# sdecoder/AVX-sort-merge-joins

Hardware: AMD Instinct MI355X
Metric: join throughput Mtuples/s (R⋈S) + achieved HBM GB/s, 128M⋈128M at 1/2/4/8 GPU (higher is better)
Workload: dtype int64; 1 GPU; sortmergejoin_multiway R=128000000 S=128000000 per GPU, 16-byte tuples, uniform, PK/FK keys 1..|R|, row-id payloads (48-bit intermediates); tuples_per_relation_per_gpu=128000000, tuples_per_relation_total=128000000, tuple_bytes=16, payload=rowid, distribution=uniform, parallelism=range-partition x1

## Files before the change

avx-sort-merge-joins_amd/csrc/bucketsort.hip:

```cpp
#include <algorithm>
#include <type_traits>
#include <vector>

#include "smj_common.hpp"
#include "smj_internal.hpp"

namespace smj {

#ifndef SMJ_TP_THREADS
#define SMJ_TP_THREADS 1024
#endif
constexpr int TP_THREADS = SMJ_TP_THREADS;
#ifndef SMJ_TP_PERSIST
#define SMJ_TP_PERSIST 1
#endif
#ifndef SMJ_GS_XCD
#define SMJ_GS_XCD 1
#endif
#ifndef SMJ_GS_PAIR
#define SMJ_GS_PAIR 1
#endif
#ifndef SMJ_GS_TWO
#define SMJ_GS_TWO 1
#endif
#ifndef SMJ_GS_META_PREFETCH
#define SMJ_GS_META_PREFETCH 0
#endif
#ifndef SMJ_GS_ARGS_MEM
#define SMJ_GS_ARGS_MEM 1
#endif
#ifndef SMJ_TP_STAGE4
#define SMJ_TP_STAGE4 (64 * 1024)
#endif
#ifndef SMJ_TP_STAGE8
#define SMJ_TP_STAGE8 (128 * 1024)
#endif
template <class W>
constexpr int tp_items() {
    return (int)((sizeof(W) == 4 ? SMJ_TP_STAGE4 : sizeof(W) == 8 ? SMJ_TP_STAGE8 : 128 * 1024)
                 / sizeof(W)) / TP_THREADS;
}
template <class W>
constexpr uint32_t tile_elems() {
    return (uint32_t)(TP_THREADS * tp_items<W>());
}
static_assert(tile_elems<uint64_t>() <= 65535 + 1, "u16 prefix rows");
template <class Lay>
struct TileStage {
    static constexpr uint32_t kBytes = sizeof(typename Lay::W);
    static constexpr int kItems = tp_items<typename Lay::W>();
};
template <>
struct TileStage<LayP48> {
    static constexpr uint32_t kBytes = 4;
    static constexpr int kItems = tp_items<uint64_t>();
};
template <class Lay>
constexpr uint32_t tile_elems_l() {
    return (uint32_t)(TP_THREADS * TileStage<Lay>::kItems);
}
#ifndef SMJ_PLAN_TILE
#define SMJ_PLAN_TILE 16384
#endif
const uint32_t kTileTuples = SMJ_PLAN_TILE;

#ifndef SMJ_GS_THREADS
#define SMJ_GS_THREADS 256
#endif
constexpr int GS_THREADS = SMJ_GS_THREADS;
#ifndef SMJ_GS_WG_PER_CU
#define SMJ_GS_WG_PER_CU 2
#endif
#ifndef SMJ_GS_WG_PER_CU8
#define SMJ_GS_WG_PER_CU8 4
#endif
#ifndef SMJ_GS_WG_PER_CU12
#define SMJ_GS_WG_PER_CU12 3
#endif
#ifndef SMJ_GS_WG_PER_CU4P
#define SMJ_GS_WG_PER_CU4P 5
#endif
template <class W, bool PAIR = false>
constexpr int gs_wg_per_cu() {
    return sizeof(W) == 16 ? SMJ_GS_WG_PER_CU
         : sizeof(W) == 12 ? SMJ_GS_WG_PER_CU12
         : (sizeof(W) == 4 && PAIR) ? SMJ_GS_WG_PER_CU4P : SMJ_GS_WG_PER_CU8;
}
#ifndef SMJ_GS_ITEMS
#define SMJ_GS_ITEMS (2560 / SMJ_GS_THREADS)
#endif
constexpr int GS_ITEMS = SMJ_GS_ITEMS;
constexpr int GS_CAP = GS_THREADS * GS_ITEMS;
constexpr int GS_D3MAX = GS_CAP >= 2048 ? 11 : 10;
constexpr int GS_BPT = (1 << GS_D3MAX) / GS_THREADS;
constexpr int GS_NB3 = 1 << GS_D3MAX;
constexpr int GS_TMAX = 256;
constexpr int GS_WIN = GS_CAP / 64;
constexpr int GS_RUNMAX = 32;
static_assert(GS_CAP % 64 == 0 && GS_CAP % GS_THREADS == 0, "group capacity");

#ifdef KEY_8B
typedef int64_t KeyT;
#else
typedef int32_t KeyT;
#endif

struct TileTable {
    uint64_t* off;
    uint32_t* len;
    uint32_t* bucket;
    uint32_t* btile0;
    uint16_t* pref;
    uint16_t* prefT;
    uint32_t tstride;
};

struct OvfEntry {
    uint32_t bucket, d2;
    uint32_t nr[2];
    uint64_t off[2];
    uint32_t counted;
    uint32_t pad;
};

__global__ void __launch_bounds__(64)
k_tiles(const uint64_t* __restrict__ bstart, const int64_t* __restrict__ bcount,
        const uint64_t* __restrict__ seg_start, const int64_t* __restrict__ seg_cnt,
        uint32_t nseg, TileTable tt, uint32_t tsz) {
    const uint32_t b = blockIdx.x;
    uint32_t t0 = tt.btile0[b];
    for (uint32_t q = 0; q < nseg; q++) {
        const uint64_t s0 = seg_start ? seg_start[(size_t)b * nseg + q] : bstart[b];
        const int64_t cnt = seg_cnt ? seg_cnt[(size_t)b * nseg + q] : bcount[b];
        const uint32_t nt = (uint32_t)((cnt + tsz - 1) / tsz);
        for (uint32_t i = threadIdx.x; i < nt; i += 64) {
            const uint64_t o = (uint64_t)i * tsz;
            const int64_t rem = cnt - (int64_t)o;
            tt.off[t0 + i] = s0 + o;
            tt.len[t0 + i] = (uint32_t)(rem < (int64_t)tsz ? rem : tsz);
            tt.bucket[t0 + i] = b;
        }
        t0 += nt;
    }
}

struct TilePassArgs {
    const void* part[2];
    void* tmp[2];
    TileTable tt[2];
    uint32_t t0[2];
    uint32_t nt[2];
    const uint32_t* ntiles[2];
    RangePlan plan;
    uint32_t nb2;
    const unsigned int* pack_bad;
    uint32_t d2_fast;
    uint64_t pstride[2] = {0, 0};
    uint64_t ostride[2] = {0, 0};
};

template <class Lay, class LayO = Lay>
__global__ void __launch_bounds__(TP_THREADS)
k_tilepass(TilePassArgs A) {
    typedef typename Lay::W W;
    static_assert(std::is_same<W, typename LayO::W>::value, "one element type");
    typedef TileStage<Lay> TS;
    constexpr int TP_ITEMS = TS::kItems;
    constexpr uint32_t TSZ = tile_elems_l<Lay>();
    extern __shared__ __attribute__((aligned(16))) unsigned char lds_raw[];
    if (A.pack_bad && *A.pack_bad) return;
    const RangePlan& P = A.plan;
    const uint32_t nb2 = A.nb2;
    W* stage = reinterpret_cast<W*>(lds_raw);
    uint32_t* hist = reinterpret_cast<uint32_t*>(lds_raw + ((TSZ * TS::kBytes + 15) & ~15u));
    uint32_t* scr = hist + nb2;

    const int r = blockIdx.x < A.nt[0] ? 0 : 1;
    const uint32_t t = A.t0[r] + (r ? blockIdx.x - A.nt[0] : blockIdx.x);
    if (A.ntiles[r] && t >= *A.ntiles[r]) return;
    const TileTable& tt = A.tt[r];
    const typename Lay::CView part = Lay::cview(A.part[r], A.pstride[r]);
    const typename LayO::View tmp =
        LayO::view(A.tmp[r], std::is_same<Lay, LayO>::value ? A.pstride[r] : A.ostride[r]);
    const uint64_t off = tt.off[t];
    const uint32_t len = tt.len[t];
    const uint32_t b = tt.bucket[t];

    for (uint32_t d = threadIdx.x; d < nb2; d += TP_THREADS) hist[d] = 0;
    W v[TP_ITEMS];
    uint32_t dg[TP_ITEMS];
#pragma unroll
    for (int j = 0; j < TP_ITEMS; j++) {
        uint32_t i = j * TP_THREADS + threadIdx.x;
        if (i < len) v[j] = part[off + i];
    }
    __syncthreads();
    if (A.d2_fast && b != 0 && b != (1u << P.D1) - 1) {
        const uint32_t base_lo = (uint32_t)P.base, mask = nb2 - 1;
#pragma unroll
        for (int j = 0; j < TP_ITEMS; j++) {
            uint32_t i = j * TP_THREADS + threadIdx.x;
            if (i < len) {
                dg[j] = Lay::digit_fast(v[j], base_lo, P.s1, P.s2, mask);
                atomicAdd(&hist[dg[j]], 1u);
            }
        }
    } else {
#pragma unroll
        for (int j = 0; j < TP_ITEMS; j++) {
            uint32_t i = j * TP_THREADS + threadIdx.x;
            if (i < len) {
                dg[j] = plan_d2(P, Lay::rel(P, v[j], b), b);
                atomicAdd(&hist[dg[j]], 1u);
            }
        }
    }
    __syncthreads();
    const uint32_t per = (nb2 + TP_THREADS - 1) / TP_THREADS;
    const uint32_t d0 = threadIdx.x * per;
    uint32_t loc = 0;
    for (uint32_t k = 0; k < per; k++)
        if (d0 + k < nb2) loc += hist[d0 + k];
    uint32_t tot;
    uint32_t ex = block_exclusive_scan(loc, scr, &tot);
    uint16_t* pref = tt.pref + (uint64_t)t * (nb2 + 1);
    for (uint32_t k = 0; k < per; k++) {
        uint32_t d = d0 + k;
        if (d < nb2) {
            uint32_t c = hist[d];
            hist[d] = ex;
            pref[d] = (uint16_t)ex;
            ex += c;
        }
    }
    if (threadIdx.x == 0) pref[nb2] = (uint16_t)len;
    __syncthreads();
#pragma unroll
    for (int j = 0; j < TP_ITEMS; j++) {
        uint32_t i = j * TP_THREADS + threadIdx.x;
        if (i < len) {
            uint32_t pos = atomicAdd(&hist[dg[j]], 1u);
            stage[pos] = v[j];
        }
    }
    __syncthreads();
#pragma unroll
    for (int j = 0; j < TP_ITEMS; j++) {
        uint32_t i = j * TP_THREADS + threadIdx.x;
        if (i < len) st_w(tmp + off + i, stage[i]);
    }
}

template <class LayO>
struct Plane2;
template <>
struct Plane2<LayP48> {
    typedef uint16_t T;
};
template <>
struct Plane2<LayP40> {
    typedef uint8_t T;
};
__device__ __forceinline__ void st_plane(G32 p, uint32_t v) {
#if SMJ_NT_STORES
    __builtin_nontemporal_store(v, p);
#else
    *p = v;
#endif
}
__device__ __forceinline__ void st_plane(G16 p, uint16_t v) {
#if SMJ_NT_STORES
    __builtin_nontemporal_store(v, p);
#else
    *p = v;
#endif
}
__device__ __forceinline__ void st_plane(G8 p, uint8_t v) {
#if SMJ_NT_STORES
    __builtin_nontemporal_store(v, p);
#else
    *p = v;
#endif
}

constexpr int TP48_WG_PER_CU = 2;

template <class LayO>
__global__ void __launch_bounds__(TP_THREADS, TP48_WG_PER_CU * TP_THREADS / 256)
k_tilepass48(TilePassArgs A) {
    typedef LayP48 Lay;
    typedef typename Plane2<LayO>::T HT;
    constexpr int TP_ITEMS = TileStage<Lay>::kItems;
    constexpr uint32_t TSZ = tile_elems_l<Lay>();
    static_assert(TP_ITEMS % 2 == 0, "uint16 pairs");
    static_assert(TileStage<Lay>::kBytes == 4 && (TSZ + 4) * sizeof(HT) <= TSZ * 4, "one stage");
    extern __shared__ __attribute__((aligned(16))) unsigned char lds_raw[];
    if (A.pack_bad && *A.pack_bad) return;
    const RangePlan& P = A.plan;
    const uint32_t nb2 = A.nb2;
    uint32_t* stage_lo = reinterpret_cast<uint32_t*>(lds_raw);
    HT* stage_hi = reinterpret_cast<HT*>(lds_raw);
    uint32_t* hist = reinterpret_cast<uint32_t*>(lds_raw + ((TSZ * 4 + 15) & ~15u));
    uint32_t* scr = hist + nb2;

    const int r = blockIdx.x < A.nt[0] ? 0 : 1;
    const uint32_t t = A.t0[r] + (r ? blockIdx.x - A.nt[0] : blockIdx.x);
    if (A.ntiles[r] && t >= *A.ntiles[r]) return;
    const TileTable& tt = A.tt[r];
    const uint64_t off = tt.off[t];
    const uint32_t len = tt.len[t];
    const uint32_t b = tt.bucket[t];
    const Lay::CView part = Lay::cview(A.part[r], A.pstride[r]) + off;
    const typename LayO::View tmp =
        LayO::view(A.tmp[r], std::is_same<Lay, LayO>::value ? A.pstride[r] : A.ostride[r]) + off;

    for (uint32_t d = threadIdx.x; d < nb2; d += TP_THREADS) hist[d] = 0;
    uint32_t lo[TP_ITEMS];
    uint32_t hp[TP_ITEMS / 2];
    uint32_t rk[TP_ITEMS / 2];
#pragma unroll
    for (int k = 0; k < TP_ITEMS / 2; k++) {
        uint32_t h[2] = {0, 0};
#pragma unroll
        for (int e = 0; e < 2; e++) {
            const int j = 2 * k + e;
            const uint32_t i = j * TP_THREADS + threadIdx.x;
            lo[j] = 0;
            if (i < len) {
                lo[j] = (part.lo + j * TP_THREADS)[threadIdx.x];
                h[e] = (part.hi + j * TP_THREADS)[threadIdx.x];
            }
        }
        hp[k] = h[0] | (h[1] << 16);
    }
    auto word = [&](int j) -> uint64_t {
        const uint32_t h = (j & 1) ? hp[j >> 1] >> 16 : hp[j >> 1] & 0xffffu;
        return (uint64_t)lo[j] | ((uint64_t)h << 32);
    };
    __syncthreads();
    const bool fast = A.d2_fast && b != 0 && b != (1u << P.D1) - 1;
    const uint32_t base_lo = (uint32_t)P.base, mask = nb2 - 1;
    if (fast) {
#pragma unroll
        for (int j = 0; j < TP_ITEMS; j++) {
            const uint32_t i = j * TP_THREADS + threadIdx.x;
            if (i < len) atomicAdd(&hist[Lay::digit_fast(word(j), base_lo, P.s1, P.s2, mask)], 1u);
        }
    } else {
#pragma unroll
        for (int j = 0; j < TP_ITEMS; j++) {
            const uint32_t i = j * TP_THREADS + threadIdx.x;
            if (i < len) atomicAdd(&hist[plan_d2(P, Lay::rel(P, word(j), b), b)], 1u);
        }
    }
    __syncthreads();
    const uint32_t per = (nb2 + TP_THREADS - 1) / TP_THREADS;
    const uint32_t d0 = threadIdx.x * per;
    uint32_t loc = 0;
    for (uint32_t k = 0; k < per; k++)
        if (d0 + k < nb2) loc += hist[d0 + k];
    uint32_t tot;
    uint32_t ex = block_exclusive_scan(loc, scr, &tot);
    uint16_t* pref = tt.pref + (uint64_t)t * (nb2 + 1);
    for (uint32_t k = 0; k < per; k++) {
        uint32_t d = d0 + k;
        if (d < nb2) {
            uint32_t c = hist[d];
            hist[d] = ex;
            pref[d] = (uint16_t)ex;
            ex += c;
        }
    }
    if (threadIdx.x == 0) pref[nb2] = (uint16_t)len;
    __syncthreads();
#pragma unroll
    for (int k = 0; k < TP_ITEMS / 2; k++) {
        uint32_t p[2] = {0, 0};
#pragma unroll
        for (int e = 0; e < 2; e++) {
            const int j = 2 * k + e;
            const uint32_t i = j * TP_THREADS + threadIdx.x;
            if (i < len) {
                const uint64_t w = word(j);
                const uint32_t d = fast ? Lay::digit_fast(w, base_lo, P.s1, P.s2, mask)
                                        : plan_d2(P, Lay::rel(P, w, b), b);
                p[e] = atomicAdd(&hist[d], 1u);
                stage_lo[p[e]] = lo[j];
            }
        }
        rk[k] = p[0] | (p[1] << 16);
    }
    __syncthreads();
#pragma unroll
    for (int j = 0; j < TP_ITEMS; j++) {
        const uint32_t i = j * TP_THREADS + threadIdx.x;
        if (i < len) st_plane(tmp.lo + j * TP_THREADS + threadIdx.x, stage_lo[i]);
    }
    __syncthreads();
    constexpr uint32_t EPD = 4 / sizeof(HT);
    const uint32_t pad = (uint32_t)(((uintptr_t)tmp.hi & 3u) / sizeof(HT));
#pragma unroll
    for (int j = 0; j < TP_ITEMS; j++) {
        const uint32_t i = j * TP_THREADS + threadIdx.x;
        if (i < len) {
            const uint32_t pos = (j & 1) ? rk[j >> 1] >> 16 : rk[j >> 1] & 0xffffu;
            const uint32_t h = (j & 1) ? hp[j >> 1] >> 16 : hp[j >> 1];
            stage_hi[pad + pos] = (HT)h;
        }
    }
    __syncthreads();
    const uint32_t end = pad + len;
    const uint32_t nq = (end + EPD - 1) / EPD;
    const uint32_t* stage_q = reinterpret_cast<const uint32_t*>(lds_raw);
    const G32 out_q = (G32)(tmp.hi - pad);
    constexpr int NQ = (int)((TSZ / EPD + TP_THREADS - 1) / TP_THREADS) + 1;
#pragma unroll
    for (int j = 0; j < NQ; j++) {
        const uint32_t q = j * TP_THREADS + threadIdx.x;
        if (q < nq) {
            const uint32_t e0 = q * EPD;
            if (e0 >= pad && e0 + EPD <= end) {
                st_plane(out_q + j * TP_THREADS + threadIdx.x, stage_q[q]);
            } else {
#pragma unroll
                for (uint32_t e = e0; e < e0 + EPD; e++)
                    if (e >= pad && e < end) st_plane(tmp.hi + (e - pad), stage_hi[e]);
            }
        }
    }
}

template <class Lay, class LayO>
struct TilePassP {
    typedef typename Lay::W W;
    static constexpr int ITEMS = tp_items<W>();
    __device__ static __forceinline__ uint32_t elem(int j) {
        return (uint32_t)j * TP_THREADS + threadIdx.x;
    }
    const TilePassArgs& A;
    W* stage;
    uint32_t* hist;
    uint32_t* scr;
    uint32_t n0, total;

    struct Meta {
        uint64_t off;
        uint32_t len, b, t;
        int r;
    };
    __device__ __forceinline__ Meta meta(uint32_t idx) const {
        const bool none = idx >= total;
        if (none) idx = total - 1;
        Meta m;
        m.r = idx < n0 ? 0 : 1;
        m.t = A.t0[m.r] + (m.r ? idx - n0 : idx);
        const TileTable& tt = A.tt[m.r];
        typedef const __attribute__((address_space(4))) uint64_t* C64;
        typedef const __attribute__((address_space(4))) uint32_t* C32;
        m.off = ((C64)tt.off)[m.t];
        m.len = none ? 0u : ((C32)tt.len)[m.t];
        m.b = ((C32)tt.bucket)[m.t];
        return m;
    }
    __device__ __forceinline__ void load(W (&v)[ITEMS], const Meta& m) const {
        const typename Lay::CView part = Lay::cview(A.part[m.r], A.pstride[m.r]) + m.off;
        const uint32_t lim = m.len ? m.len - 1 : 0u;
#pragma unroll
        for (int j = 0; j < ITEMS; j++) {
            const uint32_t i = elem(j);
            v[j] = part[i < lim ? i : lim];
        }
    }
    template <bool RANK>
    __device__ __forceinline__ void digits(const W (&v)[ITEMS], const Meta& m) const {
        const RangePlan& P = A.plan;
        if (A.d2_fast && m.b != 0 && m.b != (1u << P.D1) - 1) {
            const uint32_t base_lo = (uint32_t)P.base, mask = A.nb2 - 1;
#pragma unroll
            for (int j = 0; j < ITEMS; j++) {
                const uint32_t i = elem(j);
                if (i < m.len) {
                    const uint32_t d = Lay::digit_fast(v[j], base_lo, P.s1, P.s2, mask);
                    if (RANK)
                        stage[atomicAdd(&hist[d], 1u)] = v[j];
                    else
                        atomicAdd(&hist[d], 1u);
                }
            }
        } else {
#pragma unroll
            for (int j = 0; j < ITEMS; j++) {
                const uint32_t i = elem(j);
                if (i < m.len) {
                    const uint32_t d = plan_d2(P, Lay::rel(P, v[j], m.b), m.b);
                    if (RANK)
                        stage[atomicAdd(&hist[d], 1u)] = v[j];
                    else
                        atomicAdd(&hist[d], 1u);
                }
            }
        }
    }
    __device__ __forceinline__ void tile(const W (&v)[ITEMS], const Meta& m) const {
        const uint32_t nb2 = A.nb2;
        __syncthreads();
        digits<false>(v, m);
        __syncthreads();
        const uint32_t per = (nb2 + TP_THREADS - 1) / TP_THREADS;
        const uint32_t d0 = threadIdx.x * per;
        uint32_t loc = 0;
        for (uint32_t k = 0; k < per; k++)
            if (d0 + k < nb2) loc += hist[d0 + k];
        uint32_t tot;
        uint32_t ex = block_exclusive_scan(loc, scr, &tot);
        uint16_t* pref = A.tt[m.r].pref + (uint64_t)m.t * (nb2 + 1);
        for (uint32_t k = 0; k < per; k++) {
            const uint32_t d = d0 + k;
            if (d < nb2) {
                const uint32_t c = hist[d];
                hist[d] = ex;
                pref[d] = (uint16_t)ex;
                ex += c;
            }
        }
        if (threadIdx.x == 0) pref[nb2] = (uint16_t)m.len;
        __syncthreads();
        digits<true>(v, m);
        __syncthreads();
        for (uint32_t d = threadIdx.x; d < nb2; d += TP_THREADS) hist[d] = 0;
        const typename LayO::View tmp = LayO::view(
            A.tmp[m.r], std::is_same<Lay, LayO>::value ? A.pstride[m.r] : A.ostride[m.r]) + m.off;
#pragma unroll
        for (int j = 0; j < ITEMS; j++) {
            const uint32_t i = elem(j);
            if (i < m.len) st_w(tmp + i, stage[i]);
        }
    }
};

template <class Lay, class LayO = Lay>
__global__ void __launch_bounds__(TP_THREADS)
k_tilepass_p(TilePassArgs A) {
    typedef TilePassP<Lay, LayO> TP;
    typedef typename TP::W W;
    static_assert(std::is_same<W, typename LayO::W>::value, "one element type");
    extern __shared__ __attribute__((aligned(16))) unsigned char lds_raw[];
    if (A.pack_bad && *A.pack_bad) return;
    TP s{A};
    s.stage = reinterpret_cast<W*>(lds_raw);
    s.hist = reinterpret_cast<uint32_t*>(lds_raw + tile_elems<W>() * sizeof(W));
    s.scr = s.hist + A.nb2;
    uint32_t n[2];
    for (int r = 0; r < 2; r++)
        n[r] = A.nt[r] == 0 ? 0u : A.ntiles[r] ? min(*A.ntiles[r], A.nt[r]) : A.nt[r];
    s.n0 = n[0];
    s.total = n[0] + n[1];
    uint32_t idx = blockIdx.x;
    if (idx >= s.total) return;
    for (uint32_t d = threadIdx.x; d < A.nb2; d += TP_THREADS) s.hist[d] = 0;
    W a[TP::ITEMS], b[TP::ITEMS];
    typename TP::Meta ma = s.meta(idx), mb;
    s.load(a, ma);
    for (;;) {
        mb = s.meta(idx + gridDim.x);
        s.load(b, mb);
        s.tile(a, ma);
        if ((idx += gridDim.x) >= s.total) break;
        ma = s.meta(idx + gridDim.x);
        s.load(a, ma);
        s.tile(b, mb);
        if ((idx += gridDim.x) >= s.total) break;
    }
}

constexpr int PT_TILES = 64;
__global__ void __launch_bounds__(256)
k_preft(TileTable tt0, TileTable tt1, uint32_t nb0, const uint32_t* __restrict__ ntiles0,
        const uint32_t* __restrict__ ntiles1, uint32_t nt0_host, uint32_t nt1_host,
        uint32_t nb2) {
    extern __shared__ uint16_t sp[];
    const int r = blockIdx.x < nb0 ? 0 : 1;
    const TileTable& tt = r ? tt1 : tt0;
    const uint32_t ntl = (r ? ntiles1 : ntiles0) ? *(r ? ntiles1 : ntiles0)
                                                 : (r ? nt1_host : nt0_host);
    const uint32_t tb = (r ? blockIdx.x - nb0 : blockIdx.x) * PT_TILES;
    if (tb >= ntl) return;
    const uint32_t nt = min((uint32_t)PT_TILES, ntl - tb);
    const uint32_t row = nb2 + 1;
    const uint16_t* src = tt.pref + (uint64_t)tb * row;
    for (uint32_t i = threadIdx.x; i < nt * row; i += 256) sp[i] = src[i];
    __syncthreads();
    for (uint32_t i = threadIdx.x; i < row * PT_TILES; i += 256) {
        const uint32_t d = i / PT_TILES, t = i % PT_TILES;
        if (t < nt) tt.prefT[(uint64_t)d * tt.tstride + tb + t] = sp[t * row + d];
    }
}

struct GroupArgs {
    const void* tmp[2];
    Tup* out[2];
    const uint64_t* bstart[2];
    const uint64_t* ostart[2];
    TileTable tt[2];
    int nrel;
    RangePlan plan;
    unsigned long long* count_dev;
    uint32_t nb2;
    uint32_t g_begin, g_end;
    uint32_t per;
    OvfEntry* ovf;
    uint32_t* novf;
    uint32_t ovf_cap;
    const unsigned int* pack_bad;
    uint32_t d3_fast;
    uint64_t pstride[2] = {0, 0};
    uint32_t pair;
};

__device__ __forceinline__ uint32_t otid() {
    uint32_t t = threadIdx.x;
    asm volatile("" : "+v"(t));
    return t;
}

template <class W>
struct GroupLDS {
    W B[GS_CAP + 1];
    uint32_t cnt[2][GS_NB3 / 2];
    uint32_t cur[GS_NB3 / 2];
    uint32_t run[2][GS_TMAX];
    struct alignas(16) Win {
        unsigned long long m;
        uint32_t wk, pad;
    } win[2][GS_WIN];
    uint32_t wtot[2][GS_THREADS / 64];
    uint32_t flags;
    unsigned long long scan64[GS_THREADS / 64 + 1];
    uint32_t n[2];
    uint32_t off[2];
};

struct SrcPlain {
    __device__ static __forceinline__ void run(const TileTable& tt, uint32_t nb2, uint32_t t,
                                               uint32_t g, uint32_t& lo, uint32_t& len) {
        const uint16_t* pf = tt.prefT + (uint64_t)g * tt.tstride + t;
        lo = pf[0];
        len = (uint32_t)(pf[tt.tstride] - pf[0]);
    }
    template <class V>
    __device__ static __forceinline__ auto load(const V& p) { return p[0]; }
};

template <int TPL>
struct GroupMeta {
    uint32_t b[2], g[2];
    uint32_t t0[2], nt[2];
    uint64_t bst[2];
    uint64_t ost[2];
    uint32_t lo[TPL], len[TPL];
    uint32_t toff[TPL];
};

template <bool PAIR>
__device__ __forceinline__ int group_slots(const GroupArgs& A) { return PAIR ? 2 : A.nrel; }

template <class Src, bool PAIR, int TPL>
__device__ __forceinline__ void load_meta(const GroupArgs& A, uint32_t g0, uint32_t stride,
                                          uint32_t cnt, uint32_t j, GroupMeta<TPL>& M,
                                          bool same_bucket) {
    const int nslot = group_slots<PAIR>(A);
    auto bucket_meta = [&](int r, uint32_t b) {
        M.t0[r] = __builtin_amdgcn_readfirstlane(A.tt[r].btile0[b]);
        M.nt[r] = __builtin_amdgcn_readfirstlane(A.tt[r].btile0[b + 1]) - M.t0[r];
        const uint64_t bs = A.bstart[r][b];
        M.bst[r] = ((uint64_t)__builtin_amdgcn_readfirstlane((uint32_t)(bs >> 32)) << 32) |
                   __builtin_amdgcn_readfirstlane((uint32_t)bs);
        const uint64_t os = A.ostart[r][b];
        M.ost[r] = ((uint64_t)__builtin_amdgcn_readfirstlane((uint32_t)(os >> 32)) << 32) |
                   __builtin_amdgcn_readfirstlane((uint32_t)os);
    };
    if (!PAIR) {
        const uint32_t gi = g0 + j * stride;
        const uint32_t b = gi / A.nb2;
        M.g[0] = gi % A.nb2;
        if (!same_bucket || b != M.b[0]) {
#pragma unroll
            for (int r = 0; r < 2; r++) {
                M.t0[r] = M.nt[r] = 0;
                M.bst[r] = M.ost[r] = 0;
                if (r < A.nrel) bucket_meta(r, b);
            }
        }
        M.b[0] = b;
    } else {
#pragma unroll
        for (int r = 0; r < 2; r++) {
            const uint32_t k = 2 * j + r;
            const bool valid = k < cnt;
            const uint32_t gi = g0 + k * stride;
            const uint32_t b = valid ? gi / A.nb2 : 0xffffffffu;
            M.g[r] = valid ? gi % A.nb2 : 0u;
            if (!valid) {
                M.t0[r] = M.nt[r] = 0;
                M.bst[r] = M.ost[r] = 0;
            } else if (!same_bucket || b != M.b[r]) {
                bucket_meta(r, b);
            }
            M.b[r] = b;
        }
    }
    const uint32_t wid = __builtin_amdgcn_readfirstlane(otid() >> 6), lane = otid() & 63;
#pragma unroll
    for (int h = 0; h < TPL; h++) M.lo[h] = M.len[h] = M.toff[h] = 0;
    if (wid < (uint32_t)nslot) {
        const uint32_t nt = wid ? M.nt[1] : M.nt[0];
        const uint32_t t0 = wid ? M.t0[1] : M.t0[0];
        const uint32_t g = PAIR && wid ? M.g[1] : M.g[0];
#pragma unroll
        for (int h = 0; h < TPL; h++) {
            const uint32_t t = lane + 64 * h;
            if (nt <= 64 * TPL && t < nt) {
                Src::run(A.tt[wid], A.nb2, t0 + t, g, M.lo[h], M.len[h]);
                M.toff[h] = (uint32_t)(A.tt[wid].off[t0 + t] - (wid ? M.bst[1] : M.bst[0]));
            }
        }
    }
}

__device__ __forceinline__ uint32_t wave_incl_scan32(uint32_t x) {
    const int lane = lane_id();
#pragma unroll
    for (int o = 1; o < 64; o <<= 1) {
        const uint32_t y = __shfl_up(x, o, 64);
        if (lane >= o) x += y;
    }
    return x;
}

__device__ __forceinline__ unsigned long long wave_incl_scan64(unsigned long long x) {
    const int lane = lane_id();
#pragma unroll
    for (int o = 1; o < 64; o <<= 1) {
        const unsigned long long y = __shfl_up(x, o, 64);
        if (lane >= o) x += y;
    }
    return x;
}

__device__ __forceinline__ void wave_lds_sync() {
    __builtin_amdgcn_fence(__ATOMIC_RELEASE, "wavefront");
    __builtin_amdgcn_wave_barrier();
    __builtin_amdgcn_fence(__ATOMIC_ACQUIRE, "wavefront");
}

__device__ __forceinline__ unsigned long long block_scan64(unsigned long long v,
                                                           unsigned long long* scr,
                                                           unsigned long long* total) {
    const int lane = lane_id(), wid = otid() >> 6, nw = blockDim.x >> 6;
    const unsigned long long x = wave_incl_scan64(v);
    if (lane == 63) scr[wid] = x;
    __syncthreads();
    if (otid() == 0) {
        unsigned long long run = 0;
        for (int w = 0; w < nw; w++) {
            const unsigned long long t = scr[w];
            scr[w] = run;
            run += t;
        }
        scr[nw] = run;
    }
    __syncthreads();
    const unsigned long long r = scr[wid] + x - v;
    *total = scr[nw];
    __syncthreads();
    return r;
}

template <class Lay>
__device__ __forceinline__ void insertion_sort(typename Lay::W* a, uint32_t n) {
    for (uint32_t i = 1; i < n; i++) {
        typename Lay::W x = a[i];
        uint32_t j = i;
        while (j > 0 && Lay::less(x, a[j - 1])) {
            a[j] = a[j - 1];
            j--;
        }
        a[j] = x;
    }
}

template <bool PAIR, int TPL, class LDS>
__device__ __forceinline__ void build_tables(const GroupArgs& A, LDS& L,
                                             const GroupMeta<TPL>& M) {
    const uint32_t wid = otid() >> 6, lane = otid() & 63;
    if (wid < (uint32_t)group_slots<PAIR>(A)) {
        const int r = wid;
        const uint32_t nt = r ? M.nt[1] : M.nt[0];
        if (lane < GS_WIN) L.win[r][lane].m = 0ull;
        unsigned long long acc = 0;
        uint32_t kacc = 0;
        uint32_t s[TPL], k[TPL];
        bool e[TPL];
#pragma unroll
        for (int h = 0; h < TPL; h++) {
            const unsigned long long p = ((unsigned long long)M.lo[h] << 32) | M.len[h];
            const unsigned long long incl = wave_incl_scan64(p) + acc;
            acc = __shfl(incl, 63, 64);
            s[h] = (uint32_t)(incl - p);
            e[h] = lane + 64 * h < nt && M.len[h] > 0 && s[h] < GS_CAP;
            const uint64_t bal = __ballot(e[h]);
            k[h] = kacc + (uint32_t)__popcll(bal & lanemask_lt());
            kacc += (uint32_t)__popcll(bal);
        }
#pragma unroll
        for (int h = 0; h < TPL; h++)
            if (e[h]) L.run[r][k[h]] = M.toff[h] + M.lo[h] - s[h];
        if (lane == 0) {
            L.n[r] = nt <= 64 * TPL ? (uint32_t)acc : 0xffffffffu;
            L.off[r] = (uint32_t)(acc >> 32);
        }
        wave_lds_sync();
#pragma unroll
        for (int h = 0; h < TPL; h++)
            if (e[h]) atomicOr(&L.win[r][s[h] >> 6].m, 1ull << (s[h] & 63));
        wave_lds_sync();
        const uint32_t c = lane < GS_WIN ? (uint32_t)__popcll(L.win[r][lane].m) : 0u;
        const uint32_t incl = wave_incl_scan32(c);
        if (lane < GS_WIN) L.win[r][lane].wk = incl - c - 1u;
    }
    __syncthreads();
}

template <class Src, bool PAIR, class LDS, class Meta>
__device__ __forceinline__ void group_overflow(const GroupArgs& A, LDS& L,
                                               const Meta& M, int slot = 0) {
    uint32_t nn[2] = {0, 0};
    uint64_t oo[2] = {0, 0};
    const uint32_t tid = otid();
    const int nq = PAIR ? 1 : A.nrel;
#pragma unroll
    for (int q = 0; q < 2; q++) {
        if (q >= nq) break;
        const int r = PAIR ? slot : q;
        const uint32_t t0 = r ? M.t0[1] : M.t0[0], nt = r ? M.nt[1] : M.nt[0];
        const uint32_t g = PAIR && r ? M.g[1] : M.g[0];
        unsigned long long acc = 0;
        for (uint32_t t = tid; t < nt; t += GS_THREADS) {
            uint32_t lo, len;
            Src::run(A.tt[r], A.nb2, t0 + t, g, lo, len);
            acc += ((unsigned long long)lo << 32) | len;
        }
        unsigned long long tot;
        (void)block_scan64(acc, L.scan64, &tot);
        nn[q] = (uint32_t)tot;
        oo[q] = tot >> 32;
    }
    if (tid == 0) {
        const uint32_t k = atomicAdd(A.novf, 1u);
        if (k < A.ovf_cap) {
            OvfEntry e;
            e.bucket = PAIR && slot ? M.b[1] : M.b[0];
            e.d2 = PAIR && slot ? M.g[1] : M.g[0];
            e.nr[0] = nn[0];
            e.nr[1] = nn[1];
            e.off[0] = oo[0];
            e.off[1] = oo[1];
            e.counted = 0;
            e.pad = 0;
            A.ovf[k] = e;
        }
    }
    __syncthreads();
}

template <class Lay, class Src, class Meta>
__device__ __forceinline__ void gather_group(const GroupArgs& A, GroupLDS<typename Lay::W>& L,
                                             const Meta& C, int r, uint32_t grp, uint32_t n,
                                             typename Lay::W (&v)[GS_ITEMS]) {
    if (n == 0) return;
    const typename Lay::CView tp =
        with_group(Lay::cview(A.tmp[r], A.pstride[r]), grp, A.plan) + C.bst[r];
    const uint32_t lane = lane_id();
    const uint32_t wid = __builtin_amdgcn_readfirstlane(otid() >> 6);
    typedef uint32_t U4 __attribute__((ext_vector_type(4)));
#pragma unroll
    for (int k = 0; k < GS_ITEMS; k++) {
        const uint32_t w = k * (GS_THREADS / 64) + wid;
        const U4 win = *reinterpret_cast<const U4*>(&L.win[r][w]);
        const uint32_t below = __builtin_amdgcn_mbcnt_hi(win.y, __builtin_amdgcn_mbcnt_lo(win.x, 0u));
        const uint32_t at = (uint32_t)((((uint64_t)win.y << 32) | win.x) >> lane) & 1u;
        const uint32_t j = w * 64 + lane;
        v[k] = Src::load(tp + (min(j, n - 1) + L.run[r][win.z + below + at]));
    }
}

template <class Lay, bool PAIR, class Meta, typename Hook>
__device__ __forceinline__ bool sort_group(const GroupArgs& A, GroupLDS<typename Lay::W>& L,
                                           const Meta& C, const RangePlan& P,
                                           int r, uint32_t nr, uint32_t off,
                                           typename Lay::W (&v)[GS_ITEMS], bool& clamped,
                                           Hook&& after_place) {
    const uint32_t tid = otid(), wid = tid >> 6, lane = tid & 63;
    const uint32_t cb = PAIR && r ? C.b[1] : C.b[0], cg = PAIR && r ? C.g[1] : C.g[0];
    const uint32_t d12 = (cb << P.D2) | cg;
    uint32_t dg[GS_ITEMS];
    const bool edge = (cb == 0 && cg == 0) ||
                      (cb == (1u << P.D1) - 1 && cg == A.nb2 - 1);
    if (A.d3_fast && !edge) {
        const uint32_t base_lo = (uint32_t)P.base, mask = (1u << P.D3) - 1;
#pragma unroll
        for (int k = 0; k < GS_ITEMS; k++) {
            const bool valid = k * GS_THREADS + tid < nr;
            dg[k] = Lay::digit_fast(v[k], base_lo, P.s1, P.s3, mask);
            if (valid) atomicAdd(&L.cnt[r][dg[k] >> 1], 1u << ((dg[k] & 1) * 16));
        }
    } else {
#pragma unroll
        for (int k = 0; k < GS_ITEMS; k++) {
            const bool valid = k * GS_THREADS + tid < nr;
            clamped |= valid && Lay::clamped(P, v[k]);
            dg[k] = plan_d3(P, Lay::rel(P, v[k], cb), d12);
            if (valid) atomicAdd(&L.cnt[r][dg[k] >> 1], 1u << ((dg[k] & 1) * 16));
        }
    }
    __syncthreads();
    uint32_t c[GS_BPT];
    uint32_t loc = 0, mx = 0;
#pragma unroll
    for (int q = 0; q < GS_BPT / 2; q++) {
        const uint32_t wv = L.cnt[r][tid * (GS_BPT / 2) + q];
        c[2 * q] = wv & 0xffffu;
        c[2 * q + 1] = wv >> 16;
        loc += c[2 * q] + c[2 * q + 1];
        mx = max(mx, max(c[2 * q], c[2 * q + 1]));
    }
    const uint32_t incl = wave_incl_scan32(loc);
    if (lane == 63) L.wtot[0][wid] = incl;
    const bool dup = __syncthreads_or(mx > 1);
    uint32_t ex = incl - loc;
#pragma unroll
    for (uint32_t w = 0; w < GS_THREADS / 64; w++)
        if (w < wid) ex += L.wtot[0][w];
    const uint32_t first = ex;
#pragma unroll
    for (int q = 0; q < GS_BPT / 2; q++) {
        const uint32_t lo16 = ex;
        ex += c[2 * q];
        L.cur[tid * (GS_BPT / 2) + q] = lo16 | (ex << 16);
        ex += c[2 * q + 1];
    }
    __syncthreads();
#pragma unroll
    for (int k = 0; k < GS_ITEMS; k++) {
        const bool valid = k * GS_THREADS + tid < nr;
        const uint32_t sh = (dg[k] & 1) * 16;
        const uint32_t old = dup ? atomicAdd(&L.cur[dg[k] >> 1], valid ? 1u << sh : 0u)
                                 : L.cur[valid ? dg[k] >> 1 : 0u];
        L.B[valid ? (old >> sh) & 0xffffu : GS_CAP] = v[k];
    }
    after_place();
    __syncthreads();
    if (dup) {
        bool ok = true;
        for (uint32_t i = tid + 1; i < nr; i += GS_THREADS)
            ok &= !Lay::less(L.B[i], L.B[i - 1]);
        if (__syncthreads_or(!ok)) {
            uint32_t e = first;
            bool has_long = false;
#pragma unroll
            for (int q = 0; q < GS_BPT; q++) {
                const uint32_t b0 = e;
                e += c[q];
                if (c[q] > 1) {
                    if (c[q] <= GS_RUNMAX)
                        insertion_sort<Lay>(L.B + b0, c[q]);
                    else
                        has_long = true;
                }
            }
            if (__syncthreads_or(has_long)) {
                ok = true;
                for (uint32_t i = tid + 1; i < nr; i += GS_THREADS)
                    ok &= !Lay::less(L.B[i], L.B[i - 1]);
                if (__syncthreads_or(!ok)) return false;
            }
        }
    }
    Tup* dst = A.out[r] + C.ost[r] + off;
#pragma unroll
    for (int k = 0; k < GS_ITEMS; k++) {
        const uint32_t j = k * GS_THREADS + tid;
        if (j < nr) st_stream(dst + j, Lay::unpack(P, L.B[j], cb));
    }
    return true;
}

template <class T>
__device__ __forceinline__ void launder(T& x) {
    static_assert(sizeof(T) % 4 == 0, "word-sized");
    uint32_t* w = reinterpret_cast<uint32_t*>(&x);
#pragma unroll
    for (int i = 0; i < (int)(sizeof(T) / 4); i++) asm volatile("" : "+v"(w[i]));
}

template <class Lay>
__device__ __forceinline__ bool fix_runs(GroupLDS<typename Lay::W>& L, uint32_t nr,
                                         const uint32_t (&c)[GS_BPT], uint32_t first) {
    const uint32_t tid = otid();
    bool ok = true;
    for (uint32_t i = tid + 1; i < nr; i += GS_THREADS) ok &= !Lay::less(L.B[i], L.B[i - 1]);
    if (!__syncthreads_or(!ok)) return true;
    uint32_t e = first;
    bool has_long = false;
#pragma unroll
    for (int q = 0; q < GS_BPT; q++) {
        const uint32_t b0 = e;
        e += c[q];
        if (c[q] > 1) {
            if (c[q] <= GS_RUNMAX)
                insertion_sort<Lay>(L.B + b0, c[q]);
            else
                has_long = true;
        }
    }
    if (__syncthreads_or(has_long)) {
        ok = true;
        for (uint32_t i = tid + 1; i < nr; i += GS_THREADS) ok &= !Lay::less(L.B[i], L.B[i - 1]);
        if (__syncthreads_or(!ok)) return false;
    }
    return true;
}

template <class Lay, bool PAIR, class Meta, typename Hook0, typename Hook1>
__device__ __forceinline__ uint32_t sort_two(const GroupArgs& A, GroupLDS<typename Lay::W>& L,
                                             const Meta& C, const RangePlan& P,
                                             const uint32_t (&nr)[2], const uint32_t (&off)[2],
                                             typename Lay::W (&v0)[GS_ITEMS],
                                             typename Lay::W (&v1)[GS_ITEMS], bool join,
                                             unsigned long long& matches, bool& exact,
                                             Hook0&& after0, Hook1&& after1) {
    typedef typename Lay::W W;
    const uint32_t tid = otid(), wid = tid >> 6, lane = tid & 63;
    auto fast = [&](int r) {
        const uint32_t cb = PAIR && r ? C.b[1] : C.b[0], cg = PAIR && r ? C.g[1] : C.g[0];
        const bool edge = (cb == 0 && cg == 0) || (cb == (1u << P.D1) - 1 && cg == A.nb2 - 1);
        return A.d3_fast && !edge;
    };
    auto slow_digit = [&](int r, const W& x) -> uint32_t {
        const uint32_t cb = PAIR && r ? C.b[1] : C.b[0], cg = PAIR && r ? C.g[1] : C.g[0];
        return plan_d3(P, Lay::rel(P, x, cb), (cb << P.D2) | cg);
    };
    const uint32_t base_lo = (uint32_t)P.base, mask3 = (1u << P.D3) - 1;
    bool clamped = false;
    auto hist = [&](int r, const W(&v)[GS_ITEMS]) {
        if (fast(r)) {
            const typename Lay::FastDigit fd(P, P.s3, P.D3);
#pragma unroll
            for (int k = 0; k < GS_ITEMS; k++) {
                const uint32_t d = fd(v[k]);
                if (k * GS_THREADS + tid < nr[r])
                    atomicAdd(&L.cnt[r][d >> 1], 1u << ((d & 1) * 16));
            }
        } else {
#pragma unroll
            for (int k = 0; k < GS_ITEMS; k++) {
                const bool valid = k * GS_THREADS + tid < nr[r];
                clamped |= valid && Lay::clamped(P, v[k]);
                const uint32_t d = slow_digit(r, v[k]);
                if (valid) atomicAdd(&L.cnt[r][d >> 1], 1u << ((d & 1) * 16));
            }
        }
    };
    hist(0, v0);
    hist(1, v1);
    __syncthreads();
    uint32_t w0[GS_BPT / 2], w1[GS_BPT / 2];
    uint32_t loc0 = 0, loc1 = 0, mx0 = 0, mx1 = 0;
#pragma unroll
    for (int q = 0; q < GS_BPT / 2; q++) {
        w0[q] = L.cnt[0][tid * (GS_BPT / 2) + q];
        w1[q] = L.cnt[1][tid * (GS_BPT / 2) + q];
        const uint32_t a0 = w0[q] & 0xffffu, a1 = w0[q] >> 16;
        const uint32_t b0 = w1[q] & 0xffffu, b1 = w1[q] >> 16;
        loc0 += a0 + a1;
        loc1 += b0 + b1;
        mx0 = max(mx0, max(a0, a1));
        mx1 = max(mx1, max(b0, b1));
    }
    const uint32_t incl0 = wave_incl_scan32(loc0), incl1 = wave_incl_scan32(loc1);
    if (lane == 63) {
        L.wtot[0][wid] = incl0;
        L.wtot[1][wid] = incl1;
    }
    const uint32_t vote = (mx0 > 1 ? 1u : 0u) | (mx1 > 1 ? 2u : 0u) | (clamped ? 4u : 0u);
    if (vote) atomicOr(&L.flags, vote);
    __syncthreads();
    const uint32_t fl = __builtin_amdgcn_readfirstlane(L.flags);
    exact = join && P.s3 == 0 && !(fl & 4);
    unsigned long long m = 0;
    if (exact) {
#pragma unroll
        for (int q = 0; q < GS_BPT / 2; q++)
            m += (unsigned long long)(w0[q] & 0xffffu) * (w1[q] & 0xffffu) +
                 (unsigned long long)(w0[q] >> 16) * (w1[q] >> 16);
    }
    uint32_t ex0 = incl0 - loc0, ex1 = incl1 - loc1;
#pragma unroll
    for (uint32_t w = 0; w < GS_THREADS / 64; w++)
        if (w < wid) {
            ex0 += L.wtot[0][w];
            ex1 += L.wtot[1][w];
        }
#pragma unroll
    for (int q = 0; q < GS_BPT / 2; q++) {
        uint32_t lo16 = ex0;
        ex0 += w0[q] & 0xffffu;
        L.cur[tid * (GS_BPT / 2) + q] = lo16 | (ex0 << 16);
        ex0 += w0[q] >> 16;
        lo16 = ex1;
        ex1 += w1[q] & 0xffffu;
        L.cnt[1][tid * (GS_BPT / 2) + q] = lo16 | (ex1 << 16);
        ex1 += w1[q] >> 16;
    }
    __syncthreads();
    if (tid == 0) L.flags = 0;
    auto place1 = [&](uint32_t* cur, bool dup, bool valid, uint32_t d, const W& x) {
        const uint32_t sh = (d & 1) * 16;
        const uint32_t old = dup ? atomicAdd(&cur[d >> 1], valid ? 1u << sh : 0u)
                                 : cur[valid ? d >> 1 : 0u];
        L.B[valid ? (old >> sh) & 0xffffu : GS_CAP] = x;
    };
    auto place_loop = [&](int r, uint32_t* cur, const W(&v)[GS_ITEMS], auto&& digit,
                          auto dupc) {
#pragma unroll
        for (int k = 0; k < GS_ITEMS; k++) {
            W x = v[k];
            launder(x);
            place1(cur, decltype(dupc)::value, k * GS_THREADS + tid < nr[r], digit(x), v[k]);
        }
    };
    auto place = [&](int r, uint32_t* cur, bool dup, const W(&v)[GS_ITEMS]) {
        typedef std::integral_constant<bool, true> Dup;
        typedef std::integral_constant<bool, false> NoDup;
        if (fast(r)) {
            const typename Lay::FastDigit fd(P, P.s3, P.D3);
            if (dup) place_loop(r, cur, v, fd, Dup());
            else place_loop(r, cur, v, fd, NoDup());
        } else {
            auto sd = [&](const W& x) { return slow_digit(r, x); };
            if (dup) place_loop(r, cur, v, sd, Dup());
            else place_loop(r, cur, v, sd, NoDup());
        }
    };
    auto fix = [&](int r, const uint32_t* cur) {
        uint32_t c[GS_BPT];
        const uint32_t first = tid ? cur[tid * (GS_BPT / 2) - 1] >> 16 : 0u;
        uint32_t prev = first;
#pragma unroll
        for (int q = 0; q < GS_BPT / 2; q++) {
            const uint32_t e = cur[tid * (GS_BPT / 2) + q];
            c[2 * q] = (e & 0xffffu) - prev;
            c[2 * q + 1] = (e >> 16) - (e & 0xffffu);
            prev = e >> 16;
        }
        return fix_runs<Lay>(L, nr[r], c, first);
    };
    auto write = [&](int r) {
        const uint32_t cb = PAIR && r ? C.b[1] : C.b[0];
        Tup* dst = A.out[r] + C.ost[r] + off[r];
        const typename Lay::Unpack up(P, cb);
#pragma unroll
        for (int k = 0; k < GS_ITEMS; k++) {
            const uint32_t j = k * GS_THREADS + tid;
            if (j < nr[r]) st_stream(dst + j, up(L.B[j]));
        }
    };
    uint32_t failed = 0;
    place(0, L.cur, fl & 1, v0);
    after0();
    __syncthreads();
    if ((fl & 1) && !fix(0, L.cur)) failed |= 1;
    if (!failed) write(0);
    if (!(join && failed)) {
        __syncthreads();
        place(1, L.cnt[1], fl & 2, v1);
        after1();
        __syncthreads();
        if ((fl & 2) && !fix(1, L.cnt[1])) failed |= 2;
        if (!(failed & 2)) write(1);
    } else {
        after1();
        __syncthreads();
    }
#pragma unroll
    for (int q = 0; q < GS_BPT / 2; q++) {
        L.cnt[0][tid * (GS_BPT / 2) + q] = 0u;
        L.cnt[1][tid * (GS_BPT / 2) + q] = 0u;
    }
    if (!failed) matches += m;
    return failed;
}

template <class Lay, class Meta>
__device__ __forceinline__ void count_by_search(const GroupArgs& A, GroupLDS<typename Lay::W>& L,
                                                const Meta& C, const RangePlan& P,
                                                const uint32_t (&cn)[2], const uint32_t (&co)[2],
                                                unsigned long long& matches) {
    const uint32_t tid = otid();
    const Tup* Rs = A.out[0] + C.ost[0] + co[0];
    const uint32_t nR = cn[0], nS = cn[1];
    for (uint32_t i = tid; i < nS; i += GS_THREADS) {
        const int64_t k = tup_key(Lay::unpack(P, L.B[i], C.b[0]));
        if (i > 0 && tup_key(Lay::unpack(P, L.B[i - 1], C.b[0])) == k) continue;
        uint32_t e = i + 1;
        while (e < nS && tup_key(Lay::unpack(P, L.B[e], C.b[0])) == k) e++;
        uint32_t lo = 0, hi = nR;
        while (lo < hi) {
            const uint32_t m = (lo + hi) >> 1;
            if (tup_key(Rs[m]) < k) lo = m + 1; else hi = m;
        }
        const uint32_t lb = lo;
        hi = nR;
        while (lo < hi) {
            const uint32_t m = (lo + hi) >> 1;
            if (tup_key(Rs[m]) <= k) lo = m + 1; else hi = m;
        }
        matches += (unsigned long long)(lo - lb) * (e - i);
    }
}

template <class Lay, int TPL, class Src, bool PAIR>
__device__ __forceinline__ void group_loop(const GroupArgs& A0, GroupLDS<typename Lay::W>& L,
                                           uint32_t g0, uint32_t stride, uint32_t cnt,
                                           unsigned long long& matches) {
    typedef typename Lay::W W;
    const GroupArgs& A = A0;
    const RangePlan& P = A.plan;
    const uint32_t tid = otid();
    const int nrel = A.nrel;
    constexpr bool pair = PAIR;
    const int nslot = group_slots<PAIR>(A);
    if (cnt == 0) return;
    const uint32_t nit = pair ? (cnt + 1) / 2 : cnt;
    auto fits = [&](const uint32_t (&n)[2], bool f[2]) {
        f[0] = n[0] <= GS_CAP;
        f[1] = n[1] <= GS_CAP;
        if (!pair) f[0] = f[1] = f[0] && f[1];
    };

    for (uint32_t i = tid; i < GS_NB3; i += GS_THREADS) (&L.cnt[0][0])[i] = 0u;
    if (tid == 0) L.flags = 0u;
    GroupMeta<TPL> M;
    load_meta<Src, PAIR>(A, g0, stride, cnt, 0, M, false);
    build_tables<PAIR>(A, L, M);
    GroupMeta<TPL> C = M;
    uint32_t cn[2], co[2];
#pragma unroll
    for (int r = 0; r < 2; r++) {
        cn[r] = r < nslot ? __builtin_amdgcn_readfirstlane(L.n[r]) : 0;
        co[r] = r < nslot ? __builtin_amdgcn_readfirstlane(L.off[r]) : 0;
    }
    bool cf[2];
    fits(cn, cf);
    W vr[GS_ITEMS], vs[GS_ITEMS];
    auto slot_g = [&](const GroupMeta<TPL>& X, int r) { return PAIR && r ? X.g[1] : X.g[0]; };
    if (cf[0]) gather_group<Lay, Src>(A, L, C, 0, slot_g(C, 0), cn[0], vr);
    if (cf[1] && nslot > 1) gather_group<Lay, Src>(A, L, C, 1, slot_g(C, 1), cn[1], vs);
    if (nit > 1 && SMJ_GS_META_PREFETCH) load_meta<Src, PAIR>(A, g0, stride, cnt, 1, M, true);

    for (uint32_t j = 0; j < nit; j++) {
#if SMJ_GS_ARGS_MEM
        typedef const __attribute__((address_space(4))) GroupArgs* ConstArgs;
        ConstArgs Aj = (ConstArgs)&A0;
        asm volatile("" : "+s"(Aj));
        const GroupArgs& A = *(const GroupArgs*)Aj;
        const RangePlan& P = A.plan;
#endif
        const bool has_next = j + 1 < nit;
        if (!SMJ_GS_META_PREFETCH && has_next) load_meta<Src, PAIR>(A, g0, stride, cnt, j + 1, M, true);
        __syncthreads();
        const GroupMeta<TPL> N = M;
        uint32_t nn[2] = {0, 0}, no[2] = {0, 0};
        if (has_next) {
            build_tables<PAIR>(A, L, N);
#pragma unroll
            for (int r = 0; r < 2; r++) {
                nn[r] = r < nslot ? __builtin_amdgcn_readfirstlane(L.n[r]) : 0;
                no[r] = r < nslot ? __builtin_amdgcn_readfirstlane(L.off[r]) : 0;
            }
        }
        if (SMJ_GS_META_PREFETCH && j + 2 < nit)
            load_meta<Src, PAIR>(A, g0, stride, cnt, j + 2, M, true);
        bool nf[2];
        fits(nn, nf);
        nf[0] &= has_next;
        nf[1] &= has_next;
        auto gather_next_r = [&]() {
            if (nf[0]) gather_group<Lay, Src>(A, L, N, 0, slot_g(N, 0), nn[0], vr);
        };
        auto gather_next_s = [&]() {
            if (nf[1] && nslot > 1) gather_group<Lay, Src>(A, L, N, 1, slot_g(N, 1), nn[1], vs);
        };
        bool cleared = false;
        if (SMJ_GS_TWO && nslot == 2 && (pair || (cf[0] && cf[1]))) {
            const bool join = !pair;
            bool exact = false;
            const uint32_t nr2[2] = {cf[0] ? cn[0] : 0u, cf[1] ? cn[1] : 0u};
            const uint32_t failed = sort_two<Lay, PAIR>(A, L, C, P, nr2, co, vr, vs, join, matches,
                                                         exact, gather_next_r, gather_next_s);
            cleared = true;
            if (join) {
                if (failed) {
                    __syncthreads();
                    group_overflow<Src, PAIR>(A, L, C);
                } else if (!exact) {
                    count_by_search<Lay>(A, L, C, P, cn, co, matches);
                }
            } else {
                for (int q = 0; q < 2; q++)
                    if (!cf[q] || (failed & (1u << q))) {
                        __syncthreads();
                        group_overflow<Src, PAIR>(A, L, C, q);
                    }
            }
        } else if (pair && !SMJ_GS_TWO) {
            bool clamped = false;
            bool ok = cf[0] && sort_group<Lay, PAIR>(A, L, C, P, 0, cn[0], co[0], vr, clamped,
                                               gather_next_r);
            if (!cf[0]) gather_next_r();
            if (!ok) {
                __syncthreads();
                group_overflow<Src, PAIR>(A, L, C, 0);
            }
            ok = cf[1] && sort_group<Lay, PAIR>(A, L, C, P, 1, cn[1], co[1], vs, clamped,
                                          gather_next_s);
            if (!cf[1]) gather_next_s();
            if (!ok) {
                __syncthreads();
                group_overflow<Src, PAIR>(A, L, C, 1);
            }
        } else if (!cf[0] || (SMJ_GS_TWO && SMJ_GS_PAIR)) {
            group_overflow<Src, PAIR>(A, L, C);
            gather_next_r();
            gather_next_s();
        } else {
            bool clamped = false;
            bool ok = sort_group<Lay, PAIR>(A, L, C, P, 0, cn[0], co[0], vr, clamped, gather_next_r);
            bool s_issued = false;
            if (ok && nrel > 1) {
                ok = sort_group<Lay, PAIR>(A, L, C, P, 1, cn[1], co[1], vs, clamped, gather_next_s);
                s_issued = true;
            }
            if (!ok) {
                __syncthreads();
                group_overflow<Src, PAIR>(A, L, C);
                if (!s_issued) gather_next_s();
            } else if (nrel == 2) {
                const bool exact = P.s3 == 0 && !__syncthreads_or(clamped);
                if (exact) {
#pragma unroll
                    for (int q = 0; q < GS_BPT / 2; q++) {
                        const uint32_t a0 = L.cnt[0][tid * (GS_BPT / 2) + q];
                        const uint32_t a1 = L.cnt[1][tid * (GS_BPT / 2) + q];
                        matches += (unsigned long long)(a0 & 0xffffu) * (a1 & 0xffffu) +
                                   (unsigned long long)(a0 >> 16) * (a1 >> 16);
                    }
                } else {
                    count_by_search<Lay>(A, L, C, P, cn, co, matches);
                }
            }
        }
        if (!cleared) {
            __syncthreads();
            for (uint32_t i = tid; i < GS_NB3; i += GS_THREADS) (&L.cnt[0][0])[i] = 0u;
        }
        C = N;
        cn[0] = nn[0];
        cn[1] = nn[1];
        co[0] = no[0];
        co[1] = no[1];
        cf[0] = nf[0];
        cf[1] = nf[1];
    }
}

#if SMJ_GS_ARGS_MEM
typedef const GroupArgs* __restrict__ GroupArgsParam;
#define SMJ_GS_ARGS_REF(p) (*(p))
#else
typedef GroupArgs GroupArgsParam;
#define SMJ_GS_ARGS_REF(p) (p)
#endif

__global__ void k_put_args(GroupArgs G, GroupArgs* dst) { *dst = G; }

template <class Lay, int TPL, bool PAIR>
__global__ void __launch_bounds__(GS_THREADS,
                                  (gs_wg_per_cu<typename Lay::W, PAIR>() * GS_THREADS / 256))
k_groupsort(GroupArgsParam Ap) {
    typedef typename Lay::W W;
    const GroupArgs& A = SMJ_GS_ARGS_REF(Ap);
    extern __shared__ __attribute__((aligned(16))) unsigned char lds_raw[];
    if (A.pack_bad && *A.pack_bad) return;
    GroupLDS<W>& L = *reinterpret_cast<GroupLDS<W>*>(lds_raw);
#if SMJ_GS_XCD
    const uint32_t nx = gridDim.x / 8, k = blockIdx.x / 8;
    const uint32_t lo = A.g_begin + (blockIdx.x % 8) * nx * A.per;
    const uint32_t g0 = lo + k, stride = nx;
    const uint32_t hi = min(lo + nx * A.per, A.g_end);
    const uint32_t cnt = g0 < hi ? (hi - g0 + nx - 1) / nx : 0u;
#else
    const uint32_t g0 = A.g_begin + blockIdx.x * A.per, stride = 1;
    const uint32_t cnt = g0 < A.g_end ? min(A.per, A.g_end - g0) : 0u;
#endif
    unsigned long long matches = 0;
    if (cnt == 0) return;
    group_loop<Lay, TPL, SrcPlain, PAIR>(A, L, g0, stride, cnt, matches);
    if (A.nrel == 2) {
        matches = wave_sum(matches);
        if ((otid() & 63) == 0 && matches) atomicAdd(A.count_dev, matches);
    }
}

#ifndef SMJ_SK_THREADS
#define SMJ_SK_THREADS 256
#endif
constexpr int SK_THREADS = SMJ_SK_THREADS;
constexpr int SK_ITEMS = 8;
constexpr int SK_CHUNK = SK_THREADS * SK_ITEMS;
constexpr uint32_t kSkewSmall = SK_THREADS * 64;
#ifndef SMJ_SKEW_ITEM
#define SMJ_SKEW_ITEM 8192
#endif
constexpr int SK_TM = 256;

struct SkewArgs {
    GroupArgs G;
    OvfEntry* q;
    const uint32_t* list;
    const uint4* items;
    uint32_t n;
    uint32_t* ghist;
    const uint32_t* slot;
    uint32_t* gflag;
};

template <class Lay>
__device__ __forceinline__ typename Lay::CView skew_run(const GroupArgs& G, int r, uint32_t g,
                                                      uint32_t t0, uint32_t t, uint32_t& len) {
    const TileTable& tt = G.tt[r];
    const uint16_t* pf = tt.prefT + (uint64_t)g * tt.tstride + t0 + t;
    const uint32_t lo = pf[0];
    len = (uint32_t)(pf[tt.tstride] - lo);
    return with_group(Lay::cview(G.tmp[r], G.pstride[r]), g, G.plan) + (tt.off[t0 + t] + lo);
}

constexpr uint32_t SK_WIN = kSkewSmall / 64;
static_assert(SK_WIN == SK_THREADS, "one window per thread when the run tables are built");

struct SkewSmallLDS {
    uint32_t h[2][GS_NB3];
    unsigned long long first[GS_NB3];
    uint64_t base[SK_TM];
    struct Win {
        unsigned long long m;
        uint32_t wk, pad;
    } win[SK_WIN];
    unsigned long long scr[SK_THREADS / 64 + 1];
};

template <class Lay, class F>
__device__ __forceinline__ void skew_for_each(const GroupArgs& G, const SkewSmallLDS& L, int r,
                                              uint32_t g, uint32_t t0, uint32_t nt, uint32_t n,
                                              F&& f) {
    typedef typename Lay::W W;
    if (nt <= SK_TM) {
        const typename Lay::CView tmp = with_group(Lay::cview(G.tmp[r], G.pstride[r]), g, G.plan);
        const uint32_t lane = lane_id();
        const uint32_t wid = __builtin_amdgcn_readfirstlane(threadIdx.x >> 6);
        for (uint32_t c = 0; c < n; c += SK_CHUNK) {
            W v[SK_ITEMS];
#pragma unroll
            for (int k = 0; k < SK_ITEMS; k++) {
                const uint32_t w = (c + k * SK_THREADS) / 64 + wid;
                const uint32_t j = w * 64 + lane;
                const bool ok = j < n;
                const auto win = L.win[ok ? w : 0u];
                const uint32_t below = __builtin_amdgcn_mbcnt_hi(
                    (uint32_t)(win.m >> 32), __builtin_amdgcn_mbcnt_lo((uint32_t)win.m, 0u));
                const uint32_t at = (uint32_t)(win.m >> lane) & 1u;
                const uint32_t q = ok ? win.wk + below + at : 0u;
                v[k] = tmp[(uint64_t)(ok ? j : 0u) + L.base[q]];
            }
#pragma unroll
            for (int k = 0; k < SK_ITEMS; k++) f(v[k], c + k * SK_THREADS + threadIdx.x < n);
        }
    } else {
        for (uint32_t t = 0; t < nt; t++) {
            uint32_t len;
            const typename Lay::CView src = skew_run<Lay>(G, r, g, t0, t, len);
            for (uint32_t i0 = 0; i0 < len; i0 += SK_THREADS) {
                const uint32_t i = i0 + threadIdx.x;
                f(src[i < len ? i : len - 1], i < len);
            }
        }
    }
}

__device__ __forceinline__ bool skew_inversion(const Tup* dst, uint32_t lo, uint32_t hi) {
    bool inv = false;
    for (uint32_t c = lo; c < hi; c += SK_CHUNK) {
        Tup a[SK_ITEMS], b[SK_ITEMS];
#pragma unroll
        for (int k = 0; k < SK_ITEMS; k++) {
            const uint32_t i = min(c + k * SK_THREADS + threadIdx.x, hi - 1);
            a[k] = dst[i - 1];
            b[k] = dst[i];
        }
#pragma unroll
        for (int k = 0; k < SK_ITEMS; k++)
            if (c + k * SK_THREADS + threadIdx.x < hi) inv |= tup_less(b[k], a[k]);
    }
    return inv;
}

template <class Lay>
__global__ void __launch_bounds__(SK_THREADS)
k_skew_small(SkewArgs K) {
    typedef typename Lay::W W;
    __shared__ SkewSmallLDS L;
    const GroupArgs& G = K.G;
    const RangePlan& P = G.plan;
    const uint32_t qi = K.list[blockIdx.x];
    const OvfEntry e = K.q[qi];
    const uint32_t d12 = (e.bucket << P.D2) | e.d2;
    const uint32_t tid = threadIdx.x;
    uint32_t t0[2] = {0, 0}, nt[2] = {0, 0};
    for (uint32_t i = tid; i < 2 * GS_NB3; i += SK_THREADS) (&L.h[0][0])[i] = 0;
    __syncthreads();
    for (int r = 0; r < G.nrel; r++) {
        t0[r] = G.tt[r].btile0[e.bucket];
        nt[r] = G.tt[r].btile0[e.bucket + 1] - t0[r];
    }
    auto tables = [&](int r) {
        if (nt[r] > SK_TM) return;
        __syncthreads();
        L.win[tid].m = 0ull;
        uint32_t len = 0;
        uint64_t src = 0;
        if (tid < nt[r]) {
            const TileTable& tt = G.tt[r];
            const uint16_t* pf = tt.prefT + (uint64_t)e.d2 * tt.tstride + t0[r] + tid;
            len = (uint32_t)(pf[tt.tstride] - pf[0]);
            src = tt.off[t0[r] + tid] + pf[0];
        }
        const unsigned long long acc = ((unsigned long long)(len ? 1u : 0u) << 32) | len;
        unsigned long long tot;
        const unsigned long long ex = block_scan64(acc, L.scr, &tot);
        const uint32_t st = (uint32_t)ex, k = (uint32_t)(ex >> 32);
        if (len) {
            L.base[k] = src - st;
            atomicOr(&L.win[st >> 6].m, 1ull << (st & 63));
        }
        __syncthreads();
        const uint32_t cw = (uint32_t)__popcll(L.win[tid].m);
        unsigned long long wt;
        const uint32_t wex = (uint32_t)block_scan64(cw, L.scr, &wt);
        L.win[tid].wk = wex - 1u;
        __syncthreads();
    };
    bool clamped = false;
    for (int r = 0; r < G.nrel; r++) {
        tables(r);
        skew_for_each<Lay>(G, L, r, e.d2, t0[r], nt[r], e.nr[r], [&](const W& x, bool ok) {
            clamped |= ok && Lay::clamped(P, x);
            if (ok) atomicAdd(&L.h[r][plan_d3(P, Lay::rel(P, x, e.bucket), d12)], 1u);
        });
    }
    const bool exact = P.s3 == 0 && !__syncthreads_or(clamped);
    if (!exact) {
        for (int r = 0; r < G.nrel; r++) {
            Tup* dst = G.out[r] + G.ostart[r][e.bucket] + e.off[r];
            uint32_t pos = 0;
            for (uint32_t t = 0; t < nt[r]; t++) {
                uint32_t len;
                const typename Lay::CView src = skew_run<Lay>(G, r, e.d2, t0[r], t, len);
                for (uint32_t i = tid; i < len; i += SK_THREADS)
                    dst[pos + i] = Lay::unpack(P, src[i], e.bucket);
                pos += len;
            }
        }
        if (tid == 0) K.gflag[qi] |= 1u;
        return;
    }
    if (G.nrel == 2) {
        unsigned long long m = 0;
        for (uint32_t d = tid; d < GS_NB3; d += SK_THREADS)
            m += (unsigned long long)L.h[0][d] * L.h[1][d];
        m = wave_sum(m);
        if ((tid & 63) == 0 && m) atomicAdd(G.count_dev, m);
        if (tid == 0) K.q[qi].counted = 1;
    }
    bool inv = false;
    for (int r = 0; r < G.nrel; r++) {
        Tup* dst = G.out[r] + G.ostart[r][e.bucket] + e.off[r];
        constexpr int BPT = GS_NB3 / SK_THREADS;
        uint32_t c[BPT];
        unsigned long long loc = 0;
#pragma unroll
        for (int k = 0; k < BPT; k++) {
            c[k] = L.h[r][tid * BPT + k];
            loc += c[k];
        }
        unsigned long long tot;
        unsigned long long ex = block_scan64(loc, L.scr, &tot);
#pragma unroll
        for (int k = 0; k < BPT; k++) {
            L.h[r][tid * BPT + k] = (uint32_t)ex;
            ex += c[k];
        }
        __syncthreads();
        for (uint32_t d = tid; d < GS_NB3; d += SK_THREADS) L.first[d] = ~0ull;
        tables(r);
        __syncthreads();
        bool differ = false;
        skew_for_each<Lay>(G, L, r, e.d2, t0[r], nt[r], e.nr[r], [&](const W& x, bool ok) {
            const uint32_t d = plan_d3(P, Lay::rel(P, x, e.bucket), d12);
            if (ok) {
                dst[atomicAdd(&L.h[r][d], 1u)] = Lay::unpack(P, x, e.bucket);
                const unsigned long long id = Lay::same_key_id(x);
                const unsigned long long old = atomicCAS(&L.first[d], ~0ull, id);
                differ |= id == ~0ull || (old != ~0ull && old != id);
            }
        });
        __threadfence_block();
        if (__syncthreads_or(differ)) inv |= skew_inversion(dst, 1, e.nr[r]);
    }
    if (__syncthreads_or(inv) && tid == 0) K.gflag[qi] |= 2u;
}

template <class Lay>
__global__ void __launch_bounds__(SK_THREADS)
k_skew_hist(SkewArgs K) {
    typedef typename Lay::W W;
    __shared__ uint32_t h[GS_NB3];
    const GroupArgs& G = K.G;
    const RangePlan& P = G.plan;
    const uint4 it = K.items[blockIdx.x];
    const uint32_t qi = it.x, sl = it.y, r = it.z >> 16, s = it.z & 0xffffu, ts = it.w;
    const OvfEntry e = K.q[qi];
    const uint32_t t0 = G.tt[r].btile0[e.bucket];
    const uint32_t nt = G.tt[r].btile0[e.bucket + 1] - t0;
    if (s >= nt) return;
    for (uint32_t d = threadIdx.x; d < GS_NB3; d += SK_THREADS) h[d] = 0;
    __syncthreads();
    const uint32_t d12 = (e.bucket << P.D2) | e.d2;
    bool clamped = false;
    for (uint32_t t = s; t < nt; t += ts) {
        uint32_t len;
        const typename Lay::CView src = skew_run<Lay>(G, (int)r, e.d2, t0, t, len);
        for (uint32_t c = 0; c < len; c += SK_CHUNK) {
            W v[SK_ITEMS];
#pragma unroll
            for (int k = 0; k < SK_ITEMS; k++) {
                const uint32_t i = c + k * SK_THREADS + threadIdx.x;
                v[k] = src[i < len ? i : len - 1];
            }
#pragma unroll
            for (int k = 0; k < SK_ITEMS; k++) {
                const uint32_t i = c + k * SK_THREADS + threadIdx.x;
                const bool ok = i < len;
                clamped |= ok && Lay::clamped(P, v[k]);
                if (ok) atomicAdd(&h[plan_d3(P, Lay::rel(P, v[k], e.bucket), d12)], 1u);
            }
        }
    }
    const bool any = __syncthreads_or(clamped);
    uint32_t* gh = K.ghist + ((size_t)sl * 2 + r) * GS_NB3;
    for (uint32_t d = threadIdx.x; d < GS_NB3; d += SK_THREADS)
        if (h[d]) atomicAdd(&gh[d], h[d]);
    if (any && threadIdx.x == 0) atomicOr(&K.gflag[qi], 1u);
}

__global__ void __launch_bounds__(SK_THREADS)
k_skew_scan(SkewArgs K) {
    __shared__ unsigned long long scr[SK_THREADS / 64 + 1];
    const uint32_t qi = K.list[blockIdx.x], sl = K.slot[blockIdx.x];
    const RangePlan& P = K.G.plan;
    const bool exact = P.s3 == 0 && !(K.gflag[qi] & 1u);
    if (!exact) return;
    uint32_t* gh = K.ghist + (size_t)sl * 2 * GS_NB3;
    if (K.G.nrel == 2) {
        unsigned long long m = 0;
        for (uint32_t d = threadIdx.x; d < GS_NB3; d += SK_THREADS)
            m += (unsigned long long)gh[d] * gh[GS_NB3 + d];
        m = wave_sum(m);
        if ((threadIdx.x & 63) == 0 && m) atomicAdd(K.G.count_dev, m);
        if (threadIdx.x == 0) K.q[qi].counted = 1;
    }
    constexpr int BPT = GS_NB3 / SK_THREADS;
    for (int r = 0; r < K.G.nrel; r++) {
        uint32_t* h = gh + r * GS_NB3;
        uint32_t c[BPT];
        unsigned long long loc = 0;
#pragma unroll
        for (int k = 0; k < BPT; k++) {
            c[k] = h[threadIdx.x * BPT + k];
            loc += c[k];
        }
        unsigned long long tot;
        unsigned long long ex = block_scan64(loc, scr, &tot);
#pragma unroll
        for (int k = 0; k < BPT; k++) {
            h[threadIdx.x * BPT + k] = (uint32_t)ex;
            ex += c[k];
        }
    }
}

template <class Lay>
__global__ void __launch_bounds__(SK_THREADS)
k_skew_place(SkewArgs K) {
    typedef typename Lay::W W;
    __shared__ uint32_t h[GS_NB3];
    __shared__ unsigned long long scr[SK_THREADS / 64 + 1];
    const GroupArgs& G = K.G;
    const RangePlan& P = G.plan;
    const uint4 it = K.items[blockIdx.x];
    const uint32_t qi = it.x, sl = it.y, r = it.z >> 16, s = it.z & 0xffffu, ts = it.w;
    const OvfEntry e = K.q[qi];
    const uint32_t t0 = G.tt[r].btile0[e.bucket];
    const uint32_t nt = G.tt[r].btile0[e.bucket + 1] - t0;
    if (s >= nt) return;
    Tup* dst = G.out[r] + G.ostart[r][e.bucket] + e.off[r];
    const bool exact = P.s3 == 0 && !(K.gflag[qi] & 1u);
    if (!exact) {
        for (uint32_t t = s; t < nt; t += ts) {
            unsigned long long acc = 0;
            for (uint32_t u = threadIdx.x; u < t; u += SK_THREADS) {
                uint32_t l;
                (void)skew_run<Lay>(G, (int)r, e.d2, t0, u, l);
                acc += l;
            }
            unsigned long long pos;
            (void)block_scan64(acc, scr, &pos);
            uint32_t len;
            const typename Lay::CView src = skew_run<Lay>(G, (int)r, e.d2, t0, t, len);
            for (uint32_t i = threadIdx.x; i < len; i += SK_THREADS)
                dst[pos + i] = Lay::unpack(P, src[i], e.bucket);
        }
        return;
    }
    const uint32_t d12 = (e.bucket << P.D2) | e.d2;
    uint32_t* gcur = K.ghist + ((size_t)sl * 2 + r) * GS_NB3;
    for (uint32_t t = s; t < nt; t += ts) {
        uint32_t len;
        const typename Lay::CView src = skew_run<Lay>(G, (int)r, e.d2, t0, t, len);
        for (uint32_t c = 0; c < len; c += SK_CHUNK) {
            for (uint32_t d = threadIdx.x; d < GS_NB3; d += SK_THREADS) h[d] = 0;
            W v[SK_ITEMS];
            uint32_t dg[SK_ITEMS];
#pragma unroll
            for (int k = 0; k < SK_ITEMS; k++) {
                const uint32_t i = c + k * SK_THREADS + threadIdx.x;
                v[k] = src[i < len ? i : len - 1];
            }
            __syncthreads();
#pragma unroll
            for (int k = 0; k < SK_ITEMS; k++) {
                const uint32_t i = c + k * SK_THREADS + threadIdx.x;
                dg[k] = i < len ? plan_d3(P, Lay::rel(P, v[k], e.bucket), d12) : 0u;
                if (i < len) atomicAdd(&h[dg[k]], 1u);
            }
            __syncthreads();
            constexpr int RPT = GS_NB3 / SK_THREADS;
            uint32_t res[RPT];
#pragma unroll
            for (int k = 0; k < RPT; k++) {
                const uint32_t d = threadIdx.x + k * SK_THREADS;
                const uint32_t n = h[d];
                res[k] = n ? atomicAdd(&gcur[d], n) : 0u;
            }
#pragma unroll
            for (int k = 0; k < RPT; k++) h[threadIdx.x + k * SK_THREADS] = res[k];
            __syncthreads();
#pragma unroll
            for (int k = 0; k < SK_ITEMS; k++) {
                const bool ok = c + k * SK_THREADS + threadIdx.x < len;
                if (ok) dst[atomicAdd(&h[dg[k]], 1u)] = Lay::unpack(P, v[k], e.bucket);
            }
            __syncthreads();
        }
    }
}

__global__ void __launch_bounds__(SK_THREADS)
k_skew_check(SkewArgs K) {
    const uint4 it = K.items[blockIdx.x];
    const uint32_t qi = it.x, r = it.z >> 16, s = it.z & 0xffffu, ts = it.w;
    const RangePlan& P = K.G.plan;
    if (!(P.s3 == 0 && !(K.gflag[qi] & 1u))) return;
    const OvfEntry e = K.q[qi];
    const Tup* dst = K.G.out[r] + K.G.ostart[r][e.bucket] + e.off[r];
    const uint32_t n = e.nr[r];
    const uint32_t lo = max(1u, (uint32_t)((uint64_t)n * s / ts));
    const uint32_t hi = (uint32_t)((uint64_t)n * (s + 1) / ts);
    if (__syncthreads_or(skew_inversion(dst, lo, hi)) && threadIdx.x == 0)
        atomicOr(&K.gflag[qi], 2u);
}

template <class Lay>
static void skew_path(Workspace* ws, const GroupArgs& G, OvfEntry* ovf, uint32_t no,
                      const uint64_t* hdst, uint32_t nb, hipStream_t st,
                      Workspace::SkewStats& stats) {
    const int nrel = G.nrel;
    OvfEntry* he = (OvfEntry*)ws->host_pinned("sk_he", (size_t)no * sizeof(OvfEntry));
    SMJ_CHECK(hipMemcpyAsync(he, ovf, no * sizeof(OvfEntry), hipMemcpyDeviceToHost, st));
    ws->wait_stream(st);
    std::vector<uint32_t> small, large, lslot;
    std::vector<uint4> items;
    for (uint32_t i = 0; i < no; i++) {
        const uint32_t m = std::max(he[i].nr[0], nrel > 1 ? he[i].nr[1] : 0u);
        if (m == 0) stats.empty++;
        if (m <= kSkewSmall) {
            small.push_back(i);
            continue;
        }
        const uint32_t sl = (uint32_t)large.size();
        large.push_back(i);
        lslot.push_back(sl);
        for (int r = 0; r < nrel; r++) {
            const uint32_t ts =
                std::min<uint32_t>(std::max<uint32_t>(he[i].nr[r] / SMJ_SKEW_ITEM, 1), 256);
            for (uint32_t s = 0; s < ts; s++)
                items.push_back(make_uint4(i, sl, ((uint32_t)r << 16) | s, ts));
        }
    }
    const size_t nl = large.size();
    stats.queued = no;
    stats.small = (uint32_t)small.size();
    stats.large = (uint32_t)nl;
    stats.items = (uint32_t)items.size();
    const size_t lbytes = (small.size() + 2 * nl) * 4;
    const size_t ibytes = items.size() * sizeof(uint4);
    unsigned char* hbuf = (unsigned char*)ws->host_pinned("sk_h", lbytes + ibytes + 16);
    unsigned char* dbuf = (unsigned char*)ws->scratch("sk_d", lbytes + ibytes + 16);
    uint32_t* hl = (uint32_t*)hbuf;
    std::copy(small.begin(), small.end(), hl);
    std::copy(large.begin(), large.end(), hl + small.size());
    std::copy(lslot.begin(), lslot.end(), hl + small.size() + nl);
    const size_t ioff = (lbytes + 15) / 16 * 16;
    std::copy(items.begin(), items.end(), (uint4*)(hbuf + ioff));
    SMJ_CHECK(hipMemcpyAsync(dbuf, hbuf, ioff + ibytes, hipMemcpyHostToDevice, st));
    uint32_t* gflag = (uint32_t*)ws->scratch("sk_flag", (size_t)no * 4);
    SMJ_CHECK(hipMemsetAsync(gflag, 0, (size_t)no * 4, st));
    SkewArgs K;
    K.G = G;
    K.q = ovf;
    K.gflag = gflag;
    K.ghist = nullptr;
    K.slot = nullptr;
    K.items = nullptr;
    if (!small.empty()) {
        K.list = (const uint32_t*)dbuf;
        K.n = (uint32_t)small.size();
        TraceScope ts(ws, "k_skew_small", st);
        hipLaunchKernelGGL(k_skew_small<Lay>, dim3(K.n), dim3(SK_THREADS), 0, st, K);
    }
    if (nl) {
        K.ghist = (uint32_t*)ws->scratch("sk_hist", nl * 2 * GS_NB3 * 4);
        SMJ_CHECK(hipMemsetAsync(K.ghist, 0, nl * 2 * GS_NB3 * 4, st));
        K.list = (const uint32_t*)dbuf + small.size();
        K.slot = K.list + nl;
        K.items = (const uint4*)(dbuf + ioff);
        const uint32_t ni = (uint32_t)items.size();
        {
            TraceScope ts(ws, "k_skew_hist", st);
            hipLaunchKernelGGL(k_skew_hist<Lay>, dim3(ni), dim3(SK_THREADS), 0, st, K);
        }
        hipLaunchKernelGGL(k_skew_scan, dim3((uint32_t)nl), dim3(SK_THREADS), 0, st, K);
        {
            TraceScope ts(ws, "k_skew_place", st);
            hipLaunchKernelGGL(k_skew_place<Lay>, dim3(ni), dim3(SK_THREADS), 0, st, K);
        }
        hipLaunchKernelGGL(k_skew_check, dim3(ni), dim3(SK_THREADS), 0, st, K);
    }
    SMJ_CHECK(hipGetLastError());
    uint32_t* flags = (uint32_t*)ws->host_pinned("sk_flags", (size_t)no * 4);
    SMJ_CHECK(hipMemcpyAsync(flags, gflag, (size_t)no * 4, hipMemcpyDeviceToHost, st));
    SMJ_CHECK(hipMemcpyAsync(he, ovf, no * sizeof(OvfEntry), hipMemcpyDeviceToHost, st));
    ws->wait_stream(st);
    std::vector<uint32_t> rest;
    for (uint32_t i = 0; i < no; i++) {
        if ((flags[i] & 1u) || G.plan.s3 != 0) stats.inexact++;
        if (flags[i] & 2u) stats.unordered++;
        if (flags[i] != 0 || G.plan.s3 != 0) rest.push_back(i);
    }
    stats.resorted = (uint32_t)rest.size();
    if (rest.empty()) return;
    for (int r = 0; r < nrel; r++) {
        std::vector<uint64_t> so, sl;
        for (uint32_t i : rest) {
            so.push_back(hdst[(size_t)r * nb + he[i].bucket] + he[i].off[r]);
            sl.push_back(he[i].nr[r]);
        }
        segmented_sort(ws, G.out[r], so.data(), sl.data(), (uint32_t)rest.size(), st);
    }
    if (nrel == 2) {
        std::vector<const Tup*> rp, sp;
        std::vector<uint64_t> nr, ns;
        for (uint32_t i : rest) {
            if (he[i].counted || !he[i].nr[0] || !he[i].nr[1]) continue;
            rp.push_back(G.out[0] + hdst[he[i].bucket] + he[i].off[0]);
            sp.push_back(G.out[1] + hdst[nb + he[i].bucket] + he[i].off[1]);
            nr.push_back(he[i].nr[0]);
            ns.push_back(he[i].nr[1]);
        }
        stats.recounted = (uint32_t)rp.size();
        merge_join_count_batch(ws, rp.data(), nr.data(), sp.data(), ns.data(),
                               (uint32_t)rp.size(), G.count_dev, st);
    }
}

__global__ void __launch_bounds__(256)
k_plan(const Tup* r0, uint64_t n0, const Tup* r1, uint64_t n1, uint32_t D1,
       uint32_t D2, uint32_t D2cap, int64_t hmin, int64_t hmax, RangePlan* plan) {
    __shared__ int64_t smin[4], smax[4];
    int64_t mn = INT64_MAX, mx = INT64_MIN;
    const int S = 4096;
    for (int rel = 0; rel < 2; rel++) {
        const Tup* p = rel ? r1 : r0;
        uint64_t n = rel ? n1 : n0;
        if (!p || n == 0) continue;
        for (int i = threadIdx.x; i < S; i += 256) {
            uint64_t idx = __umul64hi((uint64_t)i * 0x9E3779B97F4A7C15ull, n);
            if (i == 0) idx = 0;
            if (i == 1) idx = n - 1;
            int64_t k = tup_key(p[idx]);
            mn = k < mn ? k : mn;
            mx = k > mx ? k : mx;
        }
    }
#pragma unroll
    for (int o = 32; o > 0; o >>= 1) {
        int64_t a = __shfl_xor(mn, o, 64), c = __shfl_xor(mx, o, 64);
        mn = a < mn ? a : mn;
        mx = c > mx ? c : mx;
    }
    if (lane_id() == 0) {
        smin[threadIdx.x >> 6] = mn;
        smax[threadIdx.x >> 6] = mx;
    }
    __syncthreads();
    if (threadIdx.x == 0) {
        for (int w = 0; w < 4; w++) {
            mn = smin[w] < mn ? smin[w] : mn;
            mx = smax[w] > mx ? smax[w] : mx;
        }
        int64_t lo, hi;
        if (hmin <= hmax) {
            lo = hmin;
            hi = hmax;
        } else if (mn > mx) {
            lo = 0;
            hi = 0;
        } else {
            uint64_t w = key_u(mx) - key_u(mn);
            uint64_t m = w / 64 + 1;
            uint64_t lu = key_u(mn) > m ? key_u(mn) - m : 0;
            uint64_t hu = (~0ull - key_u(mx)) > m ? key_u(mx) + m : ~0ull;
            lo = (int64_t)(lu ^ 0x8000000000000000ull);
            hi = (int64_t)(hu ^ 0x8000000000000000ull);
        }
        *plan = make_plan(lo, hi, D1, D2, D2cap, GS_D3MAX);
    }
}

void plan_from_sample(Workspace* ws, const Tup* const* rels, const uint64_t* ns,
                      int nrel, uint32_t D1, uint32_t D2, uint32_t D2cap,
                      int64_t hint_min, int64_t hint_max, RangePlan* plan_dev,
                      hipStream_t st) {
    (void)ws;
    hipLaunchKernelGGL(k_plan, dim3(1), dim3(256), 0, st, rels[0], ns[0],
                       nrel > 1 ? rels[1] : (const Tup*)nullptr,
                       nrel > 1 ? ns[1] : 0, D1, D2, D2cap, hint_min, hint_max,
                       plan_dev);
    SMJ_CHECK(hipGetLastError());
}

const uint32_t kGroupD3Max = GS_D3MAX;
const uint32_t kGroupTarget = GS_CAP * 4 / 5 >= 2048 ? 2048 : (GS_CAP * 4 / 5 >= 1024 ? 1024 : 512);

struct SegRel {
    const int64_t* seg_cnt[2];
    const int64_t* bcount[2];
    const uint64_t* bstart[2];
    const uint64_t* seg_start[2];
    uint32_t* ntiles[2];
    uint64_t* ostart[2];
    TileTable tt[2];
};

__global__ void __launch_bounds__(256)
k_seg_scan(SegRel S, uint32_t nb, uint32_t nseg, uint32_t tsz) {
    const int r = blockIdx.x;
    const int64_t* __restrict__ seg_cnt = S.seg_cnt[r];
    const int64_t* __restrict__ bcount = S.bcount[r];
    uint32_t* __restrict__ btile0 = S.tt[r].btile0;
    uint64_t* __restrict__ ostart = S.ostart[r];
    __shared__ unsigned long long scr[5];
    __shared__ unsigned long long base;
    if (threadIdx.x == 0) base = 0;
    __syncthreads();
    for (uint32_t b0 = 0; b0 < nb; b0 += 256) {
        const uint32_t b = b0 + threadIdx.x;
        uint32_t nt = 0;
        uint64_t cnt = 0;
        if (b < nb) {
            for (uint32_t q = 0; q < nseg; q++)
                nt += (uint32_t)((seg_cnt[(size_t)b * nseg + q] + tsz - 1) / tsz);
            cnt = (uint64_t)bcount[b];
        }
        unsigned long long tot;
        const unsigned long long ex =
            block_scan64(((unsigned long long)nt << 40) | cnt, scr, &tot);
        const unsigned long long run = base;
        if (b < nb) {
            btile0[b] = (uint32_t)((run >> 40) + (ex >> 40));
            ostart[b] = (run & ((1ull << 40) - 1)) + (ex & ((1ull << 40) - 1));
        }
        __syncthreads();
        if (threadIdx.x == 0) base = run + tot;
        __syncthreads();
    }
    if (threadIdx.x == 0) {
        btile0[nb] = (uint32_t)(base >> 40);
        *S.ntiles[r] = (uint32_t)(base >> 40);
    }
}

__global__ void __launch_bounds__(64)
k_tiles2(SegRel S, uint32_t nseg, uint32_t tsz) {
    const int r = blockIdx.y;
    const uint32_t b = blockIdx.x;
    const TileTable& tt = S.tt[r];
    uint32_t t0 = tt.btile0[b];
    for (uint32_t q = 0; q < nseg; q++) {
        const uint64_t s0 = S.seg_start[r] ? S.seg_start[r][(size_t)b * nseg + q] : S.bstart[r][b];
        const int64_t cnt = S.seg_cnt[r] ? S.seg_cnt[r][(size_t)b * nseg + q] : S.bcount[r][b];
        const uint32_t nt = (uint32_t)((cnt + tsz - 1) / tsz);
        for (uint32_t i = threadIdx.x; i < nt; i += 64) {
            const uint64_t o = (uint64_t)i * tsz;
            const int64_t rem = cnt - (int64_t)o;
            tt.off[t0 + i] = s0 + o;
            tt.len[t0 + i] = (uint32_t)(rem < (int64_t)tsz ? rem : tsz);
            tt.bucket[t0 + i] = b;
        }
        t0 += nt;
    }
}

static void launch_preft(const TileTable* tt, int nrel, const uint32_t* ub,
                         uint32_t* const* ntiles, uint32_t nb2, hipStream_t st) {
    const uint32_t nb0 = (ub[0] + PT_TILES - 1) / PT_TILES;
    const uint32_t nb1 = nrel > 1 ? (ub[1] + PT_TILES - 1) / PT_TILES : 0;
    if (nb0 + nb1 == 0) return;
    const size_t lds = (size_t)PT_TILES * (nb2 + 1) * 2;
    hipLaunchKernelGGL(k_preft, dim3(nb0 + nb1), dim3(256), lds, st, tt[0],
                       tt[nrel > 1 ? 1 : 0], nb0, ntiles[0], nrel > 1 ? ntiles[1] : nullptr,
                       ub[0], nrel > 1 ? ub[1] : 0u, nb2);
}

static void launch_preft_range(const TilePassArgs& T, int nrel, uint32_t nb2,
                               hipStream_t st) {
    TileTable tt[2];
    uint32_t ub[2] = {0, 0};
    uint32_t* nt[2] = {nullptr, nullptr};
    for (int r = 0; r < 2; r++) {
        tt[r] = T.tt[r];
        if (r < nrel) {
            tt[r].pref += (uint64_t)T.t0[r] * (nb2 + 1);
            tt[r].prefT += T.t0[r];
            ub[r] = T.nt[r];
        }
    }
    launch_preft(tt, nrel, ub, nt, nb2, st);
}

template <class Lay, class LayO>
static void launch_tilepass(const TilePassArgs& T, size_t lds, hipStream_t st) {
    const uint32_t nblk = T.nt[0] + T.nt[1];
    if constexpr (std::is_same<Lay, LayP48>::value) {
        hipLaunchKernelGGL((k_tilepass48<LayO>), dim3(nblk), dim3(TP_THREADS), lds, st, T);
    } else if (SMJ_TP_PERSIST && sizeof(typename Lay::W) >= 12) {
        hipLaunchKernelGGL((k_tilepass_p<Lay, LayO>), dim3(nblk < 256 ? nblk : 256),
                           dim3(TP_THREADS), lds, st, T);
    } else {
        hipLaunchKernelGGL((k_tilepass<Lay, LayO>), dim3(nblk), dim3(TP_THREADS), lds, st, T);
    }
}

template <class Lay>
static size_t tilepass_lds(uint32_t nb2) {
    return (((size_t)tile_elems_l<Lay>() * TileStage<Lay>::kBytes + 15) & ~(size_t)15) +
           (size_t)nb2 * 4 + 128;
}

template <class Lay, class LayO>
static void set_tilepass_attrs() {
    if constexpr (std::is_same<Lay, LayP48>::value) {
        set_lds_attr((const void*)k_tilepass48<LayO>, 160 * 1024);
    } else {
        set_lds_attr((const void*)k_tilepass<Lay, LayO>, 160 * 1024);
        set_lds_attr((const void*)k_tilepass_p<Lay, LayO>, 160 * 1024);
    }
}

template <class Lay>
static void set_pass_attrs() {
    if constexpr (!std::is_same<Lay, LayP40>::value) set_tilepass_attrs<Lay, Lay>();
    const void* gs[4] = {(const void*)k_groupsort<Lay, 2, false>,
                         (const void*)k_groupsort<Lay, 4, false>,
                         (const void*)k_groupsort<Lay, 2, true>,
                         (const void*)k_groupsort<Lay, 4, true>};
    for (const void* f : gs) set_lds_attr(f, (int)sizeof(GroupLDS<typename Lay::W>));
}

static uint64_t expected_tiles(uint64_t nmax, uint32_t nb, uint32_t nseg, uint32_t tsz) {
    const uint64_t per = nmax / (nb ? nb : 1);
    return (per + per / 4) / tsz + nseg + 1;
}
static int group_tpl(uint64_t nmax, uint32_t nb, uint32_t nseg, uint32_t tsz) {
    return expected_tiles(nmax, nb, nseg, tsz) <= 128 ? 2 : 4;
}

static uint32_t groupsort_grid(uint32_t ngroups, uint32_t maxwg, uint32_t& per) {
    per = (ngroups + maxwg - 1) / maxwg;
    const uint32_t nwg = (ngroups + per - 1) / per;
    return (nwg + 7) & ~7u;
}

template <class Lay>
static void launch_groupsort(Workspace* ws, int tpl, uint32_t nwg, hipStream_t st,
                             const GroupArgs& G0) {
    const size_t lds = sizeof(GroupLDS<typename Lay::W>);
#if SMJ_GS_ARGS_MEM
    GroupArgs* G = (GroupArgs*)ws->scratch("gs_args", sizeof(GroupArgs));
    hipLaunchKernelGGL(k_put_args, dim3(1), dim3(1), 0, st, G0, G);
#else
    const GroupArgs& G = G0;
#endif
#if SMJ_GS_XCD
    if (nwg % 8 != 0) {
        fprintf(stderr, "[ERROR] smj: group pass grid %u is not a multiple of 8\n", nwg);
        abort();
    }
#endif
    if (G0.pair) {
        if (tpl == 4)
            hipLaunchKernelGGL((k_groupsort<Lay, 4, true>), dim3(nwg), dim3(GS_THREADS), lds, st, G);
        else
            hipLaunchKernelGGL((k_groupsort<Lay, 2, true>), dim3(nwg), dim3(GS_THREADS), lds, st, G);
    } else {
        if (tpl == 4)
            hipLaunchKernelGGL((k_groupsort<Lay, 4, false>), dim3(nwg), dim3(GS_THREADS), lds, st, G);
        else
            hipLaunchKernelGGL((k_groupsort<Lay, 2, false>), dim3(nwg), dim3(GS_THREADS), lds, st, G);
    }
}

#ifndef SMJ_P40
#define SMJ_P40 1
#endif
template <class Lay, class LayG = Lay>
static bool bucket_sort_nosync(Workspace* ws, const BucketSortArgs& a, hipStream_t st) {
    typedef typename Lay::W W;
    set_pass_attrs<Lay>();
    set_pass_attrs<LayG>();
    constexpr bool p40 = !std::is_same<Lay, LayG>::value;
    if (p40) set_tilepass_attrs<Lay, LayG>();
    const uint32_t nb = a.nbuckets;
    const int nrel = a.nrel;
    const uint32_t nb2 = 1u << a.host_plan->D2;
    const uint64_t nmax = nrel > 1 && a.n[1] > a.n[0] ? a.n[1] : a.n[0];
    const uint32_t tsz = tile_elems_l<Lay>();
    TileTable tt[2];
    static const char* names[2][8] = {
        {"bs_off0", "bs_len0", "bs_bkt0", "bs_bt00", "bs_pref0", "bs_ost0", "bs_nt0", "bs_preft0"},
        {"bs_off1", "bs_len1", "bs_bkt1", "bs_bt01", "bs_pref1", "bs_ost1", "bs_nt1", "bs_preft1"}};
    uint64_t* ostart[2] = {nullptr, nullptr};
    uint32_t* ntiles[2] = {nullptr, nullptr};
    uint32_t ub[2] = {0, 0};
    for (int r = 0; r < nrel; r++) {
        ub[r] = (uint32_t)((a.n[r] + tsz - 1) / tsz + (uint64_t)nb * a.nseg);
        tt[r].off = (uint64_t*)ws->scratch(names[r][0], (size_t)ub[r] * 8);
        tt[r].len = (uint32_t*)ws->scratch(names[r][1], (size_t)ub[r] * 4);
        tt[r].bucket = (uint32_t*)ws->scratch(names[r][2], (size_t)ub[r] * 4);
        tt[r].btile0 = (uint32_t*)ws->scratch(names[r][3], (nb + 1) * 4);
        tt[r].pref = (uint16_t*)ws->scratch(names[r][4], (size_t)ub[r] * (nb2 + 1) * 2);
        tt[r].prefT = (uint16_t*)ws->scratch(names[r][7], (size_t)ub[r] * (nb2 + 1) * 2);
        tt[r].tstride = ub[r];
        ostart[r] = (uint64_t*)ws->scratch(names[r][5], (size_t)nb * 8);
        ntiles[r] = (uint32_t*)ws->scratch(names[r][6], 4);
    }
    if (nrel == 1) tt[1] = tt[0];
    int sel[2] = {0, 0}, ns = 0;
    for (int r = 0; r < nrel; r++)
        if (a.stage & (1u << r)) sel[ns++] = r;
    if (ns) {
        SegRel S;
        for (int i = 0; i < 2; i++) {
            const int rr = sel[i < ns ? i : 0];
            S.seg_cnt[i] = a.seg_cnt[rr];
            S.bcount[i] = a.bcount[rr];
            S.bstart[i] = a.bstart[rr];
            S.seg_start[i] = a.seg_start[rr];
            S.ntiles[i] = ntiles[rr];
            S.ostart[i] = ostart[rr];
            S.tt[i] = tt[rr];
        }
        hipLaunchKernelGGL(k_seg_scan, dim3(ns), dim3(256), 0, st, S, nb, a.nseg, tsz);
        hipLaunchKernelGGL(k_tiles2, dim3(nb, ns), dim3(64), 0, st, S, a.nseg, tsz);
    }
    if (a.ev_tile) SMJ_CHECK(hipEventRecord(a.ev_tile, st));

    const uint32_t ngroups = nb * nb2;
    const uint32_t ovf_cap = ngroups;
    OvfEntry* ovf = (OvfEntry*)ws->scratch("bs_ovf", (size_t)ovf_cap * sizeof(OvfEntry));
    uint32_t* novf = a.status ? a.status + 2 : (uint32_t*)ws->scratch("bs_novf", 4);
    if (!a.status && (a.stage & 4)) SMJ_CHECK(hipMemsetAsync(novf, 0, 4, st));
    TilePassArgs T;
    GroupArgs G;
    for (int i = 0; i < 2; i++) {
        const int rr = sel[i < ns ? i : 0];
        T.part[i] = a.part[rr];
        T.tmp[i] = a.tmp[rr];
        T.pstride[i] = a.pstride[rr];
        T.tt[i] = tt[rr];
        T.t0[i] = 0;
        T.nt[i] = i < ns ? ub[rr] : 0;
        T.ntiles[i] = ntiles[rr];
    }
    uint64_t hoff[2] = {0, 0};
    if (p40) {
        static const char* hn[2] = {"p40_hi0", "p40_hi1"};
        for (int r = 0; r < nrel; r++) {
            const uint8_t* hb = (const uint8_t*)ws->scratch(hn[r], a.pstride[r] ? a.pstride[r] : 1);
            hoff[r] = (uint64_t)((uintptr_t)hb - (uintptr_t)a.tmp[r]);
        }
        for (int i = 0; i < 2; i++) T.ostride[i] = hoff[sel[i < ns ? i : 0]];
    }
    for (int r = 0; r < 2; r++) {
        const int rr = r < nrel ? r : 0;
        G.tmp[r] = a.tmp[rr];
        G.pstride[r] = p40 ? hoff[rr] : a.pstride[rr];
        G.out[r] = a.out[rr];
        G.bstart[r] = a.bstart[rr];
        G.ostart[r] = ostart[rr];
        G.tt[r] = tt[rr];
    }
    T.plan = *a.host_plan;
    T.nb2 = nb2;
    T.pack_bad = a.pack_bad;
    T.d2_fast = a.digit_fast && Lay::fast_ok(T.plan, T.plan.s2, T.plan.D2);
    G.pack_bad = a.pack_bad;
    G.d3_fast = a.digit_fast && Lay::fast_ok(T.plan, T.plan.s3, T.plan.D3);
    G.nrel = nrel;
    G.pair = SMJ_GS_PAIR && nrel == 1;
    G.plan = *a.host_plan;
    G.count_dev = a.count_dev;
    G.nb2 = nb2;
    G.ovf = ovf;
    G.novf = novf;
    G.ovf_cap = ovf_cap;
    G.g_begin = 0;
    G.g_end = ngroups;
    if (ns) {
        {
            TraceScope ts(ws, "k_tilepass", st);
            launch_tilepass<Lay, LayG>(T, tilepass_lds<Lay>(nb2), st);
        }
        const uint32_t ubs[2] = {T.nt[0], T.nt[1]};
        uint32_t* nts[2] = {ntiles[sel[0]], ntiles[sel[ns > 1 ? 1 : 0]]};
        launch_preft(T.tt, ns, ubs, nts, nb2, st);
    }
    if (!(a.stage & 4)) {
        SMJ_CHECK(hipGetLastError());
        return true;
    }
    if (a.ev_bucket) SMJ_CHECK(hipEventRecord(a.ev_bucket, st));
    Workspace::SkewStats stats;
    {
        const uint32_t maxwg =
            (G.pair ? gs_wg_per_cu<W, true>() : gs_wg_per_cu<W, false>()) * 256;
        const uint32_t nwg = groupsort_grid(ngroups, maxwg, G.per);
        TraceScope ts(ws, "k_groupsort", st);
        stats.tpl = (uint32_t)group_tpl(nmax, nb, a.nseg, tsz);
        launch_groupsort<LayG>(ws, (int)stats.tpl, nwg, st, G);
    }
    SMJ_CHECK(hipGetLastError());
    if (a.ev_ovf) SMJ_CHECK(hipEventRecord(a.ev_ovf, st));

    uint32_t* h = (uint32_t*)ws->host_pinned("bs_h_flagovf", 16);
    h[0] = h[1] = h[2] = h[3] = 0;
    if (a.status) {
        SMJ_CHECK(hipMemcpyAsync(h, a.status, 16, hipMemcpyDeviceToHost, st));
    } else {
        SMJ_CHECK(hipMemcpyAsync(h, a.part_flag, 4, hipMemcpyDeviceToHost, st));
        SMJ_CHECK(hipMemcpyAsync(h + 2, novf, 4, hipMemcpyDeviceToHost, st));
        if (a.pack_bad)
            SMJ_CHECK(hipMemcpyAsync(h + 1, a.pack_bad, 4, hipMemcpyDeviceToHost, st));
    }
    ws->wait_stream(st);
    if (a.status_out) {
        a.status_out[0] = h[0];
        a.status_out[1] = h[1];
    }
    if (h[0] || h[1]) return false;
    const uint32_t no = h[2];
    if (no == 0) {
        ws->skew = stats;
        ws->skew_valid = true;
        return true;
    }
    if (no > ovf_cap) {
        fprintf(stderr, "[ERROR] smj: overflow table too small\n");
        abort();
    }
    uint64_t* hdst = (uint64_t*)ws->host_pinned("sk_hdst", (size_t)2 * nb * 8);
    for (int r = 0; r < nrel; r++)
        SMJ_CHECK(hipMemcpyAsync(hdst + (size_t)r * nb, ostart[r], (size_t)nb * 8,
                                 hipMemcpyDeviceToHost, st));
    skew_path<LayG>(ws, G, ovf, no, hdst, nb, st, stats);
    ws->skew = stats;
    ws->skew_valid = true;
    SMJ_CHECK(hipGetLastError());
    return true;
}

template <class K>
static int tilepass_blocks(K kernel, size_t lds) {
    set_lds_attr((const void*)kernel, 160 * 1024);
    int n = 0;
    SMJ_CHECK(hipOccupancyMaxActiveBlocksPerMultiprocessor(&n, kernel, TP_THREADS, lds));
    return n;
}
int tilepass_occupancy(Layout lay, uint32_t d2) {
    if ((lay != Layout::P48 && lay != Layout::P32) || d2 > kMaxD2) return -1;
    const uint32_t nb2 = 1u << d2;
    if (lay == Layout::P32)
        return tilepass_blocks(k_tilepass<LayP32, LayP32>, tilepass_lds<LayP32>(nb2));
    RangePlan P{};
    P.D2 = d2;
    if (SMJ_P40 && sizeof(Tup) == 16 && LayP40::holds(P))
        return tilepass_blocks(k_tilepass48<LayP40>, tilepass_lds<LayP48>(nb2));
    return tilepass_blocks(k_tilepass48<LayP48>, tilepass_lds<LayP48>(nb2));
}

bool bucket_sort(Workspace* ws, const BucketSortArgs& a, hipStream_t st) {
    const uint32_t nb = a.nbuckets;
    const int nrel = a.nrel;
    set_lds_attr((const void*)k_preft, PT_TILES * ((1 << kMaxD2) + 1) * 2);
    set_pass_attrs<LayTup>();
    if (a.host_plan && a.seg_start[0] && a.part_flag) {
        switch (a.layout) {
            case Layout::P32: return bucket_sort_nosync<LayP32>(ws, a, st);
            case Layout::P48:
                return SMJ_P40 && sizeof(Tup) == 16 && LayP40::holds(*a.host_plan)
                    ? bucket_sort_nosync<LayP48, LayP40>(ws, a, st)
                    : bucket_sort_nosync<LayP48>(ws, a, st);
#ifdef KEY_8B
            case Layout::Words: return bucket_sort_nosync<LayPacked>(ws, a, st);
            case Layout::P96: return bucket_sort_nosync<LayP96>(ws, a, st);
#endif
            default: return bucket_sort_nosync<LayTup>(ws, a, st);
        }
    }
    if (a.layout != Layout::Tuples || a.stage != 7) {
        fprintf(stderr, "[ERROR] smj: packed or staged bucket sorts need the host plan\n");
        abort();
    }

    const uint32_t tsz = tile_elems<Tup>();
    uint64_t* hcnt = (uint64_t*)ws->host_pinned("bs_hcnt", (size_t)2 * nb * 8);
    RangePlan* hplan = (RangePlan*)ws->host_pinned("bs_hplan", sizeof(RangePlan));
    const bool segs = a.seg_start[0] != nullptr;
    const uint32_t nseg = segs ? a.nseg : 1;
    int64_t* hseg = (int64_t*)ws->host_pinned("bs_hseg", (size_t)2 * nb * nseg * 8);
    for (int r = 0; r < nrel; r++) {
        SMJ_CHECK(hipMemcpyAsync(hcnt + r * nb, a.bcount[r], nb * 8,
                                 hipMemcpyDeviceToHost, st));
        if (segs)
            SMJ_CHECK(hipMemcpyAsync(hseg + (size_t)r * nb * nseg, a.seg_cnt[r],
                                     (size_t)nb * nseg * 8, hipMemcpyDeviceToHost, st));
    }
    SMJ_CHECK(hipMemcpyAsync(hplan, a.plan_dev, sizeof(RangePlan),
                             hipMemcpyDeviceToHost, st));
    unsigned int* hflag = (unsigned int*)ws->host_pinned("bs_hflag", 4);
    *hflag = 0;
    if (a.part_flag)
        SMJ_CHECK(hipMemcpyAsync(hflag, a.part_flag, 4, hipMemcpyDeviceToHost, st));
    SMJ_CHECK(hipStreamSynchronize(st));
    if (*hflag) return false;
    const uint32_t nb2 = 1u << hplan->D2;

    TileTable tt[2];
    static const char* names[2][6] = {
        {"bs_off0", "bs_len0", "bs_bkt0", "bs_bt00", "bs_pref0", "bs_preft0"},
        {"bs_off1", "bs_len1", "bs_bkt1", "bs_bt01", "bs_pref1", "bs_preft1"}};
    uint32_t* hbt = (uint32_t*)ws->host_pinned("bs_hbt", (size_t)2 * (nb + 1) * 4);
    uint64_t* hdst = (uint64_t*)ws->host_pinned("bs_hdst", (size_t)2 * nb * 8);
    uint64_t* ostart[2] = {nullptr, nullptr};
    for (int r = 0; r < nrel; r++) {
        uint32_t* bt0 = hbt + r * (nb + 1);
        uint32_t acc = 0;
        uint64_t dacc = 0;
        for (uint32_t b = 0; b < nb; b++) {
            hdst[r * nb + b] = dacc;
            dacc += hcnt[r * nb + b];
            bt0[b] = acc;
            if (segs) {
                for (uint32_t q = 0; q < nseg; q++)
                    acc += (uint32_t)((hseg[((size_t)r * nb + b) * nseg + q] + tsz - 1) / tsz);
            } else {
                acc += (uint32_t)((hcnt[r * nb + b] + tsz - 1) / tsz);
            }
        }
        bt0[nb] = acc;
        const uint64_t ntl = acc ? acc : 1;
        tt[r].off = (uint64_t*)ws->scratch(names[r][0], ntl * 8);
        tt[r].len = (uint32_t*)ws->scratch(names[r][1], ntl * 4);
        tt[r].bucket = (uint32_t*)ws->scratch(names[r][2], ntl * 4);
        tt[r].btile0 = (uint32_t*)ws->scratch(names[r][3], (nb + 1) * 4);
        tt[r].pref = (uint16_t*)ws->scratch(names[r][4], ntl * (nb2 + 1) * 2);
        tt[r].prefT = (uint16_t*)ws->scratch(names[r][5], ntl * (nb2 + 1) * 2);
        tt[r].tstride = (uint32_t)ntl;
        SMJ_CHECK(hipMemcpyAsync(tt[r].btile0, bt0, (nb + 1) * 4,
                                 hipMemcpyHostToDevice, st));
        ostart[r] = (uint64_t*)ws->scratch(r ? "bs_ost1" : "bs_ost0", (size_t)nb * 8);
        SMJ_CHECK(hipMemcpyAsync(ostart[r], hdst + r * nb, (size_t)nb * 8,
                                 hipMemcpyHostToDevice, st));
        hipLaunchKernelGGL(k_tiles, dim3(nb), dim3(64), 0, st, a.bstart[r],
                           a.bcount[r], a.seg_start[r], a.seg_cnt[r], nseg, tt[r], tsz);
    }
    if (nrel == 1) tt[1] = tt[0];
    if (a.ev_tile) SMJ_CHECK(hipEventRecord(a.ev_tile, st));

    const uint32_t ngroups = nb * nb2;
    const uint32_t ovf_cap = ngroups;
    OvfEntry* ovf = (OvfEntry*)ws->scratch("bs_ovf", (size_t)ovf_cap * sizeof(OvfEntry));
    uint32_t* novf = (uint32_t*)ws->scratch("bs_novf", 4);
    SMJ_CHECK(hipMemsetAsync(novf, 0, 4, st));
    const size_t tp_lds = (size_t)tsz * sizeof(Tup) + nb2 * 4 + 64;

    TilePassArgs T;
    GroupArgs G;
    for (int r = 0; r < 2; r++) {
        const int rr = r < nrel ? r : 0;
        T.part[r] = a.part[rr];
        T.tt[r] = tt[rr];
        T.t0[r] = 0;
        T.nt[r] = 0;
        T.ntiles[r] = nullptr;
        G.out[r] = a.out[rr];
        G.bstart[r] = a.bstart[rr];
        G.ostart[r] = ostart[rr];
        G.tt[r] = tt[rr];
    }
    T.plan = *hplan;
    T.nb2 = nb2;
    T.pack_bad = nullptr;
    T.d2_fast = a.digit_fast && LayTup::fast_ok(*hplan, hplan->s2, hplan->D2);
    G.pack_bad = nullptr;
    G.d3_fast = a.digit_fast && LayTup::fast_ok(*hplan, hplan->s3, hplan->D3);
    G.nrel = nrel;
    G.pair = SMJ_GS_PAIR && nrel == 1;
    G.plan = *hplan;
    G.count_dev = a.count_dev;
    G.nb2 = nb2;
    G.ovf = ovf;
    G.novf = novf;
    G.ovf_cap = ovf_cap;
    uint32_t ntiles = 0;
    for (int r = 0; r < 2; r++) {
        const int rr = r < nrel ? r : 0;
        T.tmp[r] = a.tmp[rr];
        G.tmp[r] = a.tmp[rr];
        if (r < nrel) {
            T.t0[r] = 0;
            T.nt[r] = hbt[r * (nb + 1) + nb];
            ntiles += T.nt[r];
        }
    }
    if (ntiles) {
        {
            TraceScope ts(ws, "k_tilepass", st);
            launch_tilepass<LayTup, LayTup>(T, tp_lds, st);
        }
        launch_preft_range(T, nrel, nb2, st);
    }
    if (a.ev_bucket) SMJ_CHECK(hipEventRecord(a.ev_bucket, st));
    G.g_begin = 0;
    G.g_end = nb * nb2;
    Workspace::SkewStats stats;
    {
        const uint32_t ng = G.g_end - G.g_begin;
        const uint32_t maxwg = gs_wg_per_cu<Tup>() * 256;
        const uint32_t nwg = groupsort_grid(ng, maxwg, G.per);
        TraceScope ts(ws, "k_groupsort", st);
        const uint64_t nmax = nrel > 1 && a.n[1] > a.n[0] ? a.n[1] : a.n[0];
        stats.tpl = (uint32_t)group_tpl(nmax, nb, nseg, tsz);
        launch_groupsort<LayTup>(ws, (int)stats.tpl, nwg, st, G);
    }
    SMJ_CHECK(hipGetLastError());
    if (a.ev_ovf) SMJ_CHECK(hipEventRecord(a.ev_ovf, st));

    uint32_t* h_novf = (uint32_t*)ws->host_pinned("bs_h_novf", 4);
    SMJ_CHECK(hipMemcpyAsync(h_novf, novf, 4, hipMemcpyDeviceToHost, st));
    ws->wait_stream(st);
    const uint32_t no = *h_novf;
    if (no == 0) {
        ws->skew = stats;
        ws->skew_valid = true;
        return true;
    }
    if (no > ovf_cap) {
        fprintf(stderr, "[ERROR] smj: overflow table too small\n");
        abort();
    }
    skew_path<LayTup>(ws, G, ovf, no, hdst, nb, st, stats);
    ws->skew = stats;
    ws->skew_valid = true;
    SMJ_CHECK(hipGetLastError());
    return true;
}

}
```

avx-sort-merge-joins_amd/csrc/capi.hip:

```cpp
#include <atomic>
#include <math.h>
#include <string.h>
#include <sys/time.h>

#include <algorithm>
#include <vector>

#include "../../include/smj.h"
#include "smj_common.hpp"
#include "smj_internal.hpp"
#include "partition_policy.hpp"

__global__ void k_setplan(smj::RangePlan* p, smj::RangePlan v) { *p = v; }

__global__ void __launch_bounds__(256)
k_join_begin(smj::RangePlan* p, smj::RangePlan v, int set_plan, unsigned long long* count,
             unsigned int* status, unsigned int* zero, uint32_t nzero) {
    if (threadIdx.x == 0) {
        if (set_plan) *p = v;
        *count = 0;
    }
    if (threadIdx.x < 4) status[threadIdx.x] = 0;
    for (uint32_t i = threadIdx.x; i < nzero; i += 256) zero[i] = 0;
}
// ... 18 lines not shown
using namespace smj;

static_assert(sizeof(tuple_t) == sizeof(Tup), "tuple_t / device tuple mismatch");

struct Ctx {
    hipStream_t st = nullptr;
    Workspace ws;
    int device = -1;
};

static Ctx& ctx() {
    thread_local Ctx* c = nullptr;
    if (!c) {
        int ndev = 0;
        if (hipGetDeviceCount(&ndev) != hipSuccess || ndev == 0) {
            fprintf(stderr,
                    "[ERROR] smj: no HIP device visible; the MI355X library has "
                    "no CPU fallback.\n");
            abort();
        }
        c = new Ctx();
        SMJ_CHECK(hipGetDevice(&c->device));
        SMJ_CHECK(hipStreamCreateWithFlags(&c->st, hipStreamNonBlocking));
    }
    return *c;
}


static bool is_device_ptr(const void* p) {
    if (!p) return false;
    hipPointerAttribute_t a;
    hipError_t e = hipPointerGetAttributes(&a, p);
    if (e != hipSuccess) {
        (void)hipGetLastError();
        return false;
    }
    return a.type == hipMemoryTypeDevice || a.type == hipMemoryTypeManaged;
}

struct DevBuf {
    Tup* d = nullptr;
    void* host = nullptr;
    bool staged = false;
};

static DevBuf dev_in(const void* p, uint64_t ntup, const char* slot,
                     bool copy_in) {
    DevBuf b;
    if (is_device_ptr(p)) {
        b.d = (Tup*)p;
        return b;
    }
    Ctx& c = ctx();
    b.d = (Tup*)c.ws.scratch(slot, (ntup ? ntup : 1) * sizeof(Tup));
    b.host = (void*)p;
    b.staged = true;
    if (copy_in && ntup)
        SMJ_CHECK(hipMemcpyAsync(b.d, p, ntup * sizeof(Tup),
                                 hipMemcpyHostToDevice, c.st));
    return b;
}

static void dev_out(const DevBuf& b, uint64_t ntup) {
    if (!b.staged || ntup == 0) return;
    SMJ_CHECK(hipMemcpyAsync(b.host, b.d, ntup * sizeof(Tup),
                             hipMemcpyDeviceToHost, ctx().st));
}

static void sync() { SMJ_CHECK(hipStreamSynchronize(ctx().st)); }

static uint32_t ceil_log2(uint64_t x) {
    uint32_t b = 0;
    while (b < 63 && (1ull << b) < x) b++;
    return b;
}

static void choose_levels(uint64_t n, uint32_t want_d1, uint32_t* D1,
                          uint32_t* D2, uint32_t* D2cap, uint32_t tile = kTileTuples) {
    const uint64_t target = kGroupTarget;
    uint32_t B = n > target ? ceil_log2((n + target - 1) / target) : 0;
    uint32_t d1 = want_d1 ? want_d1 : 8;
    const uint64_t bucket_cap = 192ull * tile;
    while (d1 < kNarrowDigitBits && (n >> d1) > bucket_cap) d1++;
    if (d1 > B) d1 = B;
    if (d1 > kNarrowDigitBits) d1 = kNarrowDigitBits;
    uint32_t d2 = B > d1 ? B - d1 : 0;
    if (d2 > kMaxD2) d2 = kMaxD2;
    *D1 = d1;
    *D2 = d2;
    *D2cap = d2 + 2 < kMaxD2 ? d2 + 2 : (d2 > kMaxD2 ? d2 : kMaxD2);
}

typedef unsigned long long KrVec __attribute__((ext_vector_type(2)));
constexpr int KR_U = 8;
constexpr int KR_THREADS = 512;

__device__ __forceinline__ void kr_acc(uint64_t u, uint64_t& lo, uint64_t& hi) {
    lo = u < lo ? u : lo;
    hi = u > hi ? u : hi;
}

__device__ __forceinline__ void kr_vec(const KrVec& v, uint64_t& lo, uint64_t& hi) {
#ifdef KEY_8B
    kr_acc(key_u((int64_t)v.y), lo, hi);
#else
    kr_acc(key_u(tup_key((Tup)v.x)), lo, hi);
    kr_acc(key_u(tup_key((Tup)v.y)), lo, hi);
#endif
}

__device__ __forceinline__ void kr_chunk(const KrVec* __restrict__ v, uint64_t nv,
                                         uint64_t& lo, uint64_t& hi) {
    const uint64_t per = (nv + gridDim.x - 1) / gridDim.x;
    const uint64_t beg = (uint64_t)blockIdx.x * per;
    const uint64_t end = beg + per < nv ? beg + per : nv;
    constexpr int TILE = KR_THREADS * KR_U;
    KrVec a[KR_U], b[KR_U];
    auto load = [&](KrVec (&x)[KR_U], uint64_t base) {
#pragma unroll
        for (int u = 0; u < KR_U; u++) {
            const uint64_t i = base + (uint64_t)u * KR_THREADS + threadIdx.x;
            x[u] = __builtin_nontemporal_load(v + (i < end ? i : end - 1));
        }
    };
    auto reduce = [&](const KrVec (&x)[KR_U], uint64_t base) {
#pragma unroll
        for (int u = 0; u < KR_U; u++)
            if (base + (uint64_t)u * KR_THREADS + threadIdx.x < end) kr_vec(x[u], lo, hi);
    };
    if (beg >= end) return;
    load(a, beg);
    for (uint64_t base = beg; base < end;) {
        load(b, base + TILE);
        reduce(a, base);
        if ((base += TILE) >= end) break;
        load(a, base + TILE);
        reduce(b, base);
        base += TILE;
    }
}

__global__ void __launch_bounds__(KR_THREADS)
k_keyrange(const Tup* __restrict__ r0, uint64_t n0, const Tup* __restrict__ r1, uint64_t n1,
           unsigned long long* __restrict__ mm) {
    __shared__ unsigned long long sl[KR_THREADS / 64], sh[KR_THREADS / 64];
    uint64_t lo = ~0ull, hi = 0;
    const uint64_t gt = (uint64_t)blockIdx.x * KR_THREADS + threadIdx.x;
    const uint64_t G = (uint64_t)gridDim.x * KR_THREADS;
    for (int rel = 0; rel < 2; rel++) {
        const Tup* p = rel ? r1 : r0;
        const uint64_t n = rel ? n1 : n0;
        if (!p || n == 0) continue;
        if (((uintptr_t)p & 15) == 0) {
            const uint64_t nv = n * sizeof(Tup) / 16;
            kr_chunk(reinterpret_cast<const KrVec*>(p), nv, lo, hi);
            if (gt == 0 && nv * 16 / sizeof(Tup) < n) kr_acc(key_u(tup_key(p[n - 1])), lo, hi);
        } else {
            for (uint64_t i = gt; i < n; i += G) kr_acc(key_u(tup_key(p[i])), lo, hi);
        }
    }
#pragma unroll
    for (int o = 32; o > 0; o >>= 1) {
        const uint64_t a = __shfl_xor(lo, o, 64), c = __shfl_xor(hi, o, 64);
        lo = a < lo ? a : lo;
        hi = c > hi ? c : hi;
    }
    if (lane_id() == 0) {
        sl[threadIdx.x >> 6] = lo;
        sh[threadIdx.x >> 6] = hi;
    }
    __syncthreads();
    if (threadIdx.x == 0) {
        for (int w = 1; w < KR_THREADS / 64; w++) {
            lo = sl[w] < lo ? sl[w] : lo;
            hi = sh[w] > hi ? sh[w] : hi;
        }
        atomicMin(&mm[0], (unsigned long long)lo);
        atomicMax(&mm[1], (unsigned long long)hi);
    }
}

namespace smj {
bool key_range(Workspace* ws, const Tup* const* rels, const uint64_t* ns, int nrel,
               int64_t* lo, int64_t* hi, hipStream_t st) {
    unsigned long long* mm = (unsigned long long*)ws->scratch("keyrange", 16);
    unsigned long long* h = (unsigned long long*)ws->host_pinned("keyrange_h", 16);
    const unsigned long long init[2] = {~0ull, 0ull};
    SMJ_CHECK(hipMemcpyAsync(mm, init, 16, hipMemcpyHostToDevice, st));
    const uint64_t n = ns[0] + (nrel > 1 ? ns[1] : 0);
    uint64_t g = (n * sizeof(Tup) / 16 + KR_THREADS * KR_U - 1) / (KR_THREADS * KR_U);
    if (g > 256) g = 256;
    if (g == 0) g = 1;
    hipLaunchKernelGGL(k_keyrange, dim3((uint32_t)g), dim3(KR_THREADS), 0, st, rels[0], ns[0],
                       nrel > 1 ? rels[1] : (const Tup*)nullptr, nrel > 1 ? ns[1] : 0, mm);
    SMJ_CHECK(hipMemcpyAsync(h, mm, 16, hipMemcpyDeviceToHost, st));
    SMJ_CHECK(hipStreamSynchronize(st));
    if (h[0] > h[1]) return false;
    *lo = (int64_t)(h[0] ^ 0x8000000000000000ull);
    *hi = (int64_t)(h[1] ^ 0x8000000000000000ull);
    return true;
}
}

static LayoutCaps layout_caps(const Workspace* ws, const RangePlan& hplan, uint32_t nb,
                              bool sampled, bool plan_on_host, bool p48_fits) {
    const uint32_t off = ws->layouts_off;
    const bool words = sampled && plan_on_host && !(off & SMJ_LAYOUT_NO_PACKED);
    LayoutCaps c;
    c.sampled = sampled;
    c.plan_on_host = plan_on_host;
    c.p48_fits = p48_fits;
    c.p32_usable = words && !(off & SMJ_LAYOUT_NO_P32) && LayP32::usable(hplan);
#ifdef KEY_8B
    c.can_pack = words && LayPacked::usable(hplan);
    c.p48_ok = c.can_pack && !(off & SMJ_LAYOUT_NO_P48) && nb <= 512;
    c.p96_ok = sampled && plan_on_host && !(off & SMJ_LAYOUT_NO_P96) && LayP96::usable(hplan) &&
               nb <= (LayP96::Pack::kStoreBytes < 8 ? 512u : 1024u);
#else
    c.can_pack = false;
    c.p48_ok = words && !(off & SMJ_LAYOUT_NO_P48) && LayP48::usable(hplan) && nb <= 512;
    c.p96_ok = false;
#endif
    return c;
}

static void device_bucket(Workspace* ws, const Tup* const* rels, const uint64_t* ns,
                          int nrel, Tup* const* outs, uint32_t fanout_bits,
                          int64_t hint_min, int64_t hint_max, uint64_t size_guess,
                          unsigned long long* count_dev, hipStream_t st) {
    static const char* nm[2][6] = {{"bk_part0", "bk_st0", "bk_h0", "bk_sgs0", "bk_sgc0", ""},
                                   {"bk_part1", "bk_st1", "bk_h1", "bk_sgs1", "bk_sgc1", ""}};
    ws->events();
    SMJ_CHECK(hipEventRecord(ws->ev[0], st));
    const uint64_t nmax = nrel > 1 && ns[1] > ns[0] ? ns[1] : ns[0];
    uint32_t D1, D2, D2cap;
    choose_levels(nmax, fanout_bits, &D1, &D2, &D2cap);
    RangePlan* plan = (RangePlan*)ws->scratch("plan", sizeof(RangePlan));
    uint32_t nb = 1u << D1;
    const bool sampled = !(ws->layouts_off & SMJ_LAYOUT_NO_SAMPLED) && D1 <= 10;
    bool plan_on_host = hint_min <= hint_max;
    bool guessed = false;
    const bool sample_plan = (ws->layouts_off & SMJ_LAYOUT_SAMPLE_PLAN) != 0;
    if (!plan_on_host && size_guess > 0 && sampled && !sample_plan) {
        hint_min = 1;
        hint_max = (int64_t)(size_guess < (uint64_t)INT64_MAX ? size_guess : INT64_MAX);
        plan_on_host = guessed = true;
    }
    if (!plan_on_host && !sample_plan)
        plan_on_host = key_range(ws, rels, ns, nrel, &hint_min, &hint_max, st);
    RangePlan hplan = make_plan(hint_min, hint_max, D1, D2, D2cap, kGroupD3Max);
    if (!plan_on_host)
        plan_from_sample(ws, rels, ns, nrel, D1, D2, D2cap, hint_min, hint_max, plan, st);
    Tup* part[2] = {nullptr, nullptr};
    uint64_t* bst[2] = {nullptr, nullptr};
    int64_t* bh[2] = {nullptr, nullptr};
    uint64_t* sgs[2] = {nullptr, nullptr};
    int64_t* sgc[2] = {nullptr, nullptr};
    unsigned int* sample = nullptr;
    auto alloc = [&]() {
        for (int r = 0; r < nrel; r++) {
            const uint64_t cap = sampled ? sampled_capacity(ns[r], D1) : (ns[r] ? ns[r] : 1);
            part[r] = (Tup*)ws->scratch(nm[r][0], cap * sizeof(Tup));
            bst[r] = (uint64_t*)ws->scratch(nm[r][1], nb * 8);
            bh[r] = (int64_t*)ws->scratch(nm[r][2], nb * 8);
            sgs[r] = (uint64_t*)ws->scratch(nm[r][3], (size_t)nb * kShards * 8);
            sgc[r] = (int64_t*)ws->scratch(nm[r][4], (size_t)nb * kShards * 8);
        }
        sample = (unsigned int*)ws->scratch("sp_sample", (size_t)nrel * nb * 4);
    };
    alloc();
    unsigned int* status = (unsigned int*)ws->scratch("join_status", 16);
    bool tuple_levels = sizeof(Tup) != 16;
    auto tuple_plan = [&]() {
        if (tuple_levels) return;
        tuple_levels = true;
        uint32_t d1, d2, d2c;
        choose_levels(nmax, fanout_bits, &d1, &d2, &d2c, kTileTuples / 2);
        if (d1 == D1 || (sampled && d1 > 10)) return;
        D1 = d1;
        D2 = d2;
        D2cap = d2c;
        nb = 1u << D1;
        hplan = make_plan(hint_min, hint_max, D1, D2, D2cap, kGroupD3Max);
        if (!plan_on_host)
            plan_from_sample(ws, rels, ns, nrel, D1, D2, D2cap, hint_min, hint_max, plan, st);
        alloc();
    };
    unsigned long long* cnt = count_dev
        ? count_dev : (unsigned long long*)ws->scratch("sort_cnt", 8);
    const bool p48_fits = hplan.s1 >= 1 && hplan.s1 <= 32 && hplan.span < (1ull << (48 - hplan.s1));
    const uint64_t shape = ((uint64_t)nrel << 62) ^ ns[0] ^ (nrel > 1 ? ns[1] << 31 : 0);
    ShapeHint& H = ws->hint_for(shape);
    auto caps_now = [&]() { return layout_caps(ws, hplan, nb, sampled, plan_on_host, p48_fits); };
    bool started_hinted = false, rehinted = false;
    Rung rung = first_rung(caps_now(), H, &started_hinted);
    Rung payload_fb = Rung::P32;
    Layout lay = Layout::Tuples;
    for (;;) {
        if (rung >= Rung::Sampled) tuple_plan();
        const LayoutCaps caps = caps_now();
        lay = layout_of(rung, caps.p96_ok);
        const bool exact = rung == Rung::Exact;
        const bool planes = lay == Layout::P48 || lay == Layout::P96;
        const bool check = lay != Layout::Tuples || (guessed && rung == Rung::Sampled);
        unsigned int* bad = check ? status + 1 : nullptr;
        hipLaunchKernelGGL(k_join_begin, dim3(1), dim3(256), 0, st, plan, hplan,
                           plan_on_host ? 1 : 0, cnt, status, sample,
                           exact ? 0u : (uint32_t)nrel * nb);
        uint64_t pstride[2] = {0, 0};
        for (int r = 0; r < nrel && planes; r++)
            pstride[r] = (sampled_capacity(ns[r], D1) + 31) & ~31ull;
        if (exact) {
            for (int r = 0; r < nrel; r++)
                plan_partition(ws, rels[r], ns[r], part[r], plan, D1, bst[r], bh[r], st);
        } else if (planes && nrel > 1 && pstride[0] != pstride[1]) {
            for (int r = 0; r < nrel; r++) {
                void* out1 = part[r];
                sampled_partition(ws, 1, rels + r, ns + r, &out1, plan, D1,
                                  sample + (size_t)r * nb, bst + r, bh + r, sgs + r, sgc + r,
                                  status, st, lay, &hplan, bad, pstride[r]);
            }
        } else {
            void* outs_v[2] = {part[0], part[nrel > 1 ? 1 : 0]};
            sampled_partition(ws, nrel, rels, ns, outs_v, plan, D1, sample, bst, bh, sgs, sgc,
                              status, st, lay, plan_on_host ? &hplan : nullptr, bad, pstride[0]);
        }
        SMJ_CHECK(hipEventRecord(ws->ev[1], st));
        BucketSortArgs a;
        for (int r = 0; r < 2; r++) {
            a.part[r] = part[r];
            a.bstart[r] = bst[r];
            a.bcount[r] = bh[r];
            a.tmp[r] = part[r];
            a.out[r] = r < nrel ? outs[r] : nullptr;
            a.n[r] = r < nrel ? ns[r] : 0;
            if (!exact) {
                a.seg_start[r] = sgs[r];
                a.seg_cnt[r] = sgc[r];
            }
            a.pstride[r] = pstride[r];
        }
        a.nrel = nrel;
        a.nbuckets = nb;
        a.plan_dev = plan;
        a.count_dev = nrel == 2 ? count_dev : nullptr;
        a.ev_tile = nullptr;
        a.ev_bucket = ws->ev[2];
        a.ev_ovf = ws->ev[3];
        a.host_plan = plan_on_host ? &hplan : nullptr;
        a.layout = lay;
        a.pack_bad = bad;
        a.status = status;
        if (!exact) a.part_flag = status;
        uint32_t why[2] = {0, 0};
        a.status_out = why;
        if (bucket_sort(ws, a, st)) break;
        const Next next = after_void(rung, caps, why, guessed, H, &payload_fb);
        if (next.what == Next::Stop) break;
        rung = next.rung;
        if (next.what == Next::Restart) {
            guessed = false;
            plan_on_host = key_range(ws, rels, ns, nrel, &hint_min, &hint_max, st);
            hplan = make_plan(hint_min, hint_max, D1, D2, D2cap, kGroupD3Max);
            if (!plan_on_host)
                plan_from_sample(ws, rels, ns, nrel, D1, D2, D2cap, hint_min, hint_max, plan,
                                 st);
            rung = first_rung(caps_now(), H, &rehinted);
        }
    }
    static_assert((int)Layout::Tuples == SMJ_LAYOUT_USED_TUPLES &&
                  (int)Layout::Words == SMJ_LAYOUT_USED_WORDS &&
                  (int)Layout::P48 == SMJ_LAYOUT_USED_P48 &&
                  (int)Layout::P32 == SMJ_LAYOUT_USED_P32 &&
                  (int)Layout::P96 == SMJ_LAYOUT_USED_P96, "smj.h / layout_policy.hpp");
    ws->last_layout = (int)lay;
    end_hint(H, payload_fb, started_hinted);
    SMJ_CHECK(hipEventRecord(ws->ev[4], st));
}

static void device_sort(Workspace* ws, const Tup* in, uint64_t n, Tup* out,
                        hipStream_t st) {
    if (n == 0) return;
    const Tup* rels[1] = {in};
    uint64_t ns[1] = {n};
    const uintptr_t a = (uintptr_t)in, b = (uintptr_t)out, len = (uintptr_t)n * sizeof(Tup);
    const bool overlap = a < b + len && b < a + len;
    Tup* outs[1] = {overlap ? (Tup*)ws->scratch("sort_inplace", n * sizeof(Tup)) : out};
    device_bucket(ws, rels, ns, 1, outs, 0, 1, 0, n, nullptr, st);
    if (overlap)
        SMJ_CHECK(hipMemcpyAsync(out, outs[0], n * sizeof(Tup), hipMemcpyDeviceToDevice, st));
}

static void device_join(Workspace* ws, const Tup* R, uint64_t nR, const Tup* S,
                        uint64_t nS, Tup* sortedR, Tup* sortedS,
                        uint32_t fanout_bits, int64_t hint_min,
                        int64_t hint_max, unsigned long long* count_dev,
                        hipStream_t st, uint64_t size_guess = 0) {
    const Tup* rels[2] = {R, S};
    uint64_t ns[2] = {nR, nS};
    Tup* outs[2] = {sortedR, sortedS};
    device_bucket(ws, rels, ns, 2, outs, fanout_bits, hint_min, hint_max, size_guess,
                  count_dev, st);
}

static void partition_common(relation_t** parts, relation_t* input,
                             relation_t* output, uint32_t nbits,
                             uint32_t shiftbits, int padded) {
    Ctx& c = ctx();
    const uint64_t n = input->num_tuples;
    const uint32_t fan = 1u << nbits;
    const uint32_t mask = (uint32_t)(((1ull << nbits) - 1) << shiftbits);
    DevBuf in = dev_in(input->tuples, n, "api_in", true);
    const uint64_t cap = n + (padded ? (uint64_t)fan * TUPLESPERCACHELINE : 0);
    DevBuf out = dev_in(output->tuples, cap, "api_out", false);
    int64_t* hist = (int64_t*)c.ws.scratch("api_hist", fan * 8);
    int64_t* off = (int64_t*)c.ws.scratch("api_off", fan * 8);
    Digit32 dig{mask, shiftbits};
    stable_partition(&c.ws, in.d, n, out.d, dig, nbits, padded, hist, off, c.st);
    std::vector<int64_t> hh(fan), ho(fan);
    SMJ_CHECK(hipMemcpyAsync(hh.data(), hist, fan * 8, hipMemcpyDeviceToHost, c.st));
    SMJ_CHECK(hipMemcpyAsync(ho.data(), off, fan * 8, hipMemcpyDeviceToHost, c.st));
    sync();
    const uint64_t extent = fan ? (uint64_t)(ho[fan - 1] + hh[fan - 1]) : 0;
    std::vector<tuple_t> gaps;
    if (out.staged && padded) {
        for (uint32_t i = 0; i + 1 < fan; i++)
            for (int64_t j = ho[i] + hh[i]; j < ho[i + 1]; j++)
                gaps.push_back(output->tuples[j]);
    }
    dev_out(out, extent);
    sync();
    if (!gaps.empty()) {
        size_t k = 0;
        for (uint32_t i = 0; i + 1 < fan; i++)
            for (int64_t j = ho[i] + hh[i]; j < ho[i + 1]; j++)
                output->tuples[j] = gaps[k++];
    }
    for (uint32_t i = 0; i < fan; i++) {
        parts[i]->tuples = output->tuples + ho[i];
        parts[i]->num_tuples = (uint64_t)hh[i];
    }
}

extern "C" {

void partition_relation(relation_t** partitions, relation_t* input,
                        relation_t* output, int radixbits, int shiftbits) {
    partition_common(partitions, input, output, (uint32_t)radixbits,
                     (uint32_t)shiftbits, 0);
}

void partition_relation_optimized(relation_t** partitions, relation_t* input,
                                  relation_t* output, uint32_t nbits,
                                  uint32_t shiftbits) {
    partition_common(partitions, input, output, nbits, shiftbits, 1);
}

void partition_relation_optimized_V2(relation_t** partitions,
                                     relation_t* input, relation_t* output,
                                     uint32_t nbits, uint32_t shiftbits) {
    partition_common(partitions, input, output, nbits, shiftbits, 1);
}

void histogram_memcpy_bench(relation_t** partitions, relation_t* input,
                            relation_t* output, uint32_t nbits) {
    (void)partitions;
    Ctx& c = ctx();
    const uint64_t n = input->num_tuples;
    DevBuf in = dev_in(input->tuples, n, "api_in", true);
    DevBuf out = dev_in(output->tuples, n, "api_out", false);
    hist_memcpy(&c.ws, in.d, n, out.d, nbits, c.st);
    dev_out(out, n);
    sync();
}

void radix_cluster(relation_t* outRel, relation_t* inRel, int32_t* hist, int R, int D) {
    Ctx& c = ctx();
    const uint64_t n = inRel->num_tuples;
    const uint32_t fan = 1u << D;
    const uint32_t mask = (uint32_t)((((1ull << D) - 1) << R) & 0xffffffffull);
    DevBuf in = dev_in(inRel->tuples, n, "api_in", true);
    bool zero = true;
    for (uint32_t i = 0; i < fan; i++) zero = zero && hist[i] == 0;
    int64_t* dh = (int64_t*)c.ws.scratch("api_hist", fan * 8);
    int64_t* doff = (int64_t*)c.ws.scratch("api_off", fan * 8);
    const Digit32 dig{mask, (uint32_t)R};
    std::vector<int64_t> hh(fan), ho(fan);
    if (zero) {
        DevBuf out = dev_in(outRel->tuples, n, "api_out", false);
        stable_partition(&c.ws, in.d, n, out.d, dig, (uint32_t)D, 0, dh, doff, c.st);
        SMJ_CHECK(hipMemcpyAsync(hh.data(), dh, fan * 8, hipMemcpyDeviceToHost, c.st));
        dev_out(out, n);
        sync();
    } else {
        Tup* tmp = (Tup*)c.ws.scratch("api_rc", (n ? n : 1) * sizeof(Tup));
        stable_partition(&c.ws, in.d, n, tmp, dig, (uint32_t)D, 0, dh, doff, c.st);
        SMJ_CHECK(hipMemcpyAsync(hh.data(), dh, fan * 8, hipMemcpyDeviceToHost, c.st));
        SMJ_CHECK(hipMemcpyAsync(ho.data(), doff, fan * 8, hipMemcpyDeviceToHost, c.st));
        sync();
        const bool dev = is_device_ptr(outRel->tuples);
        uint32_t dst = 0;
        for (uint32_t i = 0; i < fan; i++) {
            if (hh[i])
                SMJ_CHECK(hipMemcpyAsync(outRel->tuples + dst, tmp + ho[i],
                                         (size_t)hh[i] * sizeof(Tup),
                                         dev ? hipMemcpyDeviceToDevice : hipMemcpyDeviceToHost,
                                         c.st));
            dst += (uint32_t)(hist[i] + (int32_t)hh[i]);
        }
        sync();
    }
    for (uint32_t i = 0; i < fan; i++) hist[i] += (int32_t)hh[i];
}

static void sort_tuples_into(const void* inp, void* outp, uint64_t n) {
    Ctx& c = ctx();
    DevBuf in = dev_in(inp, n, "api_in", true);
    DevBuf out = dev_in(outp, n, "api_out", false);
    device_sort(&c.ws, in.d, n, out.d, c.st);
    dev_out(out, n);
    sync();
}

void avxsort_tuples(tuple_t** inputptr, tuple_t** outputptr, uint64_t nitems) {
    if (nitems == 0) return;
    sort_tuples_into(*inputptr, *outputptr, nitems);
}

void avxsortmultiway_tuples(tuple_t** inputptr, tuple_t** outputptr,
                            uint64_t nitems) {
    if (nitems == 0) return;
    sort_tuples_into(*inputptr, *outputptr, nitems);
}

void scalarsort_tuples(tuple_t** inputptr, tuple_t** outputptr,
                       uint64_t nitems) {
    tuple_t* in = *inputptr;
    tuple_t* out = *outputptr;
    if (nitems) sort_tuples_into(in, in, nitems);
    *inputptr = out;
    *outputptr = in;
}
}

__device__ __forceinline__ int64_t fp64_ord(int64_t x) {
    return x ^ ((x >> 63) & INT64_MAX);
}
__global__ void k_fp64_ord(const int64_t* __restrict__ a, int64_t* __restrict__ b,
                           uint64_t n) {
    const uint64_t s = (uint64_t)gridDim.x * blockDim.x;
    for (uint64_t i = (uint64_t)blockIdx.x * blockDim.x + threadIdx.x; i < n; i += s)
        b[i] = fp64_ord(a[i]);
}

__global__ void k_expand_i64(const int64_t* __restrict__ a, Tup* __restrict__ t,
                             uint64_t n, bool fp64) {
    const uint64_t s = (uint64_t)gridDim.x * blockDim.x;
    for (uint64_t i = (uint64_t)blockIdx.x * blockDim.x + threadIdx.x; i < n; i += s) {
#ifdef KEY_8B
        Tup x;
        x.key = fp64 ? fp64_ord(a[i]) : a[i];
        x.payload = 0;
        t[i] = x;
#else
        t[i] = (uint64_t)(fp64 ? fp64_ord(a[i]) : a[i]);
#endif
    }
}
__global__ void k_compact_i64(const Tup* __restrict__ t, int64_t* __restrict__ a,
                              uint64_t n, bool fp64) {
    const uint64_t s = (uint64_t)gridDim.x * blockDim.x;
    for (uint64_t i = (uint64_t)blockIdx.x * blockDim.x + threadIdx.x; i < n; i += s) {
#ifdef KEY_8B
        a[i] = fp64 ? fp64_ord(t[i].key) : t[i].key;
#else
        a[i] = fp64 ? fp64_ord((int64_t)t[i]) : (int64_t)t[i];
#endif
    }
}
__global__ void k_expand_i32(const int32_t* __restrict__ a, Tup* __restrict__ t,
                             uint64_t n) {
    const uint64_t s = (uint64_t)gridDim.x * blockDim.x;
    for (uint64_t i = (uint64_t)blockIdx.x * blockDim.x + threadIdx.x; i < n; i += s) {
#ifdef KEY_8B
        Tup x;
        x.key = a[i];
        x.payload = 0;
        t[i] = x;
#else
        t[i] = (uint64_t)(uint32_t)a[i] << 32;
#endif
    }
}
__global__ void k_compact_i32(const Tup* __restrict__ t, int32_t* __restrict__ a,
                              uint64_t n) {
    const uint64_t s = (uint64_t)gridDim.x * blockDim.x;
    for (uint64_t i = (uint64_t)blockIdx.x * blockDim.x + threadIdx.x; i < n; i += s)
        a[i] = (int32_t)tup_key(t[i]);
}

static uint32_t grid_n(uint64_t n) {
    uint64_t b = (n + 255) / 256;
    return (uint32_t)(b < 4096 ? (b ? b : 1) : 4096);
}

__device__ __forceinline__ bool fp64_lt_bits(uint64_t a, uint64_t b) {
    const uint64_t ma = a & 0x7fffffffffffffffull, mb = b & 0x7fffffffffffffffull;
    if (ma > 0x7ff0000000000000ull || mb > 0x7ff0000000000000ull) return false;
    if ((ma | mb) == 0) return false;
    const int64_t ka = (int64_t)a < 0 ? -(int64_t)ma : (int64_t)ma;
    const int64_t kb = (int64_t)b < 0 ? -(int64_t)mb : (int64_t)mb;
    return ka < kb;
}

__global__ void __launch_bounds__(256)
k_inreg4x4(const uint64_t* __restrict__ in, uint64_t* __restrict__ out, uint64_t nblocks) {
    const uint64_t i = (uint64_t)blockIdx.x * 256 + threadIdx.x;
    if (i >= nblocks * 4) return;
    const uint64_t b = i >> 2;
    const uint32_t j = (uint32_t)(i & 3);
    const uint64_t* x = in + 16 * b;
    auto mn = [](uint64_t p, uint64_t q) { return fp64_lt_bits(p, q) ? p : q; };
    auto mx = [](uint64_t p, uint64_t q) { return fp64_lt_bits(q, p) ? p : q; };
    const uint64_t a = x[j], bb = x[4 + j], c = x[8 + j], d = x[12 + j];
    const uint64_t a1 = mn(a, bb), b1 = mx(a, bb), c1 = mn(c, d), d1 = mx(c, d);
    const uint64_t b2 = mn(b1, d1), d2 = mx(b1, d1);
    const uint64_t a2 = mn(a1, c1), c2 = mx(a1, c1);
    const uint64_t b3 = mn(b2, c2), c3 = mx(b2, c2);
    uint64_t* o = out + 16 * b + 4 * j;
    o[0] = a2;
    o[1] = b3;
    o[2] = c3;
    o[3] = d2;
}

static void sort_int64_into(const int64_t* inp, int64_t* outp, uint64_t n, bool fp64) {
    if (n == 0) return;
    Ctx& c = ctx();
    const bool din = is_device_ptr(inp), dout = is_device_ptr(outp);
#ifndef KEY_8B
    if (!fp64) {
// ... 1438 lines not shown
```

avx-sort-merge-joins_amd/csrc/partition.hip:

```cpp
#include <stdlib.h>
#include <string.h>

#include "smj_common.hpp"
#include "smj_internal.hpp"
#include "partition_policy.hpp"

namespace smj {

template <int THREADS, int ITEMS, class Digit>
__global__ void __launch_bounds__(THREADS)
k_hist(const Tup* __restrict__ in, uint64_t n, uint64_t chunk, Digit dig_arg,
       uint32_t nbins, uint32_t* __restrict__ counts, uint32_t nwg) {
    const auto dig = dig_arg.load();
    constexpr int TILE = THREADS * ITEMS;
    extern __shared__ __attribute__((aligned(16))) uint32_t lds_hist[];
    for (uint32_t d = threadIdx.x; d < nbins; d += THREADS) lds_hist[d] = 0;
    __syncthreads();
    const uint64_t beg = (uint64_t)blockIdx.x * chunk;
    uint64_t end = beg + chunk;
    if (end > n) end = n;
    for (uint64_t base = beg; base < end; base += TILE) {
        Tup v[ITEMS];
#pragma unroll
        for (int j = 0; j < ITEMS; j++) {
// ... 1521 lines not shown
    if (ntiles == 0) ntiles = 1;
    uint32_t nwg = (uint32_t)(ntiles < 256 ? ntiles : 256);
    const uint64_t tiles_per_wg = (ntiles + nwg - 1) / nwg;
    const uint64_t chunk = tiles_per_wg * G::TILE;
    nwg = (uint32_t)((ntiles + tiles_per_wg - 1) / tiles_per_wg);
    uint32_t* counts = (uint32_t*)ws->scratch("pt_counts", (size_t)nbins * nwg * 4);
    uint64_t* totals = (uint64_t*)ws->scratch("pt_totals", (size_t)nbins * 8);
    {
        TraceScope ts(ws, "k_hist", st);
        bool vec = false;
        if constexpr (sizeof(Tup) == 8) {
            vec = ((uintptr_t)in & 15) == 0 && (chunk & 1) == 0;
            if (vec)
                hipLaunchKernelGGL((k_hist_v<512, 8, Digit>), dim3(nwg), dim3(512),
                                   nbins * sizeof(uint32_t), st, in, n, chunk, dig, nbins,
                                   counts, nwg);
        }
        if (!vec)
            hipLaunchKernelGGL((k_hist_p<512, 16, Digit, true>), dim3(nwg), dim3(512),
                               nbins * sizeof(uint32_t), st, in, n, chunk, dig, nbins, counts,
                               nwg);
    }
    {
        TraceScope ts(ws, "k_scan", st);
        hipLaunchKernelGGL(k_scanrow, dim3(nbins), dim3(256), 0, st, counts, nwg, totals);
        hipLaunchKernelGGL(k_scandig, dim3(1), dim3(256), 0, st, totals, nbins, padded,
                           starts_dev, hist_out, off_out);
    }
    if (n == 0) return;
    ws->last_scatter |= scatter_bit(Scatter::Atomic);
    set_lds_attr((const void*)k_scatter_swp<THREADS, ITEMS, Digit, true>, 160 * 1024);
    TraceScope ts(ws, "k_scatter", st);
    hipLaunchKernelGGL((k_scatter_swp<THREADS, ITEMS, Digit, true>), dim3(nwg), dim3(THREADS),
                       G::lds_bytes(nbins), st, in, n, chunk, dig, nbins, counts, nwg,
                       starts_dev, out, 1);
    SMJ_CHECK(hipGetLastError());
}

template <class Digit>
static void stable_partition_narrow(Workspace* ws, const Tup* in, uint64_t n,
                                    Tup* out, const Digit& dig, uint32_t dbits,
                                    int padded, uint64_t* starts_dev,
                                    int64_t* hist_out, int64_t* off_out,
                                    hipStream_t st) {
    const bool forced = ws->force_ballot_ranks;
    Scatter which = stable_scatter_choice(n, dbits, sizeof(Tup), true, forced, SMJ_SWP_SEG);
    if (which == Scatter::Atomic && !lds_order_ok(ws, st))
        which = stable_scatter_choice(n, dbits, sizeof(Tup), false, forced, SMJ_SWP_SEG);
    if (which == Scatter::Atomic)
        stable_partition_swp(ws, in, n, out, dig, dbits, padded, starts_dev, hist_out,
                             off_out, st);
    else if (which != Scatter::Ballot256x8)
        partition_hist_scatter<512, 16, true>(ws, in, n, out, dig, dbits, padded,
                                              starts_dev, hist_out, off_out, st);
    else
        partition_hist_scatter<256, 8, true>(ws, in, n, out, dig, dbits, padded,
                                             starts_dev, hist_out, off_out, st);
}

template <class Digit>
static void unstable_partition(Workspace* ws, const Tup* in, uint64_t n,
                               Tup* out, const Digit& dig, uint32_t dbits,
                               uint64_t* starts_dev, int64_t* hist_out,
                               hipStream_t st) {
    if (dbits <= 10)
        partition_hist_scatter<512, 16, false>(ws, in, n, out, dig, dbits, 0, starts_dev,
                                               hist_out, nullptr, st);
    else
        partition_hist_scatter<256, 8, false>(ws, in, n, out, dig, dbits, 0, starts_dev,
                                              hist_out, nullptr, st);
}

void stable_partition(Workspace* ws, const Tup* in, uint64_t n, Tup* out,
                      const Digit32& dig, uint32_t dbits, int padded,
                      int64_t* hist_out, int64_t* off_out, hipStream_t st) {
    const uint32_t nbins = 1u << dbits;
    ws->last_scatter = dbits <= kNarrowDigitBits ? 0u : kScatterTwoPass;
    if (dbits <= kNarrowDigitBits) {
        uint64_t* starts = (uint64_t*)ws->scratch("pt_starts", (size_t)nbins * 8);
        stable_partition_narrow(ws, in, n, out, dig, dbits, padded, starts,
                                hist_out, off_out, st);
        return;
    }
    const uint32_t lowb = dbits / 2, highb = dbits - lowb;
    Tup* t1 = (Tup*)ws->scratch("pt_wide1", (n ? n : 1) * sizeof(Tup));
    Tup* t2 = (Tup*)ws->scratch("pt_wide2", (n ? n : 1) * sizeof(Tup));
    uint64_t* st1 = (uint64_t*)ws->scratch("pt_wst1", (1u << lowb) * 8);
    uint64_t* st2 = (uint64_t*)ws->scratch("pt_wst2", (1u << highb) * 8);
    LowBits lo{dig, lowb};
    HighBits hi{dig, lowb};
    stable_partition_narrow(ws, in, n, t1, lo, lowb, 0, st1, nullptr, nullptr, st);
    stable_partition_narrow(ws, t1, n, t2, hi, highb, 0, st2, nullptr, nullptr, st);
    unsigned long long* h = (unsigned long long*)ws->scratch("pt_whist", (size_t)nbins * 8);
    SMJ_CHECK(hipMemsetAsync(h, 0, (size_t)nbins * 8, st));
    if (n) hipLaunchKernelGGL(k_hist_global<Digit32>, dim3(1024), dim3(256), 0,
                              st, in, n, dig, h);
    uint64_t* ust = (uint64_t*)ws->scratch("pt_wust", (size_t)nbins * 8);
    uint64_t* pst = (uint64_t*)ws->scratch("pt_wpst", (size_t)nbins * 8);
    hipLaunchKernelGGL(k_scandig, dim3(1), dim3(256), 0, st,
                       (const uint64_t*)h, nbins, 0, ust, nullptr, nullptr);
    hipLaunchKernelGGL(k_scandig, dim3(1), dim3(256), 0, st,
                       (const uint64_t*)h, nbins, padded, pst, hist_out, off_out);
    if (n) hipLaunchKernelGGL(k_padcopy<Digit32>, dim3(2048), dim3(256), 0, st,
                              t2, n, dig, ust, pst, out);
    SMJ_CHECK(hipGetLastError());
}

void plan_partition(Workspace* ws, const Tup* in, uint64_t n, Tup* out,
                    const RangePlan* plan_dev, uint32_t dbits,
                    uint64_t* starts_dev, int64_t* hist_out, hipStream_t st) {
    PlanDigit1 dig{plan_dev};
    const uint32_t nbins = 1u << dbits;
    constexpr int THREADS = 512;
    constexpr int ITEMS = sizeof(Tup) == 16 ? 8 : 16;
    constexpr int TILE = THREADS * ITEMS;
    const size_t lds = scatter_wc_lds<THREADS, ITEMS>(nbins);
    if (sizeof(Tup) != 16 || dbits > 10 || lds > 160 * 1024) {
        unstable_partition(ws, in, n, out, dig, dbits, starts_dev, hist_out, st);
        return;
    }
    uint64_t ntiles = (n + TILE - 1) / TILE;
    if (ntiles == 0) ntiles = 1;
    const uint32_t maxwg = 256;
    uint32_t nwg = (uint32_t)(ntiles < maxwg ? ntiles : maxwg);
    const uint64_t tiles_per_wg = (ntiles + nwg - 1) / nwg;
    const uint64_t chunk = tiles_per_wg * TILE;
    nwg = (uint32_t)((ntiles + tiles_per_wg - 1) / tiles_per_wg);
    uint32_t* counts = (uint32_t*)ws->scratch("pt_counts", (size_t)nbins * nwg * 4);
    uint64_t* totals = (uint64_t*)ws->scratch("pt_totals", (size_t)nbins * 8);
    {
        TraceScope ts(ws, "k_hist", st);
        hipLaunchKernelGGL((k_hist<1024, 8, PlanDigit1>), dim3(nwg), dim3(1024),
                           nbins * sizeof(uint32_t), st, in, n, chunk, dig, nbins,
                           counts, nwg);
    }
    {
        TraceScope ts(ws, "k_scan", st);
        hipLaunchKernelGGL(k_scanrow, dim3(nbins), dim3(256), 0, st, counts, nwg,
                           totals);
        hipLaunchKernelGGL(k_scandig, dim3(1), dim3(256), 0, st, totals, nbins, 0,
                           starts_dev, hist_out, (int64_t*)nullptr);
    }
    if (n == 0) return;
    set_lds_attr((const void*)k_scatter_wc<THREADS, ITEMS, PlanDigit1>, 160 * 1024);
    TraceScope ts(ws, "k_scatter", st);
    hipLaunchKernelGGL((k_scatter_wc<THREADS, ITEMS, PlanDigit1>), dim3(nwg),
                       dim3(THREADS), lds, st, in, n, chunk, dig, nbins, counts,
                       nwg, starts_dev, out);
    SMJ_CHECK(hipGetLastError());
}

#ifdef KEY_8B
void plan_partition_packed(Workspace* ws, const Tup* in, uint64_t n, uint64_t* out,
                           const RangePlan* plan_dev, const RangePlan& pack_plan,
                           uint32_t dbits, uint64_t* starts_dev, int64_t* hist_out,
                           unsigned int* pack_bad, hipStream_t st) {
    PlanDigit1 dig{plan_dev};
    LayPacked::Pack pk;
    pk.bu = key_u(pack_plan.base);
    pk.span = pack_plan.span;
    pk.s1 = pack_plan.s1;
    if (dbits > 10)
        partition_hist_scatter<256, 8, false, PlanDigit1, LayPacked::Pack>(
            ws, in, n, out, dig, dbits, 0, starts_dev, hist_out, nullptr, st, pk, pack_bad);
    else
        partition_hist_scatter<512, 16, false, PlanDigit1, LayPacked::Pack>(
            ws, in, n, out, dig, dbits, 0, starts_dev, hist_out, nullptr, st, pk, pack_bad);
}
#endif

#ifndef SMJ_SC_THREADS
#define SMJ_SC_THREADS 1024
#endif
#ifndef SMJ_SC_ITEMS16
#define SMJ_SC_ITEMS16 4
#endif
#ifndef SMJ_SC_ITEMS16Q
#define SMJ_SC_ITEMS16Q 6
#endif
#ifndef SMJ_SC_ITEMS16P
#define SMJ_SC_ITEMS16P 8
#endif
#ifndef SMJ_SC_ITEMS8
#define SMJ_SC_ITEMS8 12
#endif
#ifndef SMJ_SC_ITEMS8W
#define SMJ_SC_ITEMS8W 16
#endif
#ifndef SMJ_SC_WG_PER_CU
#define SMJ_SC_WG_PER_CU 1
#endif
#ifndef SMJ_SAMPLE_STRIDE
#define SMJ_SAMPLE_STRIDE 128
#endif
static constexpr uint32_t kSampleStride = SMJ_SAMPLE_STRIDE;
#ifndef SMJ_SAMPLE_WG
#define SMJ_SAMPLE_WG 128
#endif
static constexpr uint32_t kSampleWg = SMJ_SAMPLE_WG;
static constexpr uint64_t kRegionSlack = 1024;

uint64_t sampled_capacity(uint64_t n, uint32_t dbits) {
    const uint64_t ALIGN = kRegionAlign / 4;
    return n + n / 8 + 5 * kSampleStride + 1 +
           ((uint64_t)1 << dbits) * kShards * (kRegionSlack + ALIGN);
}

static uint64_t scatter_chunk(uint64_t n, uint64_t tile, uint32_t* nwg_out) {
    const uint64_t ntiles = (n + tile - 1) / tile;
    const uint32_t maxwg = 256 * SMJ_SC_WG_PER_CU;
    uint32_t nwg = (uint32_t)(ntiles < maxwg ? ntiles : maxwg);
    const uint64_t tiles_per_wg = (ntiles + nwg - 1) / nwg;
    *nwg_out = (uint32_t)((ntiles + tiles_per_wg - 1) / tiles_per_wg);
    return tiles_per_wg * tile;
}

template <class Pack>
static int sampled_items(uint32_t nbins) {
    constexpr int THREADS = SMJ_SC_THREADS;
    constexpr int BIG = sizeof(Tup) == 16
        ? (sizeof(typename Pack::OutT) <= 8    ? SMJ_SC_ITEMS16P
           : sizeof(typename Pack::OutT) <= 12 ? SMJ_SC_ITEMS16Q
                                               : SMJ_SC_ITEMS16)
        : (sizeof(typename Pack::OutT) <= 4 ? SMJ_SC_ITEMS8W : SMJ_SC_ITEMS8);
    constexpr int SMALL = sizeof(Tup) == 16 ? 4 : 8;
    typedef typename Pack::OutT O;
    if (ScatterGeom<THREADS, BIG, O, Pack::kStoreBytes>::lds_bytes(nbins) <= 160 * 1024) return BIG;
    if (ScatterGeom<THREADS, SMALL, O, Pack::kStoreBytes>::lds_bytes(nbins) <= 160 * 1024)
        return SMALL;
    return 0;
}

template <int ITEMS, class Pack>
static bool sampled_scatter_t(Workspace* ws, const Tup* in, uint64_t n, void* out,
                              uint64_t ostride, const PlanDigit1& dig, uint32_t nbins,
                              unsigned long long* cursor, const uint64_t* cap_end,
                              const Pack& pk, unsigned int* bad_flag, hipStream_t st) {
    constexpr int THREADS = SMJ_SC_THREADS;
    constexpr int TILE = THREADS * ITEMS;
    const size_t lds = ScatterGeom<THREADS, ITEMS, typename Pack::OutT,
                                   Pack::kStoreBytes>::lds_bytes(nbins);
    if (lds > 160 * 1024) return false;
    uint32_t nwg = 0;
    const uint64_t chunk = scatter_chunk(n, TILE, &nwg);
    constexpr bool VEC_OK = sizeof(Tup) == 8 && ITEMS % 2 == 0;
    set_lds_attr((const void*)k_scatter_res<THREADS, ITEMS, PlanDigit1, Pack, false>, 160 * 1024);
    if constexpr (VEC_OK)
        set_lds_attr((const void*)k_scatter_res<THREADS, ITEMS, PlanDigit1, Pack, true>,
                     160 * 1024);
    TraceScope ts(ws, "k_scatter", st);
    bool vec = false;
    if constexpr (VEC_OK) {
        vec = n % 2 == 0 && chunk % 2 == 0 && ((uintptr_t)in & 15) == 0;
        if (vec)
            hipLaunchKernelGGL((k_scatter_res<THREADS, ITEMS, PlanDigit1, Pack, true>), dim3(nwg),
                               dim3(THREADS), lds, st, in, n, chunk, dig, nbins, cursor,
                               cap_end, out, ostride, pk, bad_flag);
    }
    if (!vec)
        hipLaunchKernelGGL((k_scatter_res<THREADS, ITEMS, PlanDigit1, Pack, false>), dim3(nwg),
                           dim3(THREADS), lds, st, in, n, chunk, dig, nbins, cursor,
                           cap_end, out, ostride, pk, bad_flag);
    return true;
}

template <class Pack>
static void sampled_scatter(Workspace* ws, const Tup* in, uint64_t n, void* out,
                            uint64_t ostride, const PlanDigit1& dig, uint32_t nbins,
                            unsigned long long* cursor, const uint64_t* cap_end,
                            const Pack& pk, unsigned int* bad_flag, hipStream_t st) {
    constexpr int THREADS = SMJ_SC_THREADS;
    if (nbins > (uint32_t)THREADS) {
        fprintf(stderr, "[ERROR] smj: sampled scatter needs <= %d partitions\n", THREADS);
        abort();
    }
    constexpr int BIG = sizeof(Tup) == 16
        ? (sizeof(typename Pack::OutT) <= 8    ? SMJ_SC_ITEMS16P
           : sizeof(typename Pack::OutT) <= 12 ? SMJ_SC_ITEMS16Q
                                               : SMJ_SC_ITEMS16)
        : (sizeof(typename Pack::OutT) <= 4 ? SMJ_SC_ITEMS8W : SMJ_SC_ITEMS8);
    constexpr int SMALL = sizeof(Tup) == 16 ? 4 : 8;
    const int items = sampled_items<Pack>(nbins);
    if (items == BIG && sampled_scatter_t<BIG>(ws, in, n, out, ostride, dig, nbins, cursor,
                                               cap_end, pk, bad_flag, st))
        return;
    if (items == SMALL && sampled_scatter_t<SMALL>(ws, in, n, out, ostride, dig, nbins,
                                                   cursor, cap_end, pk, bad_flag, st))
        return;
    fprintf(stderr, "[ERROR] smj: sampled scatter LDS exceeds 160 KiB (%u partitions)\n", nbins);
    abort();
}

template <class Pack>
static auto set_s1(Pack& pk, const RangePlan& p, int) -> decltype((void)pk.s1) { pk.s1 = p.s1; }
template <class Pack>
static void set_s1(Pack&, const RangePlan&, long) {}

void sampled_partition(Workspace* ws, int nrel, const Tup* const* in, const uint64_t* n,
                       void* const* out, const RangePlan* plan_dev, uint32_t dbits,
                       unsigned int* sample, uint64_t* const* starts_dev,
                       int64_t* const* hist_out, uint64_t* const* seg_start,
                       int64_t* const* seg_cnt, unsigned int* flag_dev, hipStream_t st,
                       Layout lay, const RangePlan* host_plan, unsigned int* bad,
                       uint64_t pstride, bool exact) {
    PlanDigit1 dig{plan_dev};
    const uint32_t nbins = 1u << dbits;
    if (lay == Layout::P96 && (sizeof(Tup) != 16 || !host_plan || !pstride)) {
        fprintf(stderr, "[ERROR] smj: the 96-bit layout needs 16-byte tuples, the host plan "
                        "and a plane stride\n");
        abort();
    }
    if (exact && lay != Layout::Tuples && lay != Layout::Words) {
        fprintf(stderr, "[ERROR] smj: exact shard regions take tuples or 64-bit words\n");
        abort();
    }
    if (lay == Layout::Words && sizeof(Tup) != 16) {
        fprintf(stderr, "[ERROR] smj: packed words are a 16-byte-tuple layout\n");
        abort();
    }
    if (lay == Layout::P48 && !pstride) {
        fprintf(stderr, "[ERROR] smj: the 48-bit layout needs a plane stride\n");
        abort();
    }
    if (lay != Layout::Tuples && !host_plan) {
        fprintf(stderr, "[ERROR] smj: packed partition needs the host plan\n");
        abort();
    }
    static const char* cn[2] = {"sp_cursor0", "sp_cursor1"};
    static const char* en[2] = {"sp_capend0", "sp_capend1"};
    SampleRel S;
    RegionRel R;
    uint64_t nmax = 0;
    for (int r = 0; r < 2; r++) {
        const int rr = r < nrel ? r : 0;
        S.in[r] = in[rr];
        S.n[r] = n[rr];
        S.hist[r] = sample + (size_t)rr * nbins * (exact ? kShards : 1);
        R.sample[r] = S.hist[r];
        R.base[r] = starts_dev[rr];
        R.seg_start[r] = seg_start[rr];
        R.hist_out[r] = hist_out[rr];
        R.seg_cnt[r] = seg_cnt[rr];
        if (r < nrel) {
            R.cursor[r] = (unsigned long long*)ws->scratch(cn[r], (size_t)nbins * kShards * 8);
            R.cap_end[r] = (uint64_t*)ws->scratch(en[r], (size_t)nbins * kShards * 8);
            nmax = n[r] > nmax ? n[r] : nmax;
        } else {
            R.cursor[r] = R.cursor[0];
            R.cap_end[r] = R.cap_end[0];
        }
    }
    if (exact) {
        TraceScope ts(ws, "k_hist", st);
        for (int r = 0; r < nrel; r++) {
            if (!n[r]) continue;
            int items = sampled_items<PackRange>(nbins);
#ifdef KEY_8B
            if (lay == Layout::Words) items = sampled_items<LayPacked::Pack>(nbins);
#endif
            if (!items) {
                fprintf(stderr, "[ERROR] smj: sampled scatter LDS exceeds 160 KiB (%u "
                        "partitions)\n", nbins);
                abort();
            }
            uint32_t nwg = 0;
            const uint64_t chunk = scatter_chunk(n[r], (uint64_t)SMJ_SC_THREADS * items, &nwg);
            constexpr int HI = sizeof(Tup) == 16 ? 8 : 16;
            const uint32_t split = 4;
            hipLaunchKernelGGL((k_shard_hist<1024, HI, PlanDigit1>), dim3(nwg * split),
                               dim3(1024), nbins * sizeof(unsigned int), st, in[r], n[r], chunk,
                               split, dig, nbins, S.hist[r]);
        }
        hipLaunchKernelGGL(k_regions_exact, dim3(nrel), dim3(1024), 0, st, R, nbins);
    } else {
        TraceScope ts(ws, "k_sample", st);
        const uint64_t npts = (nmax + 4 * kSampleStride - 1) / (4 * kSampleStride);
        uint32_t g = (uint32_t)((npts + 255) / 256);
        if (g > kSampleWg) g = kSampleWg;
        if (g == 0) g = 1;
        hipLaunchKernelGGL((k_sample_hist<PlanDigit1>), dim3(g, nrel), dim3(256),
                           nbins * sizeof(unsigned int), st, S, kSampleStride, dig, nbins);
        hipLaunchKernelGGL(k_regions, dim3(nrel), dim3(256), 0, st, R, nbins, kSampleStride,
                           kRegionSlack,
                           lay == Layout::P96 ? (uint32_t)SMJ_P96_SEGB
                           : lay == Layout::P48 || lay == Layout::P32 ? 4u
                           : lay == Layout::Words ? 8u : (uint32_t)sizeof(Tup));
    }
    for (int r = 0; r < nrel; r++) {
        if (!n[r]) continue;
        if (lay != Layout::Tuples) {
            const auto go = [&](auto pk, uint64_t ostride) {
                pk.bu = key_u(host_plan->base);
                pk.span = host_plan->span;
                set_s1(pk, *host_plan, 0);
                sampled_scatter(ws, in[r], n[r], out[r], ostride, dig, nbins, R.cursor[r],
                                R.cap_end[r], pk, bad, st);
            };
            if (lay == Layout::P32) go(LayP32::Pack(), 0);
            else if (lay == Layout::P48) go(LayP48::Pack(), pstride);
#ifdef KEY_8B
            else if (lay == Layout::P96) go(LayP96::Pack(), pstride);
            else go(LayPacked::Pack(), 0);
#endif
            continue;
        }
        PackRange pk{0ull, ~0ull};
        if (bad && host_plan) {
            pk.bu = key_u(host_plan->base);
            pk.span = host_plan->span;
        }
        sampled_scatter(ws, in[r], n[r], out[r], 0, dig, nbins, R.cursor[r], R.cap_end[r], pk,
                        bad && host_plan ? bad : (unsigned int*)nullptr, st);
    }
    hipLaunchKernelGGL(k_regions_done, dim3(nrel), dim3(256), 0, st, R, nbins, flag_dev);
    SMJ_CHECK(hipGetLastError());
}

__global__ void __launch_bounds__(1024)
k_lds_order(uint32_t K, uint32_t iters, unsigned long long* bad) {
    __shared__ uint32_t ctr[16][64];
    const int lane = lane_id(), wid = threadIdx.x >> 6;
    ctr[wid][lane] = 0;
    __syncthreads();
    const uint64_t lt = lanemask_lt();
    unsigned long long nb = 0;
    uint32_t h = blockIdx.x * 7919u + threadIdx.x * 104729u + K;
    for (uint32_t it = 0; it < iters; it++) {
        h = h * 1664525u + 1013904223u;
        const uint32_t d = (h >> 8) % K;
        uint64_t peers = ~0ull;
        for (int b = 0; b < 6; b++) {
            const bool bit = (d >> b) & 1u;
            const uint64_t bal = __ballot(bit);
            peers &= bit ? bal : ~bal;
        }
        const uint32_t snap = ctr[wid][d];
        __builtin_amdgcn_wave_barrier();
        const uint32_t old = atomicAdd(&ctr[wid][d], 1u);
        __builtin_amdgcn_wave_barrier();
        nb += old != snap + (uint32_t)__popcll(peers & lt);
    }
    if (nb) atomicAdd(bad, nb);
}

uint64_t lds_order_selfcheck(Workspace* ws, hipStream_t st) {
    unsigned long long* bad = (unsigned long long*)ws->scratch("lds_order_bad", 8);
    SMJ_CHECK(hipMemsetAsync(bad, 0, 8, st));
    for (uint32_t K : {1u, 2u, 5u, 16u, 64u})
        hipLaunchKernelGGL(k_lds_order, dim3(512), dim3(1024), 0, st, K, 256u, bad);
    SMJ_CHECK(hipGetLastError());
    unsigned long long* h = (unsigned long long*)ws->host_pinned("lds_order_h", 8);
    SMJ_CHECK(hipMemcpyAsync(h, bad, 8, hipMemcpyDeviceToHost, st));
    SMJ_CHECK(hipStreamSynchronize(st));
    return *h;
}

void hist_memcpy(Workspace* ws, const Tup* in, uint64_t n, Tup* out,
                 uint32_t dbits, hipStream_t st) {
    constexpr int THREADS = 256, ITEMS = 8, TILE = THREADS * ITEMS;
    const uint32_t nbins = 1u << dbits;
    uint64_t ntiles = (n + TILE - 1) / TILE;
    if (ntiles == 0) ntiles = 1;
    uint32_t nwg = (uint32_t)(ntiles < 2048 ? ntiles : 2048);
    const uint64_t tiles_per_wg = (ntiles + nwg - 1) / nwg;
    const uint64_t chunk = tiles_per_wg * TILE;
    nwg = (uint32_t)((ntiles + tiles_per_wg - 1) / tiles_per_wg);
    uint32_t* counts = (uint32_t*)ws->scratch("pt_counts", (size_t)nbins * nwg * 4);
    Digit32 dig{nbins - 1u, 0u};
    if (dbits > kNarrowDigitBits) {
        unsigned long long* h = (unsigned long long*)ws->scratch("pt_whist", (size_t)nbins * 8);
        SMJ_CHECK(hipMemsetAsync(h, 0, (size_t)nbins * 8, st));
        if (n) hipLaunchKernelGGL(k_hist_global<Digit32>, dim3(1024), dim3(256), 0, st, in, n, dig, h);
    } else {
        hipLaunchKernelGGL((k_hist<THREADS, ITEMS, Digit32>), dim3(nwg), dim3(THREADS),
                           nbins * sizeof(uint32_t), st, in, n, chunk, dig, nbins,
                           counts, nwg);
    }
    if (n) SMJ_CHECK(hipMemcpyAsync(out, in, n * sizeof(Tup),
                                    hipMemcpyDeviceToDevice, st));
}

}
```

avx-sort-merge-joins_amd/csrc/smj_internal.hpp:

```cpp
#pragma once
#include <sched.h>

#include <chrono>
#include <map>
#include <mutex>
#include <string>
#include <vector>

#include <hip/hip_ext.h>

#include "smj_common.hpp"

namespace smj {

constexpr uint32_t kNarrowDigitBits = 12;
constexpr uint32_t kMaxD2 = 10;

typedef RefDigit Digit32;

__device__ __forceinline__ uint32_t uniform32(uint32_t x) {
    return __builtin_amdgcn_readfirstlane(x);
}
__device__ __forceinline__ uint64_t uniform64(uint64_t x) {
    return ((uint64_t)__builtin_amdgcn_readfirstlane((uint32_t)(x >> 32)) << 32) |
           __builtin_amdgcn_readfirstlane((uint32_t)x);
}

struct PlanDigitV {
    RangePlan p;
    __device__ __forceinline__ uint32_t operator()(const Tup& t) const {
        return plan_d1(p, plan_rel(p, tup_key(t)));
    }
};

struct PlanDigit1 {
    const RangePlan* plan;
    __device__ __forceinline__ PlanDigitV load() const {
        RangePlan q = *plan;
        PlanDigitV v;
        v.p.base = (int64_t)uniform64((uint64_t)q.base);
        v.p.span = uniform64(q.span);
        v.p.D1 = uniform32(q.D1);
        v.p.D2 = uniform32(q.D2);
        v.p.D3 = uniform32(q.D3);
        v.p.s1 = uniform32(q.s1);
        v.p.s2 = uniform32(q.s2);
        v.p.s3 = uniform32(q.s3);
        return v;
    }
};

#ifndef SMJ_SPIN_WAIT
#define SMJ_SPIN_WAIT 1
#endif
struct Workspace {
    uint32_t layouts_off = 0;
    ShapeHint hints[8];
    uint64_t hint_clock = 0;
    ShapeHint& hint_for(uint64_t shape) {
        ShapeHint* victim = &hints[0];
        for (ShapeHint& h : hints) {
            if (h.shape == shape) {
                h.used = ++hint_clock;
                return h;
            }
            if (h.used < victim->used) victim = &h;
        }
        *victim = ShapeHint();
        victim->shape = shape;
        victim->used = ++hint_clock;
        return *victim;
    }
    int last_layout = -1;
    bool force_ballot_ranks = false;
    uint32_t last_scatter = 0;
    struct SkewStats {
        uint32_t tpl = 0, queued = 0, empty = 0, small = 0, large = 0, items = 0, inexact = 0,
                 unordered = 0, resorted = 0, recounted = 0;
    };
    SkewStats skew;
    bool skew_valid = false;
    std::map<std::string, std::pair<void*, size_t>> bufs;
    std::map<std::string, std::pair<void*, size_t>> pinned;
    std::vector<unsigned char> km_last;
    const void* km_last_dev = nullptr;
    hipEvent_t ev[8] = {};
    bool ev_init = false;
    float phase_ms[5] = {0, 0, 0, 0, 0};

    void* scratch(const char* name, size_t bytes) {
        if (bytes == 0) bytes = 16;
        auto it = bufs.find(name);
        if (it != bufs.end() && it->second.second >= bytes)
            return it->second.first;
        if (it != bufs.end()) SMJ_CHECK(hipFree(it->second.first));
        void* p = nullptr;
        size_t cap = bytes + bytes / 8;
        SMJ_CHECK(hipMalloc(&p, cap));
        bufs[name] = {p, cap};
        return p;
    }
    void* host_pinned(const char* name, size_t bytes) {
        if (bytes == 0) bytes = 16;
        auto it = pinned.find(name);
        if (it != pinned.end() && it->second.second >= bytes)
            return it->second.first;
        if (it != pinned.end()) SMJ_CHECK(hipHostFree(it->second.first));
        void* p = nullptr;
        SMJ_CHECK(hipHostMalloc(&p, bytes, hipHostMallocDefault));
        pinned[name] = {p, bytes};
        return p;
    }
    static constexpr uint32_t kNRing = 8;
    struct RingSlot {
        void* p = nullptr;
        size_t cap = 0;
        hipEvent_t ev = nullptr;
        bool used = false;
    };
    std::map<std::string, std::pair<std::vector<RingSlot>, uint32_t>> rings;
    void* ring_acquire(const char* name, size_t bytes, uint32_t* slot) {
        auto& r = rings[name];
        if (r.first.empty()) r.first.resize(kNRing);
        const uint32_t i = r.second++ % kNRing;
        RingSlot& s = r.first[i];
        if (s.used) SMJ_CHECK(hipEventSynchronize(s.ev));
        if (s.cap < bytes) {
            if (s.p) SMJ_CHECK(hipHostFree(s.p));
            SMJ_CHECK(hipHostMalloc(&s.p, bytes ? bytes : 16, hipHostMallocDefault));
            s.cap = bytes;
        }
        if (!s.ev) SMJ_CHECK(hipEventCreateWithFlags(&s.ev, hipEventDisableTiming));
        *slot = i;
        return s.p;
    }
    void ring_release(const char* name, uint32_t slot, hipStream_t st) {
        RingSlot& s = rings[name].first[slot];
        SMJ_CHECK(hipEventRecord(s.ev, st));
        s.used = true;
    }
    hipEvent_t wait_ev = nullptr;
    void wait_stream(hipStream_t st) {
#if SMJ_SPIN_WAIT
        if (!wait_ev) SMJ_CHECK(hipEventCreateWithFlags(&wait_ev, hipEventDisableTiming));
        SMJ_CHECK(hipEventRecord(wait_ev, st));
        hipError_t e;
        const auto t0 = std::chrono::steady_clock::now();
        while ((e = hipEventQuery(wait_ev)) == hipErrorNotReady) {
            const auto dt = std::chrono::steady_clock::now() - t0;
            if (dt > std::chrono::microseconds(200)) {
                e = hipEventSynchronize(wait_ev);
                break;
            }
            if (dt > std::chrono::microseconds(50)) sched_yield();
        }
        SMJ_CHECK(e);
#else
        SMJ_CHECK(hipStreamSynchronize(st));
#endif
    }
    void events() {
        if (!ev_init) {
            for (auto& e : ev) SMJ_CHECK(hipEventCreate(&e));
            ev_init = true;
        }
    }

    struct TraceRec {
        const char* name;
        hipEvent_t a, b;
    };
    bool trace_on = false;
    std::string trace_only;
    std::vector<TraceRec> trace;
    size_t trace_n = 0;
    bool traced(const char* name) const {
        return trace_on && (trace_only.empty() || trace_only == name);
    }
    int trace_begin(const char* name, hipStream_t st) {
        if (!traced(name)) return -1;
        if (trace_n == trace.size()) {
            TraceRec r;
            SMJ_CHECK(hipEventCreate(&r.a));
            SMJ_CHECK(hipEventCreate(&r.b));
            trace.push_back(r);
        }
        trace[trace_n].name = name;
        SMJ_CHECK(hipEventRecord(trace[trace_n].a, st));
        return (int)trace_n++;
    }
    void trace_end(int idx, hipStream_t st) {
        if (idx >= 0) SMJ_CHECK(hipEventRecord(trace[idx].b, st));
    }
    bool trace_ext(const char* name, hipEvent_t* a, hipEvent_t* b) {
        if (!traced(name)) return false;
        if (trace_n == trace.size()) {
            TraceRec r;
            SMJ_CHECK(hipEventCreate(&r.a));
            SMJ_CHECK(hipEventCreate(&r.b));
            trace.push_back(r);
        }
        trace[trace_n].name = name;
        *a = trace[trace_n].a;
        *b = trace[trace_n].b;
        trace_n++;
        return true;
    }

    ~Workspace() {
        for (auto& r : trace) {
            (void)hipEventDestroy(r.a);
            (void)hipEventDestroy(r.b);
        }
        for (auto& kv : bufs) (void)hipFree(kv.second.first);
        for (auto& kv : pinned) (void)hipHostFree(kv.second.first);
        if (ev_init)
            for (auto& e : ev) (void)hipEventDestroy(e);
    }
};

struct TraceScope {
    Workspace* ws;
    hipStream_t st;
    int idx;
    TraceScope(Workspace* w, const char* name, hipStream_t s)
        : ws(w), st(s), idx(w ? w->trace_begin(name, s) : -1) {}
    ~TraceScope() {
        if (ws) ws->trace_end(idx, st);
    }
};

template <typename... KArgs, typename... Args>
inline void traced_launch(Workspace* ws, const char* name, void (*kernel)(KArgs...),
                          dim3 grid, dim3 block, uint32_t shmem, hipStream_t st,
                          Args... args) {
    hipEvent_t a, b;
    if (ws && ws->trace_ext(name, &a, &b))
        hipExtLaunchKernelGGL(kernel, grid, block, shmem, st, a, b, 0u, (KArgs)args...);
    else
        hipLaunchKernelGGL(kernel, grid, block, shmem, st, (KArgs)args...);
}

uint32_t glibc_rand_at(uint32_t seed, uint64_t k);
void gen_nonunique_ref(Workspace* ws, Tup* out, uint64_t n, uint64_t first, uint64_t total,
                       int64_t maxid, uint32_t seed, uint64_t skip, hipStream_t st);
void gen_zipf_ref(Workspace* ws, Tup* out, uint64_t n, uint64_t first, uint64_t maxid,
                  double theta, uint32_t seed, uint64_t skip, hipStream_t st);

void xsend(const int64_t* start, const int64_t* cnt, const unsigned int* flags, uint32_t F,
           uint32_t K, uint32_t G, uint32_t U, int64_t* msg, int64_t* chunk, hipStream_t st);
void xrecv(const int64_t* msg, const int64_t* chunk, uint32_t G, uint32_t rank, uint32_t mine,
           uint32_t K, uint32_t nb, uint64_t cap, int64_t* tstart, int64_t* tcnt,
           int64_t* summary, hipStream_t st);
void hist_tables(const int64_t* hist, uint32_t F, uint32_t K, int64_t* start, int64_t* cnt,
                 hipStream_t st);

void stable_partition(Workspace* ws, const Tup* in, uint64_t n, Tup* out,
                      const Digit32& dig, uint32_t dbits, int padded,
                      int64_t* hist_out, int64_t* off_out, hipStream_t st);
void plan_partition(Workspace* ws, const Tup* in, uint64_t n, Tup* out,
                    const RangePlan* plan_dev, uint32_t dbits,
                    uint64_t* starts_dev, int64_t* hist_out, hipStream_t st);
#ifdef KEY_8B
void plan_partition_packed(Workspace* ws, const Tup* in, uint64_t n, uint64_t* out,
                           const RangePlan* plan_dev, const RangePlan& pack_plan,
                           uint32_t dbits, uint64_t* starts_dev, int64_t* hist_out,
                           unsigned int* pack_bad, hipStream_t st);
#endif
uint64_t sampled_capacity(uint64_t n, uint32_t dbits);
#ifndef SMJ_SHARDS
#define SMJ_SHARDS 8
#endif
constexpr uint32_t kShards = SMJ_SHARDS;
void sampled_partition(Workspace* ws, int nrel, const Tup* const* in, const uint64_t* n,
                       void* const* out, const RangePlan* plan_dev, uint32_t dbits,
                       unsigned int* sample, uint64_t* const* starts_dev,
                       int64_t* const* hist_out, uint64_t* const* seg_start,
                       int64_t* const* seg_cnt, unsigned int* flag_dev, hipStream_t st,
                       Layout lay, const RangePlan* host_plan, unsigned int* bad,
                       uint64_t pstride = 0, bool exact = false);
void hist_memcpy(Workspace* ws, const Tup* in, uint64_t n, Tup* out,
                 uint32_t dbits, hipStream_t st);
uint64_t lds_order_selfcheck(Workspace* ws, hipStream_t st);

extern const uint32_t kGroupTarget;
extern const uint32_t kTileTuples;
extern const uint32_t kGroupD3Max;
struct BucketSortArgs {
    const void* part[2];
    const uint64_t* bstart[2];
    const int64_t* bcount[2];
    const uint64_t* seg_start[2] = {nullptr, nullptr};
    const int64_t* seg_cnt[2] = {nullptr, nullptr};
    uint32_t nseg = kShards;
    void* tmp[2];
    Tup* out[2];
    uint64_t n[2];
    int nrel;
    uint32_t nbuckets;
    const RangePlan* plan_dev;
    unsigned long long* count_dev;
    const unsigned int* part_flag = nullptr;
    const RangePlan* host_plan = nullptr;
    Layout layout = Layout::Tuples;
    uint64_t pstride[2] = {0, 0};
    unsigned int* status = nullptr;
    const unsigned int* pack_bad = nullptr;
    uint32_t* status_out = nullptr;
    bool digit_fast = true;
    uint32_t stage = 7;
    hipEvent_t ev_tile = nullptr;
    hipEvent_t ev_bucket = nullptr;
    hipEvent_t ev_ovf = nullptr;
};
bool bucket_sort(Workspace* ws, const BucketSortArgs& a, hipStream_t st);
int tilepass_occupancy(Layout lay, uint32_t d2);

void plan_from_sample(Workspace* ws, const Tup* const* rels,
                      const uint64_t* ns, int nrel, uint32_t D1, uint32_t D2,
                      uint32_t D2cap, int64_t hint_min, int64_t hint_max,
                      RangePlan* plan_dev, hipStream_t st);

void segmented_sort(Workspace* ws, Tup* data, const uint64_t* seg_off_host,
                    const uint64_t* seg_len_host, uint32_t nseg, hipStream_t st);
void merge2(Workspace* ws, const Tup* a, uint64_t na, const Tup* b, uint64_t nb, Tup* out,
            hipStream_t st);
void merge_join_count(const Tup* r, uint64_t nr, const Tup* s, uint64_t ns,
                      unsigned long long* count_dev, hipStream_t st);
void merge_join_count_batch(Workspace* ws, const Tup* const* r, const uint64_t* nr,
                            const Tup* const* s, const uint64_t* ns, uint32_t k,
                            unsigned long long* count_dev, hipStream_t st);
void multiway_merge(Workspace* ws, const Tup* const* runs_host,
                    const uint64_t* lens_host, uint32_t k, Tup* out,
                    hipStream_t st);
void multiway_merge_tree(Workspace* ws, const Tup* const* runs_host,
                         const uint64_t* lens_host, uint32_t k, Tup* out,
                         hipStream_t st);

uint64_t materialize(Workspace* ws, const Tup* R, uint64_t nR, const Tup* S,
                     uint64_t nS, Tup* out, uint64_t out_cap, hipStream_t st);
uint64_t join_pairs(Workspace* ws, const Tup* R, uint64_t nR, const Tup* S, uint64_t nS,
                    void* r_out, void* s_out, void* key_out, uint64_t out_cap,
                    hipStream_t st);
uint64_t semi_join(Workspace* ws, const Tup* R, uint64_t nR, const Tup* S, uint64_t nS,
                   Tup* out, uint64_t out_cap, int anti, hipStream_t st);
void mat_scan(Workspace* ws, const uint64_t* cnt, uint64_t ntiles, uint64_t* base,
              uint64_t* ibase, uint64_t* tot, hipStream_t st);

uint64_t band_join(Workspace* ws, const Tup* R, uint64_t nR, const Tup* S, uint64_t nS,
                   int64_t lo, int64_t hi, void* r_out, void* s_out, void* r_key_out,
                   void* s_key_out, uint64_t out_cap, hipStream_t st);
void band_join_count(Workspace* ws, const Tup* R, uint64_t nR, const Tup* S, uint64_t nS,
                     int64_t lo, int64_t hi, unsigned long long* count_dev, hipStream_t st);

constexpr uint32_t kAsofBackward = 0, kAsofForward = 1, kAsofNearest = 2;
void asof_join(Workspace* ws, const Tup* R, uint64_t nR, const Tup* S, uint64_t nS,
               uint32_t dir, bool strict, uint64_t tolerance, uint32_t group_shift,
               int64_t* r_index_out, void* r_payload_out, void* r_key_out,
               unsigned long long* matched_dev, hipStream_t st);

constexpr uint32_t kOuterKeepR = 1, kOuterKeepS = 2;
uint64_t outer_join(Workspace* ws, const Tup* R, uint64_t nR, const Tup* S, uint64_t nS,
                    uint32_t keep, int64_t* r_index_out, int64_t* s_index_out,
                    void* r_payload_out, void* s_payload_out, void* key_out, uint64_t out_cap,
                    hipStream_t st);
void outer_join_count(Workspace* ws, const Tup* R, uint64_t nR, const Tup* S, uint64_t nS,
                      uint32_t keep, unsigned long long* count_dev, hipStream_t st);

uint64_t group_aggregate(Workspace* ws, const Tup* in, uint64_t n, uint32_t group_shift,
                         void* key_out, int64_t* start_out, int64_t* count_out,
                         int64_t* sum_out, void* min_out, void* max_out, uint64_t out_cap,
                         hipStream_t st);
void group_count(Workspace* ws, const Tup* in, uint64_t n, uint32_t group_shift,
                 unsigned long long* groups_dev, hipStream_t st);
uint32_t group_tile();

void gen_pk(Tup* out, uint64_t n, uint64_t first, uint64_t total,
            uint64_t seed, hipStream_t st);
void gen_fk(Tup* out, uint64_t n, uint64_t first, uint64_t total,
            uint64_t maxid, uint64_t seed, hipStream_t st);
void gen_zipf(Workspace* ws, Tup* out, uint64_t n, uint64_t first,
              uint64_t maxid, double theta, uint64_t seed, hipStream_t st);

}
```

Baseline: 93300 Mtuples/s.

## Drop prefix transpose kernel, fold region finalize and arg upload into existing kernels

New measurement: 93520 Mtuples/s (median of 2 runs). Within noise of the previous version (+0.2%).

```diff
diff --git a/avx-sort-merge-joins_amd/csrc/bucketsort.hip b/avx-sort-merge-joins_amd/csrc/bucketsort.hip
--- a/avx-sort-merge-joins_amd/csrc/bucketsort.hip
+++ b/avx-sort-merge-joins_amd/csrc/bucketsort.hip
@@ -111,9 +111,14 @@
     uint32_t* bucket;
     uint32_t* btile0;
     uint16_t* pref;
-    uint16_t* prefT;
-    uint32_t tstride;
 };
+
+__device__ __forceinline__ void pref_run(const TileTable& tt, uint32_t nb2, uint32_t t0,
+                                         uint32_t t, uint32_t g, uint32_t& lo, uint32_t& len) {
+    const uint16_t* pf = tt.pref + ((uint64_t)t0 * (nb2 + 1) + g) + t * (nb2 + 1);
+    lo = pf[0];
+    len = (uint32_t)pf[1] - lo;
+}
 
 struct OvfEntry {
     uint32_t bucket, d2;
@@ -573,29 +578,6 @@
     }
 }
 
-constexpr int PT_TILES = 64;
-__global__ void __launch_bounds__(256)
-k_preft(TileTable tt0, TileTable tt1, uint32_t nb0, const uint32_t* __restrict__ ntiles0,
-        const uint32_t* __restrict__ ntiles1, uint32_t nt0_host, uint32_t nt1_host,
-        uint32_t nb2) {
-    extern __shared__ uint16_t sp[];
-    const int r = blockIdx.x < nb0 ? 0 : 1;
-    const TileTable& tt = r ? tt1 : tt0;
-    const uint32_t ntl = (r ? ntiles1 : ntiles0) ? *(r ? ntiles1 : ntiles0)
-                                                 : (r ? nt1_host : nt0_host);
-    const uint32_t tb = (r ? blockIdx.x - nb0 : blockIdx.x) * PT_TILES;
-    if (tb >= ntl) return;
-    const uint32_t nt = min((uint32_t)PT_TILES, ntl - tb);
-    const uint32_t row = nb2 + 1;
-    const uint16_t* src = tt.pref + (uint64_t)tb * row;
-    for (uint32_t i = threadIdx.x; i < nt * row; i += 256) sp[i] = src[i];
-    __syncthreads();
-    for (uint32_t i = threadIdx.x; i < row * PT_TILES; i += 256) {
-        const uint32_t d = i / PT_TILES, t = i % PT_TILES;
-        if (t < nt) tt.prefT[(uint64_t)d * tt.tstride + tb + t] = sp[t * row + d];
-    }
-}
-
 struct GroupArgs {
     const void* tmp[2];
     Tup* out[2];
@@ -615,6 +597,9 @@
     uint32_t d3_fast;
     uint64_t pstride[2] = {0, 0};
     uint32_t pair;
+    unsigned int* status = nullptr;
+    unsigned int* status_host = nullptr;
+    uint32_t nactive = 0;
 };
 
 __device__ __forceinline__ uint32_t otid() {
@@ -641,11 +626,10 @@
 };
 
 struct SrcPlain {
-    __device__ static __forceinline__ void run(const TileTable& tt, uint32_t nb2, uint32_t t,
-                                               uint32_t g, uint32_t& lo, uint32_t& len) {
-        const uint16_t* pf = tt.prefT + (uint64_t)g * tt.tstride + t;
-        lo = pf[0];
-        len = (uint32_t)(pf[tt.tstride] - pf[0]);
+    __device__ static __forceinline__ void run(const TileTable& tt, uint32_t nb2, uint32_t t0,
+                                               uint32_t t, uint32_t g, uint32_t& lo,
+                                               uint32_t& len) {
+        pref_run(tt, nb2, t0, t, g, lo, len);
     }
     template <class V>
     __device__ static __forceinline__ auto load(const V& p) { return p[0]; }
@@ -720,7 +704,7 @@
         for (int h = 0; h < TPL; h++) {
             const uint32_t t = lane + 64 * h;
             if (nt <= 64 * TPL && t < nt) {
-                Src::run(A.tt[wid], A.nb2, t0 + t, g, M.lo[h], M.len[h]);
+                Src::run(A.tt[wid], A.nb2, t0, t, g, M.lo[h], M.len[h]);
                 M.toff[h] = (uint32_t)(A.tt[wid].off[t0 + t] - (wid ? M.bst[1] : M.bst[0]));
             }
         }
@@ -847,7 +831,7 @@
         unsigned long long acc = 0;
         for (uint32_t t = tid; t < nt; t += GS_THREADS) {
             uint32_t lo, len;
-            Src::run(A.tt[r], A.nb2, t0 + t, g, lo, len);
+            Src::run(A.tt[r], A.nb2, t0, t, g, lo, len);
             acc += ((unsigned long long)lo << 32) | len;
         }
         unsigned long long tot;
@@ -1394,6 +1378,20 @@
 
 __global__ void k_put_args(GroupArgs G, GroupArgs* dst) { *dst = G; }
 
+__device__ __forceinline__ void group_done(const GroupArgs& A) {
+    if (!A.status_host) return;
+    __builtin_amdgcn_fence(__ATOMIC_RELEASE, "workgroup");
+    __syncthreads();
+    if (threadIdx.x != 0) return;
+    if (__hip_atomic_fetch_add(&A.status[3], 1u, __ATOMIC_RELAXED, __HIP_MEMORY_SCOPE_AGENT) !=
+        A.nactive - 1)
+        return;
+    for (int i = 0; i < 3; i++)
+        A.status_host[i] = __hip_atomic_load(&A.status[i], __ATOMIC_RELAXED,
+                                             __HIP_MEMORY_SCOPE_AGENT);
+    A.status_host[3] = 0;
+}
+
 template <class Lay, int TPL, bool PAIR>
 __global__ void __launch_bounds__(GS_THREADS,
                                   (gs_wg_per_cu<typename Lay::W, PAIR>() * GS_THREADS / 256))
@@ -1401,7 +1399,10 @@
     typedef typename Lay::W W;
     const GroupArgs& A = SMJ_GS_ARGS_REF(Ap);
     extern __shared__ __attribute__((aligned(16))) unsigned char lds_raw[];
-    if (A.pack_bad && *A.pack_bad) return;
+    if (A.pack_bad && *A.pack_bad) {
+        group_done(A);
+        return;
+    }
     GroupLDS<W>& L = *reinterpret_cast<GroupLDS<W>*>(lds_raw);
 #if SMJ_GS_XCD
     const uint32_t nx = gridDim.x / 8, k = blockIdx.x / 8;
@@ -1420,6 +1421,7 @@
         matches = wave_sum(matches);
         if ((otid() & 63) == 0 && matches) atomicAdd(A.count_dev, matches);
     }
+    group_done(A);
 }
 
 #ifndef SMJ_SK_THREADS
@@ -1449,9 +1451,8 @@
 __device__ __forceinline__ typename Lay::CView skew_run(const GroupArgs& G, int r, uint32_t g,
                                                       uint32_t t0, uint32_t t, uint32_t& len) {
     const TileTable& tt = G.tt[r];
-    const uint16_t* pf = tt.prefT + (uint64_t)g * tt.tstride + t0 + t;
-    const uint32_t lo = pf[0];
-    len = (uint32_t)(pf[tt.tstride] - lo);
+    uint32_t lo;
+    pref_run(tt, G.nb2, t0, t, g, lo, len);
     return with_group(Lay::cview(G.tmp[r], G.pstride[r]), g, G.plan) + (tt.off[t0 + t] + lo);
 }
 
@@ -1550,9 +1551,9 @@
         uint64_t src = 0;
         if (tid < nt[r]) {
             const TileTable& tt = G.tt[r];
-            const uint16_t* pf = tt.prefT + (uint64_t)e.d2 * tt.tstride + t0[r] + tid;
-            len = (uint32_t)(pf[tt.tstride] - pf[0]);
-            src = tt.off[t0[r] + tid] + pf[0];
+            uint32_t lo;
+            pref_run(tt, G.nb2, t0[r], tid, e.d2, lo, len);
+            src = tt.off[t0[r] + tid] + lo;
         }
         const unsigned long long acc = ((unsigned long long)(len ? 1u : 0u) << 32) | len;
         unsigned long long tot;
@@ -1992,31 +1993,52 @@
 const uint32_t kGroupTarget = GS_CAP * 4 / 5 >= 2048 ? 2048 : (GS_CAP * 4 / 5 >= 1024 ? 1024 : 512);
 
 struct SegRel {
-    const int64_t* seg_cnt[2];
-    const int64_t* bcount[2];
+    int64_t* seg_cnt[2];
+    int64_t* bcount[2];
     const uint64_t* bstart[2];
     const uint64_t* seg_start[2];
     uint32_t* ntiles[2];
     uint64_t* ostart[2];
     TileTable tt[2];
+    const unsigned long long* cursor[2] = {nullptr, nullptr};
+    const uint64_t* cap_end[2] = {nullptr, nullptr};
+    unsigned int* flag = nullptr;
 };
 
 __global__ void __launch_bounds__(256)
-k_seg_scan(SegRel S, uint32_t nb, uint32_t nseg, uint32_t tsz) {
+k_seg_scan(SegRel S, uint32_t nb, uint32_t nseg, uint32_t tsz, GroupArgs G, GroupArgs* gslot) {
     const int r = blockIdx.x;
-    const int64_t* __restrict__ seg_cnt = S.seg_cnt[r];
-    const int64_t* __restrict__ bcount = S.bcount[r];
+    if (gslot && r == 0 && threadIdx.x == 0) *gslot = G;
+    int64_t* seg_cnt = S.seg_cnt[r];
+    int64_t* bcount = S.bcount[r];
+    const unsigned long long* __restrict__ cursor = S.cursor[r];
+    const uint64_t* __restrict__ cap_end = S.cap_end[r];
+    const uint64_t* __restrict__ seg_start = S.seg_start[r];
     uint32_t* __restrict__ btile0 = S.tt[r].btile0;
     uint64_t* __restrict__ ostart = S.ostart[r];
     __shared__ unsigned long long scr[5];
     __shared__ unsigned long long base;
     if (threadIdx.x == 0) base = 0;
     __syncthreads();
+    bool over = false;
     for (uint32_t b0 = 0; b0 < nb; b0 += 256) {
         const uint32_t b = b0 + threadIdx.x;
         uint32_t nt = 0;
         uint64_t cnt = 0;
-        if (b < nb) {
+        if (b < nb && cursor) {
+            int64_t tot = 0;
+            for (uint32_t q = 0; q < nseg; q++) {
+                const size_t i = (size_t)b * nseg + q;
+                const uint64_t cu = cursor[i], ce = cap_end[i];
+                const int64_t c = (int64_t)((cu < ce ? cu : ce) - seg_start[i]);
+                seg_cnt[i] = c;
+                tot += c;
+                over |= cu > ce;
+                nt += (uint32_t)((c + tsz - 1) / tsz);
+            }
+            bcount[b] = tot;
+            cnt = (uint64_t)tot;
+        } else if (b < nb) {
             for (uint32_t q = 0; q < nseg; q++)
                 nt += (uint32_t)((seg_cnt[(size_t)b * nseg + q] + tsz - 1) / tsz);
             cnt = (uint64_t)bcount[b];
@@ -2033,6 +2055,7 @@
         if (threadIdx.x == 0) base = run + tot;
         __syncthreads();
     }
+    if (over) atomicOr(S.flag, 1u);
     if (threadIdx.x == 0) {
         btile0[nb] = (uint32_t)(base >> 40);
         *S.ntiles[r] = (uint32_t)(base >> 40);
@@ -2060,33 +2083,6 @@
     }
 }
 
-static void launch_preft(const TileTable* tt, int nrel, const uint32_t* ub,
-                         uint32_t* const* ntiles, uint32_t nb2, hipStream_t st) {
-    const uint32_t nb0 = (ub[0] + PT_TILES - 1) / PT_TILES;
-    const uint32_t nb1 = nrel > 1 ? (ub[1] + PT_TILES - 1) / PT_TILES : 0;
-    if (nb0 + nb1 == 0) return;
-    const size_t lds = (size_t)PT_TILES * (nb2 + 1) * 2;
-    hipLaunchKernelGGL(k_preft, dim3(nb0 + nb1), dim3(256), lds, st, tt[0],
-                       tt[nrel > 1 ? 1 : 0], nb0, ntiles[0], nrel > 1 ? ntiles[1] : nullptr,
-                       ub[0], nrel > 1 ? ub[1] : 0u, nb2);
-}
-
-static void launch_preft_range(const TilePassArgs& T, int nrel, uint32_t nb2,
-                               hipStream_t st) {
-    TileTable tt[2];
-    uint32_t ub[2] = {0, 0};
-    uint32_t* nt[2] = {nullptr, nullptr};
-    for (int r = 0; r < 2; r++) {
-        tt[r] = T.tt[r];
-        if (r < nrel) {
-            tt[r].pref += (uint64_t)T.t0[r] * (nb2 + 1);
-            tt[r].prefT += T.t0[r];
-            ub[r] = T.nt[r];
-        }
-    }
-    launch_preft(tt, nrel, ub, nt, nb2, st);
-}
-
 template <class Lay, class LayO>
 static void launch_tilepass(const TilePassArgs& T, size_t lds, hipStream_t st) {
     const uint32_t nblk = T.nt[0] + T.nt[1];
@@ -2140,13 +2136,31 @@
     return (nwg + 7) & ~7u;
 }
 
+static GroupArgs* group_args_slot(Workspace* ws) {
+    return (GroupArgs*)ws->scratch("gs_args", sizeof(GroupArgs));
+}
+
+static uint32_t groupsort_active(uint32_t nwg, uint32_t per, uint32_t g_begin, uint32_t g_end) {
+    uint32_t n = 0;
+    for (uint32_t b = 0; b < nwg; b++) {
+#if SMJ_GS_XCD
+        const uint32_t nx = nwg / 8, k = b / 8;
+        const uint32_t lo = g_begin + (b % 8) * nx * per;
+        const uint32_t hi = lo + nx * per < g_end ? lo + nx * per : g_end;
+        n += lo + k < hi;
+#else
+        n += g_begin + b * per < g_end;
+#endif
+    }
+    return n;
+}
+
 template <class Lay>
-static void launch_groupsort(Workspace* ws, int tpl, uint32_t nwg, hipStream_t st,
-                             const GroupArgs& G0) {
+static void launch_groupsort(int tpl, uint32_t nwg, hipStream_t st, const GroupArgs& G0,
+                             const GroupArgs* slot) {
     const size_t lds = sizeof(GroupLDS<typename Lay::W>);
 #if SMJ_GS_ARGS_MEM
-    GroupArgs* G = (GroupArgs*)ws->scratch("gs_args", sizeof(GroupArgs));
-    hipLaunchKernelGGL(k_put_args, dim3(1), dim3(1), 0, st, G0, G);
+    const GroupArgs* G = slot;
 #else
     const GroupArgs& G = G0;
 #endif
@@ -2185,9 +2199,9 @@
     const uint64_t nmax = nrel > 1 && a.n[1] > a.n[0] ? a.n[1] : a.n[0];
     const uint32_t tsz = tile_elems_l<Lay>();
     TileTable tt[2];
-    static const char* names[2][8] = {
-        {"bs_off0", "bs_len0", "bs_bkt0", "bs_bt00", "bs_pref0", "bs_ost0", "bs_nt0", "bs_preft0"},
-        {"bs_off1", "bs_len1", "bs_bkt1", "bs_bt01", "bs_pref1", "bs_ost1", "bs_nt1", "bs_preft1"}};
+    static const char* names[2][7] = {
+        {"bs_off0", "bs_len0", "bs_bkt0", "bs_bt00", "bs_pref0", "bs_ost0", "bs_nt0"},
+        {"bs_off1", "bs_len1", "bs_bkt1", "bs_bt01", "bs_pref1", "bs_ost1", "bs_nt1"}};
     uint64_t* ostart[2] = {nullptr, nullptr};
     uint32_t* ntiles[2] = {nullptr, nullptr};
     uint32_t ub[2] = {0, 0};
@@ -2198,8 +2212,6 @@
         tt[r].bucket = (uint32_t*)ws->scratch(names[r][2], (size_t)ub[r] * 4);
         tt[r].btile0 = (uint32_t*)ws->scratch(names[r][3], (nb + 1) * 4);
         tt[r].pref = (uint16_t*)ws->scratch(names[r][4], (size_t)ub[r] * (nb2 + 1) * 2);
-        tt[r].prefT = (uint16_t*)ws->scratch(names[r][7], (size_t)ub[r] * (nb2 + 1) * 2);
-        tt[r].tstride = ub[r];
         ostart[r] = (uint64_t*)ws->scratch(names[r][5], (size_t)nb * 8);
         ntiles[r] = (uint32_t*)ws->scratch(names[r][6], 4);
     }
@@ -2207,23 +2219,12 @@
     int sel[2] = {0, 0}, ns = 0;
     for (int r = 0; r < nrel; r++)
         if (a.stage & (1u << r)) sel[ns++] = r;
-    if (ns) {
-        SegRel S;
-        for (int i = 0; i < 2; i++) {
-            const int rr = sel[i < ns ? i : 0];
-            S.seg_cnt[i] = a.seg_cnt[rr];
-            S.bcount[i] = a.bcount[rr];
-            S.bstart[i] = a.bstart[rr];
-            S.seg_start[i] = a.seg_start[rr];
-            S.ntiles[i] = ntiles[rr];
-            S.ostart[i] = ostart[rr];
-            S.tt[i] = tt[rr];
-        }
-        hipLaunchKernelGGL(k_seg_scan, dim3(ns), dim3(256), 0, st, S, nb, a.nseg, tsz);
-        hipLaunchKernelGGL(k_tiles2, dim3(nb, ns), dim3(64), 0, st, S, a.nseg, tsz);
-    }
-    if (a.ev_tile) SMJ_CHECK(hipEventRecord(a.ev_tile, st));
-
+    const bool pending = a.reg_cursor[0] != nullptr;
+    if (pending && (ns != nrel || a.nseg != kShards || !a.part_flag)) {
+        fprintf(stderr, "[ERROR] smj: an unfinished sampled partition needs the tile stage "
+                "of all its relations in one call\n");
+        abort();
+    }
     const uint32_t ngroups = nb * nb2;
     const uint32_t ovf_cap = ngroups;
     OvfEntry* ovf = (OvfEntry*)ws->scratch("bs_ovf", (size_t)ovf_cap * sizeof(OvfEntry));
@@ -2275,43 +2276,74 @@
     G.ovf_cap = ovf_cap;
     G.g_begin = 0;
     G.g_end = ngroups;
+    const bool group_now = (a.stage & 4) != 0;
+    const uint32_t maxwg = (G.pair ? gs_wg_per_cu<W, true>() : gs_wg_per_cu<W, false>()) * 256;
+    const uint32_t nwg = groupsort_grid(ngroups, maxwg, G.per);
+    uint32_t* h = (uint32_t*)ws->host_pinned("bs_h_flagovf", 16);
+    if (group_now) {
+        h[0] = h[1] = h[2] = 0;
+        h[3] = a.status ? 1u : 0u;
+        if (a.status) {
+            void* hd = nullptr;
+            SMJ_CHECK(hipHostGetDevicePointer(&hd, h, 0));
+            G.status = a.status;
+            G.status_host = (unsigned int*)hd;
+            G.nactive = groupsort_active(nwg, G.per, G.g_begin, G.g_end);
+        }
+    }
+    GroupArgs* gslot = group_now ? group_args_slot(ws) : nullptr;
     if (ns) {
-        {
-            TraceScope ts(ws, "k_tilepass", st);
-            launch_tilepass<Lay, LayG>(T, tilepass_lds<Lay>(nb2), st);
-        }
-        const uint32_t ubs[2] = {T.nt[0], T.nt[1]};
-        uint32_t* nts[2] = {ntiles[sel[0]], ntiles[sel[ns > 1 ? 1 : 0]]};
-        launch_preft(T.tt, ns, ubs, nts, nb2, st);
-    }
-    if (!(a.stage & 4)) {
+        SegRel S;
+        for (int i = 0; i < 2; i++) {
+            const int rr = sel[i < ns ? i : 0];
+            S.seg_cnt[i] = const_cast<int64_t*>(a.seg_cnt[rr]);
+            S.bcount[i] = const_cast<int64_t*>(a.bcount[rr]);
+            S.bstart[i] = a.bstart[rr];
+            S.seg_start[i] = a.seg_start[rr];
+            S.ntiles[i] = ntiles[rr];
+            S.ostart[i] = ostart[rr];
+            S.tt[i] = tt[rr];
+            if (pending) {
+                S.cursor[i] = a.reg_cursor[rr];
+                S.cap_end[i] = a.reg_cap_end[rr];
+            }
+        }
+        if (pending) S.flag = const_cast<unsigned int*>(a.part_flag);
+        hipLaunchKernelGGL(k_seg_scan, dim3(ns), dim3(256), 0, st, S, nb, a.nseg, tsz, G, gslot);
+        hipLaunchKernelGGL(k_tiles2, dim3(nb, ns), dim3(64), 0, st, S, a.nseg, tsz);
+    } else if (gslot) {
+        hipLaunchKernelGGL(k_put_args, dim3(1), dim3(1), 0, st, G, gslot);
+    }
+    if (a.ev_tile) SMJ_CHECK(hipEventRecord(a.ev_tile, st));
+    if (ns) {
+        TraceScope ts(ws, "k_tilepass", st);
+        launch_tilepass<Lay, LayG>(T, tilepass_lds<Lay>(nb2), st);
+    }
+    if (!group_now) {
         SMJ_CHECK(hipGetLastError());
         return true;
     }
     if (a.ev_bucket) SMJ_CHECK(hipEventRecord(a.ev_bucket, st));
     Workspace::SkewStats stats;
     {
-        const uint32_t maxwg =
-            (G.pair ? gs_wg_per_cu<W, true>() : gs_wg_per_cu<W, false>()) * 256;
-        const uint32_t nwg = groupsort_grid(ngroups, maxwg, G.per);
         TraceScope ts(ws, "k_groupsort", st);
         stats.tpl = (uint32_t)group_tpl(nmax, nb, a.nseg, tsz);
-        launch_groupsort<LayG>(ws, (int)stats.tpl, nwg, st, G);
+        launch_groupsort<LayG>((int)stats.tpl, nwg, st, G, gslot);
     }
     SMJ_CHECK(hipGetLastError());
     if (a.ev_ovf) SMJ_CHECK(hipEventRecord(a.ev_ovf, st));
 
-    uint32_t* h = (uint32_t*)ws->host_pinned("bs_h_flagovf", 16);
-    h[0] = h[1] = h[2] = h[3] = 0;
-    if (a.status) {
-        SMJ_CHECK(hipMemcpyAsync(h, a.status, 16, hipMemcpyDeviceToHost, st));
-    } else {
+    if (!a.status) {
         SMJ_CHECK(hipMemcpyAsync(h, a.part_flag, 4, hipMemcpyDeviceToHost, st));
         SMJ_CHECK(hipMemcpyAsync(h + 2, novf, 4, hipMemcpyDeviceToHost, st));
         if (a.pack_bad)
             SMJ_CHECK(hipMemcpyAsync(h + 1, a.pack_bad, 4, hipMemcpyDeviceToHost, st));
     }
     ws->wait_stream(st);
+    if (h[3]) {
+        fprintf(stderr, "[ERROR] smj: the group pass did not report its status\n");
+        abort();
+    }
     if (a.status_out) {
         a.status_out[0] = h[0];
         a.status_out[1] = h[1];
@@ -2360,7 +2392,6 @@
 bool bucket_sort(Workspace* ws, const BucketSortArgs& a, hipStream_t st) {
     const uint32_t nb = a.nbuckets;
     const int nrel = a.nrel;
-    set_lds_attr((const void*)k_preft, PT_TILES * ((1 << kMaxD2) + 1) * 2);
     set_pass_attrs<LayTup>();
     if (a.host_plan && a.seg_start[0] && a.part_flag) {
         switch (a.layout) {
@@ -2405,9 +2436,9 @@
     const uint32_t nb2 = 1u << hplan->D2;
 
     TileTable tt[2];
-    static const char* names[2][6] = {
-        {"bs_off0", "bs_len0", "bs_bkt0", "bs_bt00", "bs_pref0", "bs_preft0"},
-        {"bs_off1", "bs_len1", "bs_bkt1", "bs_bt01", "bs_pref1", "bs_preft1"}};
+    static const char* names[2][5] = {
+        {"bs_off0", "bs_len0", "bs_bkt0", "bs_bt00", "bs_pref0"},
+        {"bs_off1", "bs_len1", "bs_bkt1", "bs_bt01", "bs_pref1"}};
     uint32_t* hbt = (uint32_t*)ws->host_pinned("bs_hbt", (size_t)2 * (nb + 1) * 4);
     uint64_t* hdst = (uint64_t*)ws->host_pinned("bs_hdst", (size_t)2 * nb * 8);
     uint64_t* ostart[2] = {nullptr, nullptr};
@@ -2433,8 +2464,6 @@
         tt[r].bucket = (uint32_t*)ws->scratch(names[r][2], ntl * 4);
         tt[r].btile0 = (uint32_t*)ws->scratch(names[r][3], (nb + 1) * 4);
         tt[r].pref = (uint16_t*)ws->scratch(names[r][4], ntl * (nb2 + 1) * 2);
-        tt[r].prefT = (uint16_t*)ws->scratch(names[r][5], ntl * (nb2 + 1) * 2);
-        tt[r].tstride = (uint32_t)ntl;
         SMJ_CHECK(hipMemcpyAsync(tt[r].btile0, bt0, (nb + 1) * 4,
                                  hipMemcpyHostToDevice, st));
         ostart[r] = (uint64_t*)ws->scratch(r ? "bs_ost1" : "bs_ost0", (size_t)nb * 8);
@@ -2492,25 +2521,23 @@
             ntiles += T.nt[r];
         }
     }
-    if (ntiles) {
-        {
-            TraceScope ts(ws, "k_tilepass", st);
-            launch_tilepass<LayTup, LayTup>(T, tp_lds, st);
-        }
-        launch_preft_range(T, nrel, nb2, st);
-    }
-    if (a.ev_bucket) SMJ_CHECK(hipEventRecord(a.ev_bucket, st));
     G.g_begin = 0;
     G.g_end = nb * nb2;
+    const uint32_t maxwg = gs_wg_per_cu<Tup>() * 256;
+    const uint32_t nwg = groupsort_grid(G.g_end - G.g_begin, maxwg, G.per);
+    GroupArgs* gslot = group_args_slot(ws);
+    hipLaunchKernelGGL(k_put_args, dim3(1), dim3(1), 0, st, G, gslot);
+    if (ntiles) {
+        TraceScope ts(ws, "k_tilepass", st);
+        launch_tilepass<LayTup, LayTup>(T, tp_lds, st);
+    }
+    if (a.ev_bucket) SMJ_CHECK(hipEventRecord(a.ev_bucket, st));
     Workspace::SkewStats stats;
     {
-        const uint32_t ng = G.g_end - G.g_begin;
-        const uint32_t maxwg = gs_wg_per_cu<Tup>() * 256;
-        const uint32_t nwg = groupsort_grid(ng, maxwg, G.per);
         TraceScope ts(ws, "k_groupsort", st);
         const uint64_t nmax = nrel > 1 && a.n[1] > a.n[0] ? a.n[1] : a.n[0];
         stats.tpl = (uint32_t)group_tpl(nmax, nb, nseg, tsz);
-        launch_groupsort<LayTup>(ws, (int)stats.tpl, nwg, st, G);
+        launch_groupsort<LayTup>((int)stats.tpl, nwg, st, G, gslot);
     }
     SMJ_CHECK(hipGetLastError());
     if (a.ev_ovf) SMJ_CHECK(hipEventRecord(a.ev_ovf, st));
diff --git a/avx-sort-merge-joins_amd/csrc/capi.hip b/avx-sort-merge-joins_amd/csrc/capi.hip
--- a/avx-sort-merge-joins_amd/csrc/capi.hip
+++ b/avx-sort-merge-joins_amd/csrc/capi.hip
@@ -344,6 +344,7 @@
         lay = layout_of(rung, caps.p96_ok);
         const bool exact = rung == Rung::Exact;
         const bool planes = lay == Layout::P48 || lay == Layout::P96;
+        RegionsPending pending{{nullptr, nullptr}, {nullptr, nullptr}};
         const bool check = lay != Layout::Tuples || (guessed && rung == Rung::Sampled);
         unsigned int* bad = check ? status + 1 : nullptr;
         hipLaunchKernelGGL(k_join_begin, dim3(1), dim3(256), 0, st, plan, hplan,
@@ -365,7 +366,8 @@
         } else {
             void* outs_v[2] = {part[0], part[nrel > 1 ? 1 : 0]};
             sampled_partition(ws, nrel, rels, ns, outs_v, plan, D1, sample, bst, bh, sgs, sgc,
-                              status, st, lay, plan_on_host ? &hplan : nullptr, bad, pstride[0]);
+                              status, st, lay, plan_on_host ? &hplan : nullptr, bad, pstride[0],
+                              false, plan_on_host ? &pending : nullptr);
         }
         SMJ_CHECK(hipEventRecord(ws->ev[1], st));
         BucketSortArgs a;
@@ -379,6 +381,8 @@
             if (!exact) {
                 a.seg_start[r] = sgs[r];
                 a.seg_cnt[r] = sgc[r];
+                a.reg_cursor[r] = pending.cursor[r];
+                a.reg_cap_end[r] = pending.cap_end[r];
             }
             a.pstride[r] = pstride[r];
         }
diff --git a/avx-sort-merge-joins_amd/csrc/partition.hip b/avx-sort-merge-joins_amd/csrc/partition.hip
--- a/avx-sort-merge-joins_amd/csrc/partition.hip
+++ b/avx-sort-merge-joins_amd/csrc/partition.hip
@@ -1847,7 +1847,7 @@
                        int64_t* const* hist_out, uint64_t* const* seg_start,
                        int64_t* const* seg_cnt, unsigned int* flag_dev, hipStream_t st,
                        Layout lay, const RangePlan* host_plan, unsigned int* bad,
-                       uint64_t pstride, bool exact) {
+                       uint64_t pstride, bool exact, RegionsPending* pending) {
     PlanDigit1 dig{plan_dev};
     const uint32_t nbins = 1u << dbits;
     if (lay == Layout::P96 && (sizeof(Tup) != 16 || !host_plan || !pstride)) {
@@ -1957,7 +1957,15 @@
         sampled_scatter(ws, in[r], n[r], out[r], 0, dig, nbins, R.cursor[r], R.cap_end[r], pk,
                         bad && host_plan ? bad : (unsigned int*)nullptr, st);
     }
-    hipLaunchKernelGGL(k_regions_done, dim3(nrel), dim3(256), 0, st, R, nbins, flag_dev);
+    if (pending && !exact) {
+        for (int r = 0; r < 2; r++) {
+            pending->cursor[r] = R.cursor[r];
+            pending->cap_end[r] = R.cap_end[r];
+        }
+    } else {
+        if (pending) *pending = RegionsPending{{nullptr, nullptr}, {nullptr, nullptr}};
+        hipLaunchKernelGGL(k_regions_done, dim3(nrel), dim3(256), 0, st, R, nbins, flag_dev);
+    }
     SMJ_CHECK(hipGetLastError());
 }
 
diff --git a/avx-sort-merge-joins_amd/csrc/smj_internal.hpp b/avx-sort-merge-joins_amd/csrc/smj_internal.hpp
--- a/avx-sort-merge-joins_amd/csrc/smj_internal.hpp
+++ b/avx-sort-merge-joins_amd/csrc/smj_internal.hpp
@@ -272,13 +272,18 @@
 #define SMJ_SHARDS 8
 #endif
 constexpr uint32_t kShards = SMJ_SHARDS;
+struct RegionsPending {
+    const unsigned long long* cursor[2];
+    const uint64_t* cap_end[2];
+};
 void sampled_partition(Workspace* ws, int nrel, const Tup* const* in, const uint64_t* n,
                        void* const* out, const RangePlan* plan_dev, uint32_t dbits,
                        unsigned int* sample, uint64_t* const* starts_dev,
                        int64_t* const* hist_out, uint64_t* const* seg_start,
                        int64_t* const* seg_cnt, unsigned int* flag_dev, hipStream_t st,
                        Layout lay, const RangePlan* host_plan, unsigned int* bad,
-                       uint64_t pstride = 0, bool exact = false);
+                       uint64_t pstride = 0, bool exact = false,
+                       RegionsPending* pending = nullptr);
 void hist_memcpy(Workspace* ws, const Tup* in, uint64_t n, Tup* out,
                  uint32_t dbits, hipStream_t st);
 uint64_t lds_order_selfcheck(Workspace* ws, hipStream_t st);
@@ -293,6 +298,8 @@
     const uint64_t* seg_start[2] = {nullptr, nullptr};
     const int64_t* seg_cnt[2] = {nullptr, nullptr};
     uint32_t nseg = kShards;
+    const unsigned long long* reg_cursor[2] = {nullptr, nullptr};
+    const uint64_t* reg_cap_end[2] = {nullptr, nullptr};
     void* tmp[2];
     Tup* out[2];
     uint64_t n[2];
```
